# Raiden-Makoto/MLX-VAE

Hardware: AMD Instinct MI355X
Metric: SELFIES sequences/sec (whole node), AR-CVAE training step (higher is better)
Workload: dtype f32

## Files before the change

### include/arcvae_hip.h

```cpp
#ifndef ARCVAE_HIP_H
#define ARCVAE_HIP_H

#include <stdint.h>

#ifdef __cplusplus
extern "C" {
#endif

#define ARCVAE_OK 0
#define ARCVAE_ERR_ARG (-1)
#define ARCVAE_ERR_LAUNCH (-2)
#define ARCVAE_ERR_DEVICE (-3)

#define ARCVAE_GEMM_ACCUMULATE 1
#define ARCVAE_GEMM_TANH 2
#define ARCVAE_GEMM_SPLITK 4
#define ARCVAE_GEMM_NO_SKINNY 8
#define ARCVAE_GEMM_TILE64 16
#define ARCVAE_GEMM_TILE128 32
#define ARCVAE_GEMM_DTANH 64
#define ARCVAE_GEMM_TILE_WIDE 128
#define ARCVAE_GEMM_BF16 256
#define ARCVAE_GEMM_SPLIT3 512
#define ARCVAE_GEMM_QUIET 1024
#define ARCVAE_LSTM_RETILE 1
#define ARCVAE_LSTM_BF16 2
#define ARCVAE_LSTM_SPLIT3 4
#define ARCVAE_PERSIST_BF16 2
#define ARCVAE_RS_HALF 16
#define ARCVAE_RS_HALF1 32
#define ARCVAE_DEC_SPLIT3 512
#define ARCVAE_DEC_NO_GPRE 1024
#define ARCVAE_DEC_PART_HEAD 2048
#define ARCVAE_DEC_PART_TAIL 4096
#define ARCVAE_DEC_BF16 256

#ifdef ARCVAE_HIP_BUILD
typedef hipStream_t arcvae_stream_t;
#else
typedef void* arcvae_stream_t;
#endif

int arcvae_abi_version(int* arch_gfx950);

int arcvae_gemm_f32(int transA, int transB, int M, int N, int K, const float* A, int lda,
                    const float* B, int ldb, float* C, int ldc, const float* bias, int flags,
                    arcvae_stream_t stream);

int arcvae_enc_lstm_ws_floats(int B, int T, int H, int L, int flags, long* floats );
int arcvae_transpose_tokens(const int32_t* src_bt, int32_t* dst_tb, int B, int T, arcvae_stream_t stream);
int arcvae_enc_lstm_forward(const int32_t* x_tb, const float* table0, const float* const* Wx,
                            const float* const* Wh, const float* const* bias, float* hseq, float* hseq_t,
                            float* cseq, float* gseq, float* wt, float* wT_bwd , int B, int T, int V,
                            int H, int L, int flags , const long* ws_floats ,
                            void* h_oct ,
                            unsigned long long* trace , arcvae_stream_t stream);
int arcvae_enc_lstm_tiled(int B, int H, int L);
int arcvae_enc_lstm_tiled_for(int B, int H, int L, int flags);
int arcvae_enc_lstm_operand_slots(int B, int T, int H, int L, int flags);
int arcvae_enc_lstm_backward(const float* const* Wx, const float* const* Wh, const float* cseq,
                             const float* gseq, const float* dh_top, int ld_dh_top, float* dG, float* dG_t,
                             float* dcs, float* dxs, float* wT, int B, int T, int H, int L, int s_begin,
                             int s_end, int flags ,
                             const long* ws_floats ,
                             void* dG_oct ,
                             unsigned* start_signal ,
                             unsigned long long* trace , arcvae_stream_t stream);
int arcvae_enc_lstm_persistent_ok(int B, int T, int H, int L);
int arcvae_enc_lstm_forward_persistent(const int32_t* x_tb, const float* table0, const float* const* Wx,
                                       const float* const* Wh, const float* const* bias, float* hseq, float* cseq,
                                       float* gseq, float* wT_bwd, long wT_bwd_floats , float* comb ,
                                       unsigned* sync_ws, unsigned* start_signal, int B, int T, int V, int H, int L,
                                       int flags, unsigned long long* trace, arcvae_stream_t stream);
int arcvae_enc_prologue(const int32_t* x_bt, int32_t* x_tb, float* zero_f32, long n_zero, float* zero2_f32 , long n_zero2,
                        unsigned* sync_ws, int n_sync, int sync_keep ,
                        const float* cond, const float* Wc, const float* bc, float* comb, float* stats, int n_stats,
                        float* onehot_ws, int V, int B, int T, int H, int C, arcvae_stream_t stream);
int arcvae_enc_lstm_bwd_persistent_ok(int B, int T, int H, int L);
int arcvae_enc_lstm_backward_persistent(const float* cseq, const float* gseq, const float* dh_top, int ld_dh_top,
                                        float* dG, float* dcs, float* dxs, const float* wT, unsigned* sync_ws,
                                        unsigned* start_signal, int B, int T, int H, int L, int s_begin, int s_end,
                                        int chunk_index, unsigned long long* trace, arcvae_stream_t stream);
int arcvae_enc_lstm_bwd_rs_ok(int B, int T, int H, int L);
long arcvae_enc_lstm_bwd_rs_part_floats(int B, int T, int H, int L);
int arcvae_enc_lstm_bwd_rs_halves(int B, int T, int H, int L);
int arcvae_enc_lstm_persist_groups(int B, int H, int L);
int arcvae_enc_lstm_backward_persistent_rs(const float* const* Wx, const float* const* Wh, const float* cseq,
                                           const float* gseq, const float* dh_top, int ld_dh_top, float* dG, float* dcs,
                                           float* dxs, float* part_ws, long part_ws_floats, unsigned* sync_ws,
                                           unsigned* start_signal, int B, int T, int H, int L, int s_begin, int s_end, int chunk_index,
                                           int flags ,
                                           unsigned long long* trace,
                                           arcvae_stream_t stream);
int arcvae_enc_lstm_backward_fused(const float* const* Wx, const float* const* Wh, const float* cseq, const float* gseq,
                                   const float* hseq, const int32_t* x_tb, const float* dh_top, int ld_dh_top,
                                   float* dG, float* dcs, float* dxs, float* part_ws, long part_ws_floats, unsigned* sync_ws,
                                   unsigned* start_signal, float* const* dWx, float* const* dWh, float* const* dbias,
                                   float* dtable_ws, int B, int T, int V, int H, int L, int s_begin, int s_end,
                                   int chunk_index, unsigned long long* trace, arcvae_stream_t stream);
int arcvae_enc_lstm_wgrad(const int32_t* x_tb, const float* emb, const float* Wx0, const float* hseq,
                          const float* dG, float* dtable_ws, float* onehot_ws, float* dEmb, float* const* dWx,
                          float* const* dWh, float* const* dbias, int B, int T, int V, int E, int H, int L,
                          int t_lo, int t_hi, int first, int last, int parts ,
                          const void* h_oct, const void* dG_oct ,
                          const long* ws_floats , arcvae_stream_t stream);

int arcvae_enc_heads_forward(const float* hT, const float* cond, const float* Wc, const float* bc,
                             const float* Wmu, const float* bmu, const float* Wlh, const float* blh,
                             const float* Wlv, const float* blv, const float* eps, float* comb, float* lh,
                             float* mu_raw, float* lv_raw, float* mu, float* logvar, float* z, float* stats,
                             int B, int H, int Z, int C, float free_bits, int comb_ready, arcvae_stream_t stream);
int arcvae_enc_seam_ok(int B, int H, int Z);
int arcvae_enc_seam(const float* comb, const float* Wmu, const float* bmu, const float* Wlh, const float* blh, const float* Wlv,
                    const float* blv, const float* eps, const float* hyper, float* lh, float* mu_raw, float* lv_raw, float* mu,
                    float* logvar, float* z, float* stats, float* scalars, float* dmu_raw, float* dlv_raw, float* dlh, float* dcomb,
                    unsigned* sync_ws, int B, int H, int Z, int T, float free_bits, int phases, int flags, arcvae_stream_t stream);
int arcvae_stats_set_recon(const float* rowloss, int B, float* stats, int Z, arcvae_stream_t stream);
int arcvae_latent_loss(const float* stats, const float* hyper, const float* mu, const float* logvar,
                       float* scalars, float* dmu_raw, float* dlv_raw, int B, int Z, int T, float free_bits,
                       arcvae_stream_t stream);
int arcvae_loss_finalize(const float* stats, float* scalars, int Z, int T, const unsigned* guard_a,
                         const unsigned* guard_b, arcvae_stream_t stream);
int arcvae_recon_finalize(const float* rowloss, int B, float* stats, float* scalars, int Z, int T,
                          const unsigned* guard_a, const unsigned* guard_b, arcvae_stream_t stream);
int arcvae_enc_heads_backward(const float* cond, const float* Wmu, const float* Wlh, const float* Wlv,
                              const float* comb, const float* lh, const float* dmu_raw, const float* dlv_raw,
                              float* dlh, float* dcomb, float* dWc, float* dbc, float* dWmu, float* dbmu,
                              float* dWlh, float* dblh, float* dWlv, float* dblv, int B, int H, int Z, int C,
                              int phase , arcvae_stream_t stream);

int arcvae_reparameterize(const float* mu, const float* logvar, const float* eps, float* z, long n,
                          arcvae_stream_t stream);
int arcvae_latent_stats(const float* mu, const float* logvar, float* stats, float* krow, int B, int Z,
                        float free_bits, arcvae_stream_t stream);
int arcvae_ce_rows(const float* logits, const int32_t* targets, float* ce, long R, int V, arcvae_stream_t stream);
int arcvae_sum(const float* x, long n, float* out, float scale, arcvae_stream_t stream);

int arcvae_dec_forward_dense(const float* emb, const float* const* Wx, const float* const* bias,
                             const float* Wout, const float* bout, const float* cond, float* tableD,
                             float* hact, float* gpre, float* logits, float* lse, int32_t* nxt, int B, int V,
                             int E, int C, int H, int L, int mode, float temperature, arcvae_stream_t stream);
int arcvae_dec_chain_ce(const int32_t* x, const uint8_t* coins, const int32_t* nxt, const float* lse,
                        const float* logits, int32_t* fed, float* rowloss, int B, int T, int V,
                        arcvae_stream_t stream);
int arcvae_dec_ce_backward(const int32_t* x, const int32_t* fed, const float* logits, const float* lse,
                           float* dlogits, int B, int T, int V, float inv_count, arcvae_stream_t stream);
int arcvae_dec_gather_logits(const float* dense, const int32_t* fed, float* out, int B, int T, int V,
                             arcvae_stream_t stream);
int arcvae_dec_sample_chain(const int32_t* nxt, int32_t* tokens, int32_t* first_end, int B, int V,
                            int max_len, int end_token, arcvae_stream_t stream);
int arcvae_dec_sample_chain_categorical(const float* dense_logits, int32_t* tokens, int32_t* first_end, int B, int V, int max_len,
                                        int end_token, float temperature, unsigned long long seed, arcvae_stream_t stream);
int arcvae_dec_row_lse(const float* dense_logits, float* lse, long R, int V, float temperature, arcvae_stream_t stream);
int arcvae_dec_beam_ws_bytes(int B, int K, int max_len, long* bytes);
int arcvae_dec_beam_search(const float* dense_logits, const float* lse, int32_t* tokens, float* scores, int32_t* lengths, void* ws,
                           long ws_bytes, int B, int V, int K, int max_len, int min_len, int end_token, int pad_token,
                           float temperature, arcvae_stream_t stream);
int arcvae_dec_sequence_logprob(const float* dense_logits, const float* lse, const int32_t* tokens, float* out, int B, int T, int V,
                                int end_token, float temperature, arcvae_stream_t stream);
int arcvae_dec_viterbi_ws_bytes(int B, int V, int max_len, long* bytes);
int arcvae_dec_viterbi(const float* dense_logits, const float* lse, int32_t* tokens, float* score, int32_t* length, void* ws,
                       long ws_bytes, int B, int V, int max_len, int min_len, int end_token, int pad_token, float temperature,
                       arcvae_stream_t stream);
int arcvae_dec_chain_marginals(const float* dense_logits, const float* lse, float* alive, int B, int V, int max_len, int end_token,
                               float temperature, arcvae_stream_t stream);
#define ARCVAE_KBEST_ROWS_IN_FLIGHT 1024
int arcvae_dec_kbest_ws_bytes(int B, int V, int K, int max_len, long* bytes);
int arcvae_dec_kbest(const float* dense_logits, const float* lse, int32_t* tokens , float* scores ,
                     int32_t* lengths , void* ws, long ws_bytes, int B, int V, int K, int max_len, int min_len,
                     int end_token, int pad_token, float temperature, arcvae_stream_t stream);
int arcvae_dec_topkp_rows(const float* dense_logits, long table_rows, const int32_t* rows, long R, int V, float temperature,
                          int top_k, float top_p, int32_t* count, int32_t* tokens, float* cum, arcvae_stream_t stream);
int arcvae_dec_topkp_ws_bytes(int B, int V, int top_k, long* bytes);
int arcvae_dec_sample_chain_topkp(const float* dense_logits, int32_t* tokens, int32_t* first_end, void* ws, long ws_bytes, int B,
                                  int V, int max_len, int end_token, float temperature, int top_k, float top_p,
                                  const unsigned long long* seed, arcvae_stream_t stream);
int arcvae_dec_backward_dense(const float* emb, const float* const* Wx, const float* const* bias,
                              const float* Wout, const float* cond, const float* tableD, const float* hact,
                              const float* gpre, const float* dlogits, float* dh, float* dG, float* dtableD,
                              float* wcpart, float* dEmb, float* const* dWx, float* const* dbias, float* dWout,
                              float* dbout, int B, int V, int E, int C, int H, int L, int flags ,
                              arcvae_stream_t stream);

int arcvae_dense_stack_ok(long R, int H, int L);
int arcvae_dense_stack_ws_floats(long R, int H, int L, long* floats );
int arcvae_dense_stack_forward(const float* const* Wx, const float* const* bias, float* hact, float* gates, float* ws,
                               long ws_floats , long R,
                               int H, int L, int flags ,
                               arcvae_stream_t stream);
int arcvae_dense_stack_backward(const float* gates, const float* dh_top, float* dG, float* dh0, float* const* dWx,
                                float* const* dbias, float* ws, long ws_floats, long R, int H, int L, int flags , arcvae_stream_t stream);

int arcvae_adam_update(float* params, const float* grads, float* m, float* v, long n, double lr,
                       double beta1, double beta2, double eps, const unsigned* guard_a, const unsigned* guard_b,
                       arcvae_stream_t stream);

int arcvae_adam_update_finalize(float* params, const float* grads, float* m, float* v, long n, double lr, double beta1,
                                double beta2, double eps, const unsigned* guard_a, const unsigned* guard_b,
                                const float* rowloss, int B, float* stats, float* scalars, int Z, int T, arcvae_stream_t stream);

int arcvae_prop_ws_floats(int B, int Z, int C, int Hp, long* floats);
int arcvae_prop_forward(const float* z, const float* cond, const float* W1, const float* b1, const float* W2,
                        const float* b2, const float* hyper, float* pred, float* scalars, float* ws, long ws_floats,
                        int B, int Z, int C, int Hp, arcvae_stream_t stream);
int arcvae_prop_backward(const float* z, const float* cond, const float* eps, const float* mu_raw, const float* lv_raw,
                         const float* W1, const float* b1, const float* W2, const float* b2, const float* hyper,
                         float* d_mu_raw, float* d_lv_raw, float* pred, float* ws, long ws_floats, int B, int Z, int C,
                         int Hp, arcvae_stream_t stream);
int arcvae_prop_wgrad(const float* z, const float* ws, long ws_floats, const float* hyper, float* dW1, float* db1,
                      float* dW2, float* db2, float* scalars, int B, int Z, int C, int Hp, arcvae_stream_t stream);

int arcvae_grad_sumsq_partials(long n, long* count);
int arcvae_grad_sumsq(const float* grads, long n, float* partials, long partials_cap, arcvae_stream_t stream);
int arcvae_adam_update_clipped(float* params, const float* grads, float* m, float* v, long n, double lr, double beta1,
                               double beta2, double eps, const unsigned* guard_a, const unsigned* guard_b,
                               const float* partials, long n_partials, double max_norm, float* scalars, arcvae_stream_t stream);
int arcvae_adam_update_finalize_clipped(float* params, const float* grads, float* m, float* v, long n, double lr,
                                        double beta1, double beta2, double eps, const unsigned* guard_a,
                                        const unsigned* guard_b, const float* rowloss, int B, float* stats, float* scalars,
                                        int Z, int T, const float* partials, long n_partials, double max_norm,
                                        arcvae_stream_t stream);

int arcvae_adam_step(float* params, const float* grads, float* m, float* v, long n,
                     const float* lr_dev,
                     double beta1, double beta2, double eps,
                     const unsigned* guard_a, const unsigned* guard_b,
                     const float* rowloss, int B, float* stats, float* scalars, int Z, int T,
                     const float* partials, long n_partials, double max_norm,
                     arcvae_stream_t stream);

int arcvae_colsum_accum(const float* X, int rows, int cols, int ld, float* out, float scale,
                        arcvae_stream_t stream);
int arcvae_segsum_rows_accum(const float* X, const int32_t* seg, int rows, int nseg, int cols, float* out,
                             arcvae_stream_t stream);
int arcvae_transpose_batched(const float* const* src, float* const* dst, const int* rows, const int* cols,
                             int n, arcvae_stream_t stream);
int arcvae_debug_occupy(int blocks, int threads, int lds_bytes, int spin_us, arcvae_stream_t stream);
int arcvae_scale_inplace(float* x, long n, float s, arcvae_stream_t stream);
int arcvae_zero(float* x, int rows, int cols, int ld, arcvae_stream_t stream);
int arcvae_table_finalize(const float* dT, const float* Wx0, int ldw, const float* emb, float* dEmb, float* dWx0,
                          float* db0, int V, int E, int G, arcvae_stream_t stream);
int arcvae_table_fold(const float* dT, const float* dT2, const float* Wx0, int ldw, const float* emb, float* dEmb,
                      float* dWx0, float* db0, int V, int E, int G, int g_lo, int g_hi, arcvae_stream_t stream);
int arcvae_gate_wait(const unsigned* flag, unsigned* steps, unsigned stride, unsigned offset, int advance,
                     unsigned max_polls, unsigned* err, arcvae_stream_t stream);
int arcvae_gate_set(unsigned* flag, unsigned value, int add, arcvae_stream_t stream);
// ... 9 lines not shown
```

### mlx-vae_amd/arcvae_hip/_lib.py

```python
from __future__ import annotations

import ctypes as C
import os
from typing import Iterable, Optional, Sequence

import torch

_HERE = os.path.dirname(os.path.abspath(__file__))
LIB_PATH = os.environ.get("ARCVAE_HIP_LIB", os.path.join(_HERE, "libarcvae_hip.so"))

GEMM_ACCUMULATE = 1
GEMM_TANH = 2
GEMM_SPLITK = 4
GEMM_NO_SKINNY = 8
GEMM_BF16 = 256
GEMM_SPLIT3 = 512
GEMM_QUIET = 1024
LSTM_RETILE = 1
LSTM_BF16 = 2
LSTM_SPLIT3 = 4
RS_HALF, RS_HALF1 = 16, 32
PERSIST_BF16 = 2
DEC_BF16 = 256
DEC_SPLIT3 = 512
DEC_PART_HEAD = 2048
DEC_PART_TAIL = 4096
DEC_NO_GPRE = 1024
WGRAD_BF16 = 128
WGRAD_QUIET = 512
WGRAD_FOLD = 8192

_vp = C.c_void_p
_i = C.c_int
_f = C.c_float
_d = C.c_double
_l = C.c_long
_pp = C.POINTER(C.c_void_p)
_ip = C.POINTER(C.c_int)
_lp = C.POINTER(C.c_long)

SIGNATURES = {
    "arcvae_abi_version": [_ip],
    "arcvae_gemm_f32": [_i, _i, _i, _i, _i, _vp, _i, _vp, _i, _vp, _i, _vp, _i, _vp],
    "arcvae_transpose_tokens": [_vp, _vp, _i, _i, _vp],
    "arcvae_enc_lstm_ws_floats": [_i, _i, _i, _i, _i, _lp],
    "arcvae_enc_lstm_forward": [_vp, _vp, _pp, _pp, _pp, _vp, _vp, _vp, _vp, _vp, _vp, _i, _i, _i, _i, _i, _i, _lp, _vp, _vp, _vp],
    "arcvae_enc_lstm_tiled": [_i, _i, _i],
    "arcvae_enc_lstm_tiled_for": [_i, _i, _i, _i],
    "arcvae_enc_lstm_operand_slots": [_i, _i, _i, _i, _i],
    "arcvae_dense_stack_ok": [_l, _i, _i],
    "arcvae_dense_stack_ws_floats": [_l, _i, _i, _lp],
    "arcvae_dense_stack_forward": [_pp, _pp, _vp, _vp, _vp, _l, _l, _i, _i, _i, _vp],
    "arcvae_dense_stack_backward": [_vp, _vp, _vp, _vp, _pp, _pp, _vp, _l, _l, _i, _i, _i, _vp],
    "arcvae_enc_lstm_persistent_ok": [_i, _i, _i, _i],
    "arcvae_enc_lstm_forward_persistent": [_vp, _vp, _pp, _pp, _pp, _vp, _vp, _vp, _vp, _l, _vp, _vp, _vp, _i, _i, _i, _i, _i, _i, _vp, _vp],
    "arcvae_enc_prologue": [_vp, _vp, _vp, _l, _vp, _l, _vp, _i, _i, _vp, _vp, _vp, _vp, _vp, _i, _vp, _i, _i, _i, _i, _i, _vp],
    "arcvae_enc_lstm_bwd_persistent_ok": [_i, _i, _i, _i],
    "arcvae_enc_lstm_backward_persistent": [_vp, _vp, _vp, _i, _vp, _vp, _vp, _vp, _vp, _vp, _i, _i, _i, _i, _i, _i, _i, _vp, _vp],
    "arcvae_enc_lstm_bwd_rs_ok": [_i, _i, _i, _i],
    "arcvae_enc_lstm_bwd_rs_halves": [_i, _i, _i, _i],
    "arcvae_enc_lstm_persist_groups": [_i, _i, _i],
    "arcvae_enc_lstm_bwd_rs_part_floats": [_i, _i, _i, _i],
    "arcvae_enc_lstm_backward_persistent_rs": [_pp, _pp, _vp, _vp, _vp, _i, _vp, _vp, _vp, _vp, _l, _vp, _vp, _i, _i, _i, _i, _i, _i, _i, _i, _vp, _vp],
    "arcvae_enc_lstm_backward_fused": [_pp, _pp, _vp, _vp, _vp, _vp, _vp, _i, _vp, _vp, _vp, _vp, _l, _vp, _vp, _pp, _pp, _pp, _vp,
                                       _i, _i, _i, _i, _i, _i, _i, _i, _vp, _vp],
    "arcvae_enc_lstm_backward": [_pp, _pp, _vp, _vp, _vp, _i, _vp, _vp, _vp, _vp, _vp, _i, _i, _i, _i, _i, _i, _i, _lp, _vp, _vp, _vp, _vp],
    "arcvae_enc_lstm_wgrad": [_vp, _vp, _vp, _vp, _vp, _vp, _vp, _vp, _pp, _pp, _pp, _i, _i, _i, _i, _i, _i, _i, _i, _i, _i, _i, _vp, _vp, _lp, _vp],
    "arcvae_enc_heads_forward": [_vp] * 19 + [_i, _i, _i, _i, _f, _i, _vp],
    "arcvae_enc_seam_ok": [_i, _i, _i],
    "arcvae_enc_seam": [_vp] * 22 + [_i, _i, _i, _i, _f, _i, _i, _vp],
    "arcvae_stats_set_recon": [_vp, _i, _vp, _i, _vp],
    "arcvae_latent_loss": [_vp, _vp, _vp, _vp, _vp, _vp, _vp, _i, _i, _i, _f, _vp],
    "arcvae_loss_finalize": [_vp, _vp, _i, _i, _vp, _vp, _vp],
    "arcvae_recon_finalize": [_vp, _i, _vp, _vp, _i, _i, _vp, _vp, _vp],
    "arcvae_enc_heads_backward": [_vp] * 18 + [_i, _i, _i, _i, _i, _vp],
    "arcvae_dec_forward_dense": [_vp, _pp, _pp, _vp, _vp, _vp, _vp, _vp, _vp, _vp, _vp, _vp,
                                 _i, _i, _i, _i, _i, _i, _i, _f, _vp],
    "arcvae_dec_chain_ce": [_vp, _vp, _vp, _vp, _vp, _vp, _vp, _i, _i, _i, _vp],
    "arcvae_dec_ce_backward": [_vp, _vp, _vp, _vp, _vp, _i, _i, _i, _f, _vp],
    "arcvae_dec_gather_logits": [_vp, _vp, _vp, _i, _i, _i, _vp],
    "arcvae_dec_sample_chain": [_vp, _vp, _vp, _i, _i, _i, _i, _vp],
    "arcvae_dec_sample_chain_categorical": [_vp, _vp, _vp, _i, _i, _i, _i, _f, C.c_ulonglong, _vp],
    "arcvae_dec_row_lse": [_vp, _vp, _l, _i, _f, _vp],
    "arcvae_dec_beam_ws_bytes": [_i, _i, _i, _lp],
    "arcvae_dec_beam_search": [_vp, _vp, _vp, _vp, _vp, _vp, _l, _i, _i, _i, _i, _i, _i, _i, _f, _vp],
    "arcvae_dec_sequence_logprob": [_vp, _vp, _vp, _vp, _i, _i, _i, _i, _f, _vp],
    "arcvae_dec_viterbi_ws_bytes": [_i, _i, _i, _lp],
    "arcvae_dec_viterbi": [_vp, _vp, _vp, _vp, _vp, _vp, _l, _i, _i, _i, _i, _i, _i, _f, _vp],
    "arcvae_dec_chain_marginals": [_vp, _vp, _vp, _i, _i, _i, _i, _f, _vp],
    "arcvae_dec_kbest_ws_bytes": [_i, _i, _i, _i, _lp],
    "arcvae_dec_kbest": [_vp, _vp, _vp, _vp, _vp, _vp, _l, _i, _i, _i, _i, _i, _i, _i, _f, _vp],
    "arcvae_dec_topkp_rows": [_vp, _l, _vp, _l, _i, _f, _i, _f, _vp, _vp, _vp, _vp],
    "arcvae_dec_topkp_ws_bytes": [_i, _i, _i, _lp],
    "arcvae_dec_sample_chain_topkp": [_vp, _vp, _vp, _vp, _l, _i, _i, _i, _i, _f, _i, _f, _vp, _vp],
    "arcvae_dec_backward_dense": [_vp, _pp, _pp, _vp, _vp, _vp, _vp, _vp, _vp, _vp, _vp, _vp, _vp, _vp,
                                  _pp, _pp, _vp, _vp, _i, _i, _i, _i, _i, _i, _i, _vp],
    "arcvae_reparameterize": [_vp, _vp, _vp, _vp, _l, _vp],
    "arcvae_latent_stats": [_vp, _vp, _vp, _vp, _i, _i, _f, _vp],
    "arcvae_ce_rows": [_vp, _vp, _vp, _l, _i, _vp],
    "arcvae_sum": [_vp, _l, _vp, _f, _vp],
    "arcvae_adam_update": [_vp, _vp, _vp, _vp, _l, _d, _d, _d, _d, _vp, _vp, _vp],
    "arcvae_adam_update_finalize": [_vp, _vp, _vp, _vp, _l, _d, _d, _d, _d, _vp, _vp, _vp, _i, _vp, _vp, _i, _i, _vp],
    "arcvae_colsum_accum": [_vp, _i, _i, _i, _vp, _f, _vp],
    "arcvae_segsum_rows_accum": [_vp, _vp, _i, _i, _i, _vp, _vp],
    "arcvae_transpose_batched": [_pp, _pp, _ip, _ip, _i, _vp],
    "arcvae_scale_inplace": [_vp, _l, _f, _vp],
    "arcvae_debug_occupy": [_i, _i, _i, _i, _vp],
    "arcvae_zero": [_vp, _i, _i, _i, _vp],
    "arcvae_table_finalize": [_vp, _vp, _i, _vp, _vp, _vp, _vp, _i, _i, _i, _vp],
    "arcvae_table_fold": [_vp, _vp, _vp, _i, _vp, _vp, _vp, _vp, _i, _i, _i, _i, _i, _vp],
    "arcvae_gate_wait": [_vp, _vp, C.c_uint, C.c_uint, _i, C.c_uint, _vp, _vp],
    "arcvae_gate_set": [_vp, C.c_uint, _i, _vp],
    "arcvae_tile_weights": [_pp, _pp, _ip, _ip, _i, _i, _vp],
    "arcvae_copy_buffers": [_pp, _pp, _lp, _i, _vp],
    "arcvae_prop_ws_floats": [_i, _i, _i, _i, _lp],
    "arcvae_prop_forward": [_vp] * 10 + [_l, _i, _i, _i, _i, _vp],
    "arcvae_prop_backward": [_vp] * 14 + [_l, _i, _i, _i, _i, _vp],
    "arcvae_prop_wgrad": [_vp, _vp, _l] + [_vp] * 6 + [_i, _i, _i, _i, _vp],
    "arcvae_grad_sumsq_partials": [_l, _lp],
    "arcvae_grad_sumsq": [_vp, _l, _vp, _l, _vp],
    "arcvae_adam_update_clipped": [_vp, _vp, _vp, _vp, _l, _d, _d, _d, _d, _vp, _vp, _vp, _l, _d, _vp, _vp],
    "arcvae_adam_update_finalize_clipped": [_vp, _vp, _vp, _vp, _l, _d, _d, _d, _d, _vp, _vp, _vp, _i, _vp, _vp, _i, _i,
                                            _vp, _l, _d, _vp],
    "arcvae_adam_step": [_vp, _vp, _vp, _vp, _l, _vp, _d, _d, _d, _vp, _vp, _vp, _i, _vp, _vp, _i, _i, _vp, _l, _d, _vp],
}

LONG_RESULTS = {"arcvae_enc_lstm_bwd_rs_part_floats"}

_lib: Optional[C.CDLL] = None


class ArcvaeHipError(RuntimeError):
    pass


def load() -> C.CDLL:
    global _lib
    if _lib is not None:
        return _lib
    if not os.path.exists(LIB_PATH):
        raise ArcvaeHipError(
            f"{LIB_PATH} not found: build it with `make -C mlx-vae_amd/csrc` "
            "(or `python -c 'import __graft_entry__ as g; g.build()'`). There is no CPU fallback.")
    lib = C.CDLL(LIB_PATH)
    for name, argtypes in SIGNATURES.items():
        fn = getattr(lib, name)
        fn.argtypes = argtypes
        fn.restype = C.c_long if name in LONG_RESULTS else C.c_int
    _lib = lib
    return lib


def check(rc: int, what: str) -> None:
    if rc != 0:
        raise ArcvaeHipError(f"{what} failed with code {rc} "
                             "(-1 bad argument/shape, -2 launch error, -3 device)")


def call(name: str, *args) -> None:
    check(getattr(load(), name)(*args), name)


def ptr(t: Optional[torch.Tensor]) -> C.c_void_p:
    if t is None:
        return C.c_void_p(0)
    if not t.is_cuda:
        raise ArcvaeHipError("arcvae_hip kernels need device tensors (no CPU path)")
    if not t.is_contiguous():
        raise ArcvaeHipError("arcvae_hip kernels need contiguous tensors")
    return C.c_void_p(t.data_ptr())


def ptr_array(ts: Sequence[Optional[torch.Tensor]]):
    arr = (C.c_void_p * len(ts))()
    for i, t in enumerate(ts):
        arr[i] = None if t is None else ptr(t).value
    return C.cast(arr, _pp), arr


def stream_ptr(stream: Optional[torch.cuda.Stream] = None) -> C.c_void_p:
    s = stream if stream is not None else torch.cuda.current_stream()
    return C.c_void_p(s.cuda_stream)


def gemm(transA: bool, transB: bool, M: int, N: int, K: int, A: torch.Tensor, lda: int, Bm: torch.Tensor,
         ldb: int, Cm: torch.Tensor, ldc: int, bias: Optional[torch.Tensor] = None, flags: int = 0,
         a_off: int = 0, b_off: int = 0, c_off: int = 0) -> None:
    def p(t, off):
        return C.c_void_p(t.data_ptr() + 4 * off)
    call("arcvae_gemm_f32", int(transA), int(transB), M, N, K, p(A, a_off), lda, p(Bm, b_off), ldb,
         p(Cm, c_off), ldc, ptr(bias), flags, stream_ptr())
```

### mlx-vae_amd/arcvae_hip/engine.py

```python
from __future__ import annotations

import ctypes as C
import dataclasses
import os
from typing import Dict, Optional, Sequence, Tuple

import numpy as np
import torch

from . import _lib
from ._lib import call, ptr, ptr_array, stream_ptr
from .store import ParamStore

SCALAR_KEYS = ("total_loss", "recon_loss", "kl_loss", "weighted_kl", "collapse_penalty", "prop_loss",
               "weighted_prop_loss", "mutual_info", "mi_penalty")


@dataclasses.dataclass(frozen=True)
class ModelDims:
    V: int
    E: int
    H: int
    Z: int
    C: int
# ... 5 lines not shown
        if not (1 <= self.L <= 8):
            raise ValueError("num_layers must be in [1, 8]")
        if not (1 <= self.C <= 8):
            raise ValueError("num_conditions must be in [1, 8]")
        if not (2 <= self.V <= 255):
            raise ValueError("vocab_size must be in [2, 255] (the vocabulary-dense decoder's per-row V x V histogram lives in LDS)")


class DeviceRate:
    __slots__ = ("word",)

    def __init__(self, word: torch.Tensor):
        self.word = word


LR_DEVICE = "lr_device"


def lr_key(lr):
    return LR_DEVICE if isinstance(lr, DeviceRate) else float(lr)


class Workspace:

    def __init__(self, d: ModelDims, B: int, T: int, device, train: bool = True):
        f32 = dict(dtype=torch.float32, device=device)
        i32 = dict(dtype=torch.int32, device=device)
        V, E, H, Z, Cc, L = d.V, d.E, d.H, d.Z, d.C, d.L
        G, BV = 4 * H, B * V
        self.B, self.T = B, T
        self.bf16 = False
        self.bf16_parts = 0
        self.planes = False
        self.x = torch.zeros(B, T, **i32)
        self.x_tb = torch.zeros(T, B, **i32)
        self.coins = torch.ones(T, dtype=torch.uint8, device=device)
        self.cond = torch.zeros(B, Cc, **f32)
        self._hyper_vals = None
        self.eps = torch.zeros(B, Z, **f32)
        self.hyper = torch.zeros(8, **f32)
        self.rate = DeviceRate(torch.zeros(1, **f32))
        self._rate_val = None
        self.table0 = torch.empty(V, G, **f32)
        self.hseq = torch.empty(L, T, B, H, **f32)
        RS = int(os.environ.get("ARCVAE_RING", "16"))
        RS = T if (RS <= 0 or RS > T) else RS
        self.hseq_t = torch.empty(L, RS, B * H * 3 // 2, **f32)
        self.wt = torch.empty(2 * L - 1, G * H * 3 // 2, **f32)
        self.cseq = torch.empty(L, T, B, H, **f32)
        self.gseq = torch.empty(L, T, B, G, **f32)
        self.comb = torch.empty(B, 2 * H, **f32)
        self.lh = torch.empty(B, 2 * H, **f32)
        self.mu_raw = torch.empty(B, Z, **f32)
        self.lv_raw = torch.empty(B, Z, **f32)
        self.mu = torch.empty(B, Z, **f32)
        self.logvar = torch.empty(B, Z, **f32)
        self.z = torch.empty(B, Z, **f32)
        self.stats = torch.zeros(2 * Z + 4, **f32)
        self.psync = torch.zeros(8192, **i32)
        self.psync_words = 5696
        self.seam_bwd_done = False
        self.bptt_rearmed = False
        self.trace_fwd: Optional[torch.Tensor] = None
        self.trace_bwd: Optional[torch.Tensor] = None
        self.scalars = torch.zeros(16, **f32)
        self.tableD = torch.empty(V, G, **f32)
        self.hact = torch.empty(L, BV, H, **f32)
        self.gpre = torch.empty(max(L - 1, 1), BV, G, **f32)
        self.logits = torch.empty(BV, V, **f32)
        self.lse = torch.empty(BV, **f32)
        self.nxt = torch.zeros(BV, **i32)
        self.fed = torch.zeros(B, T, **i32)
        self.rowloss = torch.zeros(B, **f32)
        if train:
            self.dmu_raw = torch.empty(B, Z, **f32)
            self.dlv_raw = torch.empty(B, Z, **f32)
            self.dlh = torch.empty(B, 2 * H, **f32)
            self.dcomb = torch.empty(B, 2 * H, **f32)
            self.dG = self.gseq if os.environ.get("ARCVAE_INPLACE_DG", "1") != "0" else torch.empty(L, T, B, G, **f32)
            self.dG_t = torch.empty(L, RS, B * G * 3 // 2, **f32)
            self.dcs = torch.empty(L, RS, B, H, **f32)
            self.dxs = torch.empty(L, RS, B, H, **f32)
            self.wT = torch.empty(2 * L - 1, H * G * 3 // 2, **f32)
            self.dtables = torch.zeros(2, V, G, **f32)
            self.dtable0 = self.dtables[0]
            self.dtable1 = self.dtables[1]
            self.tables_zeroed = False
            self.onehot = torch.empty(T * B, (V + 3) // 4 * 4, **f32)
            npart = _lib.load().arcvae_enc_lstm_bwd_rs_part_floats(B, T, H, L)
            if npart > 0:
                self.ppart = torch.empty(npart, **f32)
            self.dlogits = torch.empty(BV, V, **f32)
            self.ddh = torch.empty(2, BV, H, **f32)
            self.ddG = torch.empty(BV, G, **f32)
            self.dtableD = torch.empty(V, G, **f32)
            self.wcpart = torch.empty(V, G, max(Cc, 1), **f32)


def _lstm_flags(ws) -> int:
    if ws.bf16_parts & 1:
        return _lib.LSTM_BF16
    return _lib.LSTM_SPLIT3 if os.environ.get("ARCVAE_LSTM_SPLIT3", "1") != "0" else 0


def _caps(ws, h=None, g=None):
    def n(t):
        return 0 if t is None else t.numel() * t.element_size() // 4
    h = ws.hseq_t if h is None else h
    g = getattr(ws, "dG_t", None) if g is None else g
    return (C.c_long * 4)(n(h), n(g), n(ws.wt), n(getattr(ws, "wT", None)))


def _oct(ws, name: str) -> C.c_void_p:
    t = getattr(ws, name, None)
    return ptr(t) if t is not None else C.c_void_p(0)


def _layer_ptrs(store: ParamStore, L: int, leaf: str, grad: bool = False, skip0: bool = False):
    get = store.g if grad else store.p
    ts = [None if (skip0 and l == 0) else get(f"lstm_layer_{l}.{leaf}") for l in range(L)]
    return ptr_array(ts)


def bptt_reduce_scatter_ok(ws, d: ModelDims) -> bool:
    if os.environ.get("ARCVAE_PERSIST_BWD", "3") != "3":
        return False
    return _lib.load().arcvae_enc_lstm_bwd_rs_ok(ws.B, ws.T, d.H, d.L) == 1


def fused_wgrad_ok(ws, d: ModelDims) -> bool:
    return os.environ.get("ARCVAE_FUSED_WGRAD", "0") == "1" and d.V <= 128 and bptt_reduce_scatter_ok(ws, d)


def persistent_forward_ok(ws: Workspace, d: ModelDims) -> bool:
    return _lib.load().arcvae_enc_lstm_persistent_ok(ws.B, ws.T, d.H, d.L) == 1


def seam_fused_ok(ws: Workspace, d: ModelDims) -> bool:
    return persistent_forward_ok(ws, d) and _lib.load().arcvae_enc_seam_ok(ws.B, d.H, d.Z) == 1


def encoder_seam(enc: ParamStore, ws: Workspace, d: ModelDims, free_bits: float, phases: int) -> None:
    train = (phases & 2) != 0
    call("arcvae_enc_seam", ptr(ws.comb), ptr(enc.p("fc_mu.weight")), ptr(enc.p("fc_mu.bias")),
         ptr(enc.p("fc_logvar_hidden.weight")), ptr(enc.p("fc_logvar_hidden.bias")), ptr(enc.p("fc_logvar.weight")),
         ptr(enc.p("fc_logvar.bias")), ptr(ws.eps), ptr(ws.hyper), ptr(ws.lh), ptr(ws.mu_raw), ptr(ws.lv_raw), ptr(ws.mu),
         ptr(ws.logvar), ptr(ws.z), ptr(ws.stats), ptr(ws.scalars), ptr(ws.dmu_raw) if train else C.c_void_p(0),
         ptr(ws.dlv_raw) if train else C.c_void_p(0), ptr(ws.dlh) if train else C.c_void_p(0),
         ptr(ws.dcomb) if train else C.c_void_p(0), ptr(ws.psync), ws.B, d.H, d.Z, ws.T, float(free_bits), phases, 1, stream_ptr())
    if train:
        ws.seam_bwd_done = True


def encoder_forward(enc: ParamStore, ws: Workspace, d: ModelDims, free_bits: float,
                    start_signal: Optional[C.c_void_p] = None, zero_grad: bool = False, seam: int = 1) -> None:
    B, T = ws.B, ws.T
    G = 4 * d.H
    s = stream_ptr()
    wx, _k1 = _layer_ptrs(enc, d.L, "Wx", skip0=True)
    wh, _k2 = _layer_ptrs(enc, d.L, "Wh")
    bs, _k3 = _layer_ptrs(enc, d.L, "bias", skip0=True)
    if persistent_forward_ok(ws, d):
        grad = enc.grad if zero_grad else None
        tabs = ws.dtables if (zero_grad and hasattr(ws, "dtables")) else None
        ws.tables_zeroed = tabs is not None
        ws.bptt_rearmed = True
        call("arcvae_enc_prologue", ptr(ws.x), ptr(ws.x_tb), ptr(grad), C.c_long(grad.numel() if grad is not None else 0),
             ptr(tabs), C.c_long(tabs.numel() if tabs is not None else 0), ptr(ws.psync), ws.psync_words, 500, ptr(ws.cond), ptr(enc.p("condition_fc.weight")), ptr(enc.p("condition_fc.bias")),
             ptr(ws.comb), ptr(ws.stats), 2 * d.Z + 4, ptr(ws.onehot) if (zero_grad and hasattr(ws, "onehot")) else C.c_void_p(0),
             d.V, B, T, d.H, d.C, s)
        comb_ready = 1
        call("arcvae_gemm_f32", 0, 1, d.V, G, d.E, ptr(enc.p("embedding.weight")), d.E,
             ptr(enc.p("lstm_layer_0.Wx")), d.E, ptr(ws.table0), G, ptr(enc.p("lstm_layer_0.bias")), 0, s)
        need_wT = hasattr(ws, "wT") and not bptt_reduce_scatter_ok(ws, d)
        call("arcvae_enc_lstm_forward_persistent", ptr(ws.x_tb), ptr(ws.table0), wx, wh, bs, ptr(ws.hseq),
             ptr(ws.cseq), ptr(ws.gseq), ptr(ws.wT) if need_wT else C.c_void_p(0), C.c_long(ws.wT.numel() if need_wT else 0),
             ptr(ws.comb), ptr(ws.psync),
             start_signal if start_signal is not None else C.c_void_p(0), B, T, d.V, d.H, d.L,
             1 | (_lib.PERSIST_BF16 if ws.bf16_parts & 1 else 0) | (_lstm_flags(ws) & _lib.LSTM_SPLIT3), ptr(ws.trace_fwd), s)
    else:
        comb_ready = 0
        if zero_grad:
            enc.grad.zero_()
        call("arcvae_transpose_tokens", ptr(ws.x), ptr(ws.x_tb), B, T, s)
        call("arcvae_gemm_f32", 0, 1, d.V, G, d.E, ptr(enc.p("embedding.weight")), d.E,
             ptr(enc.p("lstm_layer_0.Wx")), d.E, ptr(ws.table0), G, ptr(enc.p("lstm_layer_0.bias")), 0, s)
        wT = ptr(ws.wT) if hasattr(ws, "wT") else C.c_void_p(0)
        if start_signal is not None:
            call("arcvae_gate_set", start_signal, 1, 1, s)
        call("arcvae_enc_lstm_forward", ptr(ws.x_tb), ptr(ws.table0), wx, wh, bs, ptr(ws.hseq), ptr(ws.hseq_t),
             ptr(ws.cseq), ptr(ws.gseq), ptr(ws.wt), wT, B, T, d.V, d.H, d.L, _lstm_flags(ws), _caps(ws),
             _oct(ws, "h_oct"), ptr(ws.trace_fwd), s)
    if comb_ready and seam_fused_ok(ws, d):
        encoder_seam(enc, ws, d, free_bits, 3 if (seam == 3 and hasattr(ws, "dcomb")) else 1)
        return
    hT = ws.hseq[d.L - 1, T - 1]
    call("arcvae_enc_heads_forward", ptr(hT), ptr(ws.cond), ptr(enc.p("condition_fc.weight")),
         ptr(enc.p("condition_fc.bias")), ptr(enc.p("fc_mu.weight")), ptr(enc.p("fc_mu.bias")),
         ptr(enc.p("fc_logvar_hidden.weight")), ptr(enc.p("fc_logvar_hidden.bias")),
         ptr(enc.p("fc_logvar.weight")), ptr(enc.p("fc_logvar.bias")), ptr(ws.eps), ptr(ws.comb), ptr(ws.lh),
         ptr(ws.mu_raw), ptr(ws.lv_raw), ptr(ws.mu), ptr(ws.logvar), ptr(ws.z), ptr(ws.stats), B, d.H, d.Z,
         d.C, float(free_bits), comb_ready, s)


def _dec_gemm_bits(ws) -> int:
    if ws.bf16_parts & 2:
        return _lib.DEC_BF16
    return _lib.DEC_SPLIT3 if getattr(ws, "dec_split3", False) else 0


def decoder_forward_dense(dec: ParamStore, ws: Workspace, d: ModelDims, mode: int = 0,
                          temperature: float = 1.0, keep_gpre: bool = True, alone: bool = False) -> None:
    if not keep_gpre:
        mode |= _lib.DEC_NO_GPRE
    wx, _k1 = _layer_ptrs(dec, d.L, "Wx")
    bs, _k2 = _layer_ptrs(dec, d.L, "bias")

    def part(bits):
        call("arcvae_dec_forward_dense", ptr(dec.p("embedding.weight")), wx, bs, ptr(dec.p("fc_out.weight")),
             ptr(dec.p("fc_out.bias")), ptr(ws.cond), ptr(ws.tableD), ptr(ws.hact), ptr(ws.gpre), ptr(ws.logits),
             ptr(ws.lse), ptr(ws.nxt), ws.B, d.V, d.E, d.C, d.H, d.L, mode | bits | _dec_gemm_bits(ws),
             float(temperature), stream_ptr())

    if alone and not keep_gpre and not (ws.bf16_parts & 2) and os.environ.get("ARCVAE_SAMPLER_TILED", "0") == "1" \
            and _lib.load().arcvae_dense_stack_ok(ws.B * d.V, d.H, d.L) == 1:
        if getattr(ws, "dense_ws_fwd", None) is None:
            n = C.c_long(0)
            _lib.load().arcvae_dense_stack_ws_floats(ws.B * d.V, d.H, d.L, C.byref(n))
            ws.dense_ws_fwd = torch.empty(n.value, dtype=torch.float32, device=ws.hact.device)
        mode &= ~_lib.DEC_NO_GPRE
        part(_lib.DEC_PART_HEAD)
        call("arcvae_dense_stack_forward", wx, bs, ptr(ws.hact), C.c_void_p(0), ptr(ws.dense_ws_fwd), C.c_long(ws.dense_ws_fwd.numel()),
             ws.B * d.V, d.H, d.L, 1, stream_ptr())
        part(_lib.DEC_PART_TAIL)
        return
    if keep_gpre and getattr(ws, "dense_ws", None) is not None:
        part(_lib.DEC_PART_HEAD)
        call("arcvae_dense_stack_forward", wx, bs, ptr(ws.hact), ptr(ws.gpre), ptr(ws.dense_ws), C.c_long(ws.dense_ws.numel()),
             ws.B * d.V, d.H, d.L, _lib.LSTM_BF16 if (ws.bf16_parts & 2) else 0, stream_ptr())
        part(_lib.DEC_PART_TAIL)
        ws.dense_fwd = True
        return
    ws.dense_fwd = False
    part(0)


def decoder_chain(ws: Workspace, d: ModelDims) -> None:
    call("arcvae_dec_chain_ce", ptr(ws.x), ptr(ws.coins), ptr(ws.nxt), ptr(ws.lse), ptr(ws.logits), ptr(ws.fed),
         ptr(ws.rowloss), ws.B, ws.T, d.V, stream_ptr())


def decoder_backward(dec: ParamStore, ws: Workspace, d: ModelDims, inv_count: float) -> None:
    s = stream_ptr()
    call("arcvae_dec_ce_backward", ptr(ws.x), ptr(ws.fed), ptr(ws.logits), ptr(ws.lse), ptr(ws.dlogits), ws.B,
         ws.T, d.V, float(inv_count), s)
    wx, _k1 = _layer_ptrs(dec, d.L, "Wx")
    bs, _k2 = _layer_ptrs(dec, d.L, "bias")
    dwx, _k3 = _layer_ptrs(dec, d.L, "Wx", grad=True)
    dbs, _k4 = _layer_ptrs(dec, d.L, "bias", grad=True)

    def part(bits, dh):
        call("arcvae_dec_backward_dense", ptr(dec.p("embedding.weight")), wx, bs, ptr(dec.p("fc_out.weight")),
             ptr(ws.cond), ptr(ws.tableD), ptr(ws.hact), ptr(ws.gpre), ptr(ws.dlogits), dh, ptr(ws.ddG),
             ptr(ws.dtableD), ptr(ws.wcpart), ptr(dec.g("embedding.weight")), dwx, dbs, ptr(dec.g("fc_out.weight")),
             ptr(dec.g("fc_out.bias")), ws.B, d.V, d.E, d.C, d.H, d.L, bits | _dec_gemm_bits(ws), s)

    if getattr(ws, "dense_fwd", False):
        part(_lib.DEC_PART_TAIL, ptr(ws.ddh))
        call("arcvae_dense_stack_backward", ptr(ws.gpre), ptr(ws.ddh[0]), ptr(ws.ddG), ptr(ws.ddh[1]), dwx, dbs,
             ptr(ws.dense_ws), C.c_long(ws.dense_ws.numel()), ws.B * d.V, d.H, d.L, _lib.LSTM_BF16 if (ws.bf16_parts & 2) else 0, s)
        part(_lib.DEC_PART_HEAD, ptr(ws.ddh[1]))
        return
    part(0, ptr(ws.ddh))


def latent_loss(ws: Workspace, d: ModelDims, free_bits: float, with_grads: bool) -> None:
    call("arcvae_latent_loss", ptr(ws.stats), ptr(ws.hyper), ptr(ws.mu), ptr(ws.logvar), ptr(ws.scalars),
         ptr(ws.dmu_raw) if with_grads else C.c_void_p(0), ptr(ws.dlv_raw) if with_grads else C.c_void_p(0),
         ws.B, d.Z, ws.T, float(free_bits), stream_ptr())


def prop_backward(prop: ParamStore, ws: Workspace, d: ModelDims, hp: int) -> None:
    call("arcvae_prop_backward", ptr(ws.z), ptr(ws.cond), ptr(ws.eps), ptr(ws.mu_raw), ptr(ws.lv_raw),
         ptr(prop.p("fc1.weight")), ptr(prop.p("fc1.bias")), ptr(prop.p("fc2.weight")), ptr(prop.p("fc2.bias")),
         ptr(ws.hyper), ptr(ws.dmu_raw), ptr(ws.dlv_raw), ptr(ws.pred), ptr(ws.prop_ws), C.c_long(ws.prop_ws.numel()),
         ws.B, d.Z, d.C, hp, stream_ptr())


def prop_wgrad(prop: ParamStore, ws: Workspace, d: ModelDims, hp: int) -> None:
    call("arcvae_prop_wgrad", ptr(ws.z), ptr(ws.prop_ws), C.c_long(ws.prop_ws.numel()), ptr(ws.hyper),
         ptr(prop.g("fc1.weight")), ptr(prop.g("fc1.bias")), ptr(prop.g("fc2.weight")), ptr(prop.g("fc2.bias")),
         ptr(ws.scalars), ws.B, d.Z, d.C, hp, stream_ptr())


def prop_forward(prop: ParamStore, ws: Workspace, d: ModelDims, hp: int) -> None:
    call("arcvae_prop_forward", ptr(ws.z), ptr(ws.cond), ptr(prop.p("fc1.weight")), ptr(prop.p("fc1.bias")),
         ptr(prop.p("fc2.weight")), ptr(prop.p("fc2.bias")), ptr(ws.hyper), ptr(ws.pred), ptr(ws.scalars),
         ptr(ws.prop_ws), C.c_long(ws.prop_ws.numel()), ws.B, d.Z, d.C, hp, stream_ptr())


def _inline(key, fn, stream) -> None:
    with torch.cuda.stream(stream):
        fn()


class Gates:
    STRIDE = 9
    LONG, SHORT = 16_000_000, 3_000
    P, Q, NS, NA, ERR, PROBE, R, NM, D, H, HG = range(11)

    def __init__(self, device):
        self.mem = torch.zeros(11 * 32, dtype=torch.int32, device=device)
        self._probed: Dict[Tuple[int, int], bool] = {}

    def word(self, i: int) -> C.c_void_p:
        return C.c_void_p(self.mem.data_ptr() + 128 * i)

    def signal(self, w: int, add: int = 1) -> None:
        call("arcvae_gate_set", self.word(w), add, 1, stream_ptr())

    def wait(self, w: int, steps: int, stride: int, offset: int, advance: bool = False) -> None:
        call("arcvae_gate_wait", self.word(w), self.word(steps), stride, offset, int(advance), self.LONG,
             self.word(self.ERR), stream_ptr())

    def join(self) -> None:
        self.wait(self.R, self.NM, 2, 2, advance=True)

    def errors(self) -> int:
        return int(self.mem[self.ERR * 32].item())

    def probe(self, waiter: torch.cuda.Stream, signaller: torch.cuda.Stream) -> bool:
        key = (waiter.cuda_stream, signaller.cuda_stream)
        if key not in self._probed:
            torch.cuda.synchronize()
            self.mem[self.PROBE * 32] = 0
            before = self.errors()
            with torch.cuda.stream(waiter):
                call("arcvae_gate_wait", self.word(self.PROBE), C.c_void_p(0), 0, 1, 0, self.SHORT,
                     self.word(self.ERR), stream_ptr())
            with torch.cuda.stream(signaller):
                call("arcvae_gate_set", self.word(self.PROBE), 1, 0, stream_ptr())
            torch.cuda.synchronize()
            ok = self.errors() == before
            self.mem[self.ERR * 32] = before
            torch.cuda.synchronize()
            self._probed[key] = ok
        return self._probed[key]


class SegmentRunner:

    def __init__(self, capture: bool):
        self.capture = capture
        self._g: Dict[str, object] = {}
        self._cap_stream: Optional[torch.cuda.Stream] = None
        self.steps = 0

    def __call__(self, key: str, fn, stream: torch.cuda.Stream, eager_first: bool = True) -> None:
        with torch.cuda.stream(stream):
            if not self.capture:
                fn()
                return
            g = self._g.get(key)
            if g is None and not eager_first:
                try:
                    if self._cap_stream is None:
                        self._cap_stream = torch.cuda.Stream(device=stream.device)
                    g = torch.cuda.CUDAGraph()
                    with torch.cuda.graph(g, stream=self._cap_stream, capture_error_mode="thread_local"):
                        fn()
                    self._g[key] = g
                    g.replay()
                except Exception as exc:
                    print(f"[arcvae_hip] graph capture of segment {key!r} failed ({exc}); running it eagerly")
                    torch.cuda.synchronize()
                    self._g[key] = False
                    fn()
                return
            if g is None:
                fn()
                stream.synchronize()
                try:
                    if self._cap_stream is None:
                        self._cap_stream = torch.cuda.Stream(device=stream.device)
                    g = torch.cuda.CUDAGraph()
                    with torch.cuda.graph(g, stream=self._cap_stream, capture_error_mode="thread_local"):
                        fn()
                    self._g[key] = g
                except Exception as exc:
                    print(f"[arcvae_hip] graph capture of segment {key!r} failed ({exc}); running it eagerly")
                    torch.cuda.synchronize()
                    self._g[key] = False
            elif g is False:
                fn()
            else:
                g.replay()


WGRAD_QUIET_DEFAULT = "1"
TAIL_FORM_DEFAULT = "1"


def wgrad_quiet() -> bool:
    return os.environ.get("ARCVAE_WGRAD_QUIET", WGRAD_QUIET_DEFAULT) != "0"


class EncoderBackwardPlan:

    FRACTIONS_LAUNCHES = "0.3,0.6,0.85,1.0"
    FRACTIONS_PERSISTENT = "0.63,1.0"
    FRACTIONS_QUIET = "0.7,1.0"
    FRACTIONS_FUSED = "1.0"

    def __init__(self, enc: ParamStore, ws: Workspace, d: ModelDims):
        self.enc, self.ws, self.d = enc, ws, d
        L, T = d.L, ws.T
        self.persistent = bptt_reduce_scatter_ok(ws, d)
        self.fused = fused_wgrad_ok(ws, d)
        self.quiet = (self.persistent and not self.fused and ws.B <= 64 and wgrad_quiet()
                      and not getattr(ws, "bf16", False))
        default = self.FRACTIONS_FUSED if self.fused else (self.FRACTIONS_QUIET if self.quiet else
                                                           (self.FRACTIONS_PERSISTENT if self.persistent else self.FRACTIONS_LAUNCHES))
        self.FRACTIONS = tuple(float(f) for f in os.environ.get("ARCVAE_BPTT_CHUNKS", default).split(","))
        self.S = T + 2 * (L - 1)
        self._wx = _layer_ptrs(enc, L, "Wx", skip0=True)
        self._wh = _layer_ptrs(enc, L, "Wh")
        self._dwx = _layer_ptrs(enc, L, "Wx", grad=True)
        self._dwh = _layer_ptrs(enc, L, "Wh", grad=True)
        self._dbs = _layer_ptrs(enc, L, "bias", grad=True)
        self.chunks = self.chunk_schedule(T, L, self.FRACTIONS)

    @staticmethod
    def chunk_schedule(T: int, L: int, fractions) -> list:
        S = T + 2 * (L - 1)
        bounds = sorted({0, S} | {min(S, max(1, round(f * S))) for f in fractions})
        chunks = []
        t_hi = T
        for s0, s1 in zip(bounds[:-1], bounds[1:]):
            t_lo = 0 if s1 >= S else min(T, max(0, T - s1 + 2 * (L - 1)))
            chunks.append((s0, s1, t_lo, t_hi, t_hi == T, s1 >= S))
            t_hi = t_lo
        return chunks

    def heads(self, phase: int) -> None:
        enc, ws, d = self.enc, self.ws, self.d
        if phase in (0, 1) and getattr(ws, "seam_bwd_done", False):
            ws.seam_bwd_done = False
            if phase == 1:
                return
            phase = 2
        call("arcvae_enc_heads_backward", ptr(ws.cond), ptr(enc.p("fc_mu.weight")),
             ptr(enc.p("fc_logvar_hidden.weight")), ptr(enc.p("fc_logvar.weight")), ptr(ws.comb), ptr(ws.lh),
             ptr(ws.dmu_raw), ptr(ws.dlv_raw), ptr(ws.dlh), ptr(ws.dcomb), ptr(enc.g("condition_fc.weight")),
             ptr(enc.g("condition_fc.bias")), ptr(enc.g("fc_mu.weight")), ptr(enc.g("fc_mu.bias")),
             ptr(enc.g("fc_logvar_hidden.weight")), ptr(enc.g("fc_logvar_hidden.bias")),
             ptr(enc.g("fc_logvar.weight")), ptr(enc.g("fc_logvar.bias")), ws.B, d.H, d.Z, d.C, phase, stream_ptr())

    def sweep(self, s0: int, s1: int, start_signal: Optional[C.c_void_p] = None, chunk_index: int = 0) -> None:
        ws, d = self.ws, self.d
        sig = start_signal if start_signal is not None else C.c_void_p(0)
        rearmed = 1 if (chunk_index == 0 and getattr(ws, "bptt_rearmed", False)) else 0
        if chunk_index == 0:
            ws.bptt_rearmed = False
        if self.fused:
            enc = self.enc
            call("arcvae_enc_lstm_backward_fused", self._wx[0], self._wh[0], ptr(ws.cseq), ptr(ws.gseq), ptr(ws.hseq),
                 ptr(ws.x_tb), ptr(ws.dcomb), 2 * d.H, ptr(ws.dG), ptr(ws.dcs), ptr(ws.dxs), ptr(ws.ppart), C.c_long(ws.ppart.numel()), ptr(ws.psync),
                 sig, self._dwx[0], self._dwh[0], self._dbs[0], ptr(ws.dtable0), ws.B, ws.T, d.V, d.H, d.L, s0, s1,
                 chunk_index, ptr(ws.trace_bwd), stream_ptr())
            return
        if self.persistent:
            halves = _lib.load().arcvae_enc_lstm_bwd_rs_halves(ws.B, ws.T, d.H, d.L) == 1
            for hf in ((_lib.RS_HALF, _lib.RS_HALF | _lib.RS_HALF1) if halves else (0,)):
                call("arcvae_enc_lstm_backward_persistent_rs", self._wx[0], self._wh[0], ptr(ws.cseq), ptr(ws.gseq),
                     ptr(ws.dcomb), 2 * d.H, ptr(ws.dG), ptr(ws.dcs), ptr(ws.dxs), ptr(ws.ppart), C.c_long(ws.ppart.numel()), ptr(ws.psync),
                     sig if not (hf & _lib.RS_HALF1) else C.c_void_p(0),
                     ws.B, ws.T, d.H, d.L, s0, s1, chunk_index, (_lib.PERSIST_BF16 if ws.bf16_parts & 1 else 0) | rearmed | hf,
                     ptr(ws.trace_bwd) if not (hf & _lib.RS_HALF1) else C.c_void_p(0), stream_ptr())
            return
        if _lib.load().arcvae_enc_lstm_bwd_persistent_ok(ws.B, ws.T, d.H, d.L) == 1:
            call("arcvae_enc_lstm_backward_persistent", ptr(ws.cseq), ptr(ws.gseq), ptr(ws.dcomb), 2 * d.H, ptr(ws.dG),
                 ptr(ws.dcs), ptr(ws.dxs), ptr(ws.wT), ptr(ws.psync), sig, ws.B, ws.T, d.H, d.L, s0, s1, chunk_index,
                 ptr(ws.trace_bwd), stream_ptr())
            return
        call("arcvae_enc_lstm_backward", self._wx[0], self._wh[0], ptr(ws.cseq), ptr(ws.gseq), ptr(ws.dcomb),
             2 * d.H, ptr(ws.dG), ptr(ws.dG_t), ptr(ws.dcs), ptr(ws.dxs), ptr(ws.wT), ws.B, ws.T, d.H, d.L, s0, s1,
             _lstm_flags(ws),
             _caps(ws), _oct(ws, "dG_oct"), start_signal if start_signal is not None else C.c_void_p(0), ptr(ws.trace_bwd), stream_ptr())

    def wgrad(self, t_lo: int, t_hi: int, first: bool, last: bool, parts: int = 3, table=None) -> None:
        enc, ws, d = self.enc, self.ws, self.d
        if os.environ.get("ARCVAE_DEBUG_SKIP_WGRAD", "0") == "1":
            return
        if self.fused:
            if last and (parts & 2):
                call("arcvae_table_finalize", ptr(ws.dtable0), ptr(enc.p("lstm_layer_0.Wx")), d.E,
                     ptr(enc.p("embedding.weight")), ptr(enc.g("embedding.weight")), ptr(enc.g("lstm_layer_0.Wx")),
                     ptr(enc.g("lstm_layer_0.bias")), d.V, d.E, 4 * d.H, stream_ptr())
            return
        if (ws.bf16_parts & 4) and not self.persistent:
            parts |= _lib.WGRAD_BF16
        elif getattr(ws, "pl_g", None) is not None:
            parts |= 2048 | 4096 | 16
            call("arcvae_enc_lstm_wgrad", ptr(ws.x_tb), ptr(enc.p("embedding.weight")), ptr(enc.p("lstm_layer_0.Wx")),
                 ptr(ws.hseq), ptr(ws.dG), ptr(table if table is not None else ws.dtable0), ptr(ws.onehot),
                 ptr(enc.g("embedding.weight")), self._dwx[0], self._dwh[0], self._dbs[0], ws.B, ws.T, d.V, d.E, d.H, d.L,
                 t_lo, t_hi, int(first), int(last), parts, ptr(ws.pl_h), ptr(ws.pl_g), _caps(ws, ws.pl_h, ws.pl_g), stream_ptr())
            return
        elif getattr(ws, "planes", False) and not self.persistent:
            parts |= 2048 | 16
            call("arcvae_enc_lstm_wgrad", ptr(ws.x_tb), ptr(enc.p("embedding.weight")), ptr(enc.p("lstm_layer_0.Wx")),
                 ptr(ws.hseq), ptr(ws.dG), ptr(table if table is not None else ws.dtable0), ptr(ws.onehot),
                 ptr(enc.g("embedding.weight")), self._dwx[0], self._dwh[0], self._dbs[0], ws.B, ws.T, d.V, d.E, d.H, d.L,
                 t_lo, t_hi, int(first), int(last), parts, ptr(ws.hseq_t), ptr(ws.dG_t), _caps(ws), stream_ptr())
            return
        elif (not self.persistent and os.environ.get("ARCVAE_WGRAD_SPLIT3", "1") != "0"
              and (_lib.load().arcvae_enc_lstm_tiled_for(ws.B, d.H, d.L, _lstm_flags(ws)) & 2)):
            parts |= 1024 | 16
        elif not (self.persistent and ws.B <= 64):
            parts |= 16
        elif last and os.environ.get("ARCVAE_WIDE_TAIL", "0") == "1":
            parts |= 64
        elif self.quiet:
            parts |= _lib.WGRAD_QUIET
        call("arcvae_enc_lstm_wgrad", ptr(ws.x_tb), ptr(enc.p("embedding.weight")), ptr(enc.p("lstm_layer_0.Wx")),
             ptr(ws.hseq), ptr(ws.dG), ptr(table if table is not None else ws.dtable0), ptr(ws.onehot),
             ptr(enc.g("embedding.weight")), self._dwx[0],
             self._dwh[0],
             self._dbs[0], ws.B, ws.T, d.V, d.E, d.H, d.L, t_lo, t_hi, int(first), int(last), parts,
             _oct(ws, "h_oct"), _oct(ws, "dG_oct"), None, stream_ptr())


def encoder_backward(enc: ParamStore, ws: Workspace, d: ModelDims, aux: Optional[torch.cuda.Stream] = None,
                     run=_inline, prologue=None, after_first=None, aux2: Optional[torch.cuda.Stream] = None,
                     gates: Optional[Gates] = None, epilogue=None) -> None:
    plan = EncoderBackwardPlan(enc, ws, d)
    main = torch.cuda.current_stream()
    if aux is None:
        def everything():
            if prologue:
                prologue()
            plan.heads(0)
            plan.sweep(0, plan.S)
            plan.wgrad(0, ws.T, True, True)
        run("enc_all", everything, main)
        if after_first:
            after_first()
        return
    if gates is not None:
        _encoder_backward_gated(plan, ws, aux, aux2, run, prologue, after_first, gates, epilogue)
        return
    for c, (s0, s1, t_lo, t_hi, first, last) in enumerate(plan.chunks):
        def main_seg(c=c, s0=s0, s1=s1):
            if c == 0:
                if prologue:
                    prologue()
                plan.heads(1)
            plan.sweep(s0, s1, None, c)

        split_tail = last and aux2 is not None

        def aux_seg(c=c, t_lo=t_lo, t_hi=t_hi, first=first, last=last, split_tail=split_tail):
            if c == 0:
                plan.heads(2)
            plan.wgrad(t_lo, t_hi, first, last, 1 if split_tail else 3)

        run(f"main{c}", main_seg, main)
        if c == 0 and after_first:
            after_first()
        ev = torch.cuda.Event()
        ev.record(main)
        aux.wait_event(ev)
        if split_tail:
            aux2.wait_stream(aux)
            aux2.wait_event(ev)
            run(f"aux2_{c}", lambda a=t_lo, b=t_hi, f=first, l=last: plan.wgrad(a, b, f, l, 2), aux2)
        run(f"aux{c}", aux_seg, aux)
    main.wait_stream(aux)
    if aux2 is not None:
        main.wait_stream(aux2)


def _tables_on_main(plan, ws) -> bool:
    return (ws is not None and hasattr(ws, "dtable1") and os.environ.get("ARCVAE_TABLE_ON_MAIN", "1") != "0"
            and bool(getattr(plan, "persistent", False)) and persistent_forward_ok(ws, plan.d))


def _encoder_backward_gated(plan: EncoderBackwardPlan, ws: Workspace, aux, aux2, run, prologue, after_first,
                            g: Gates, epilogue=None) -> None:
    main = torch.cuda.current_stream()
    nc = len(plan.chunks)
    if nc + 1 > g.STRIDE:
        raise ValueError("too many BPTT chunks for the gate stride")
    if getattr(plan, "fused", False) and nc == 1 and aux2 is not None:
        _encoder_backward_gated_fused(plan, ws, aux, aux2, run, prologue, after_first, g)
        return
    tail_on_side = aux2 is not None and nc >= 2
    table_on_side = tail_on_side and os.environ.get("ARCVAE_TABLE_ON_SIDE", "1") != "0"
    mid_batch = ws is not None and ws.B >= 256 and not (_lib.load().arcvae_enc_lstm_tiled_for(ws.B, plan.d.H, plan.d.L, _lstm_flags(ws)) & 2)
    two_launches = (plan.persistent and not getattr(plan, "quiet", False)) or mid_batch
    wx_on_side = table_on_side and os.environ.get("ARCVAE_WX_ON_SIDE", "1" if two_launches else "0") != "0"
    own_tables = table_on_side and _tables_on_main(plan, ws)
    tail_form1 = (own_tables and bool(getattr(plan, "quiet", False)) and not wx_on_side
                  and os.environ.get("ARCVAE_TAIL_FORM", TAIL_FORM_DEFAULT) == "1")

    def pre_zeroed() -> int:
        return 256 if (nc == 2 and ws is not None and getattr(ws, "tables_zeroed", False)) else 0

    def main_seg():
        if prologue:
            prologue()
        plan.heads(1)
        for c, (s0, s1, _t_lo, _t_hi, _first, _last) in enumerate(plan.chunks):
            plan.sweep(s0, s1, g.word(g.P) if c > 0 else g.word(g.H), c)
        g.signal(g.P, g.STRIDE - nc)
        if tail_form1:
            _s0, _s1, t_lo_l, t_hi_l, first_l, last_l = plan.chunks[-1]
            plan.wgrad(t_lo_l, t_hi_l, first_l, last_l, 1)
        elif own_tables:
            _s0, _s1, t_lo_l, t_hi_l, _f, _l = plan.chunks[-1]
            plan.wgrad(t_lo_l, t_hi_l, True, True, 2 | 32 | pre_zeroed(), table=getattr(ws, "dtable1", None))
        if epilogue is not None:
            epilogue()

    if epilogue is not None:
# ... 582 lines not shown
```

### mlx-vae_amd/csrc/latent.hip

```cpp
#include "ops.h"
#include "skinny.h"
#include "xcd.h"

namespace {

__global__ __launch_bounds__(256) void build_comb_kernel(const float* __restrict__ hT,
                                                         const float* __restrict__ cond,
                                                         const float* __restrict__ Wc,
                                                         const float* __restrict__ bc, float* comb, float* stats,
                                                         int nstats, int B, int H, int C) {
    const int idx = blockIdx.x * blockDim.x + threadIdx.x;
    if (idx < nstats) stats[idx] = 0.f;
    if (idx >= B * 2 * H) return;
    const int b = idx / (2 * H), j = idx % (2 * H);
    float v;
    if (j < H) {
        v = hT[(long)b * H + j];
    } else {
        const int u = j - H;
        float s = 0.f;
        for (int c = 0; c < C; ++c) s += cond[b * C + c] * Wc[u * C + c];
        v = s + bc[u];
    }
    comb[idx] = v;
// ... 243 lines not shown
                       logvar, z, stats, B, Z, fb_min);
    return arcvae_launch_status();
}

extern "C" int arcvae_stats_set_recon(const float* rowloss, int B, float* stats, int Z, hipStream_t stream) {
    if (!rowloss || !stats || B <= 0 || Z <= 0) return ARCVAE_ERR_ARG;
    hipLaunchKernelGGL(sum_to_kernel, dim3(1), dim3(256), 0, stream, rowloss, B, stats + 2 * Z + 3);
    return arcvae_launch_status();
}

extern "C" int arcvae_latent_loss(const float* stats, const float* hyper, const float* mu, const float* logvar,
                                  float* scalars, float* dmu_raw, float* dlv_raw, int B, int Z, int T,
                                  float free_bits, hipStream_t stream) {
    if (!stats || !hyper || !mu || !logvar || !scalars || B <= 0 || Z <= 0 || T <= 0) return ARCVAE_ERR_ARG;
    if (dmu_raw && dlv_raw) {
        const float fb_min = free_bits > 0.0f ? free_bits / (float)Z : 0.0f;
        hipLaunchKernelGGL(latent_grad_kernel, dim3(ceil_div(B * Z, 256)), dim3(256), 0, stream, mu, logvar, stats,
                           hyper, scalars, dmu_raw, dlv_raw, B, Z, T, fb_min);
    } else {
        hipLaunchKernelGGL(latent_scalars_kernel, dim3(1), dim3(256), 0, stream, stats, hyper, scalars, Z, T);
    }
    return arcvae_launch_status();
}

namespace {
__device__ __forceinline__ bool step_guard_tripped(const unsigned* ga, const unsigned* gb) {
    return (ga && __hip_atomic_load(ga, __ATOMIC_RELAXED, __HIP_MEMORY_SCOPE_AGENT) != 0u) ||
           (gb && __hip_atomic_load(gb, __ATOMIC_RELAXED, __HIP_MEMORY_SCOPE_AGENT) != 0u);
}
__device__ __forceinline__ void poison_scalars(float* scalars) {
    for (int i = 0; i < 9; ++i) scalars[i] = __builtin_nanf("");
    scalars[15] = 1.0f;
}
__global__ void loss_finalize_kernel(const float* __restrict__ stats, float* scalars, int Z, int T,
                                     const unsigned* ga, const unsigned* gb) {
    if (threadIdx.x == 0 && blockIdx.x == 0) {
        const float recon = stats[2 * Z + 3] / (stats[2 * Z + 2] * (float)T);
        scalars[1] = recon;
        scalars[0] = recon + scalars[3] + scalars[4] + scalars[6] + scalars[8];
        scalars[15] = 0.0f;
        if (step_guard_tripped(ga, gb)) poison_scalars(scalars);
    }
}
}

namespace {
__global__ __launch_bounds__(256) void recon_finalize_kernel(const float* __restrict__ rowloss, int n, float* stats,
                                                             float* scalars, int Z, int T, const unsigned* ga,
                                                             const unsigned* gb) {
    float s = 0.f;
    for (int i = threadIdx.x; i < n; i += 256) s += rowloss[i];
    __shared__ float red[4];
    s = wave_sum(s);
    if ((threadIdx.x & 63) == 0) red[threadIdx.x >> 6] = s;
    __syncthreads();
    if (threadIdx.x == 0) {
        const float ce = (red[0] + red[1]) + (red[2] + red[3]);
        stats[2 * Z + 3] = ce;
        const float recon = ce / (stats[2 * Z + 2] * (float)T);
        scalars[1] = recon;
        scalars[0] = recon + scalars[3] + scalars[4] + scalars[6] + scalars[8];
        scalars[15] = 0.0f;
        if (step_guard_tripped(ga, gb)) poison_scalars(scalars);
    }
}
}

extern "C" int arcvae_recon_finalize(const float* rowloss, int B, float* stats, float* scalars, int Z, int T,
                                     const unsigned* guard_a, const unsigned* guard_b, hipStream_t stream) {
    if (!rowloss || !stats || !scalars || B <= 0 || Z <= 0 || T <= 0) return ARCVAE_ERR_ARG;
    hipLaunchKernelGGL(recon_finalize_kernel, dim3(1), dim3(256), 0, stream, rowloss, B, stats, scalars, Z, T, guard_a,
                       guard_b);
    return arcvae_launch_status();
}

extern "C" int arcvae_loss_finalize(const float* stats, float* scalars, int Z, int T, const unsigned* guard_a,
                                    const unsigned* guard_b, hipStream_t stream) {
    if (!stats || !scalars || Z <= 0 || T <= 0) return ARCVAE_ERR_ARG;
    hipLaunchKernelGGL(loss_finalize_kernel, dim3(1), dim3(64), 0, stream, stats, scalars, Z, T, guard_a, guard_b);
    return arcvae_launch_status();
}


namespace {
struct HeadsWg {
    const float* A[4];
    const float* B[4];
    float* C[4];
    float* bias[4];
    int M[4], N[4], lda[4], ldb[4], ldc[4];
    int tile0[5];
    int K;
};
__global__ __launch_bounds__(256) void heads_wgrad_kernel(HeadsWg g) {
    __shared__ __attribute__((aligned(16))) float As[16][64];
    __shared__ __attribute__((aligned(16))) float Bs[16][64];
    int pi = 0;
    while (pi < 3 && (int)blockIdx.x >= g.tile0[pi + 1]) ++pi;
    const int t = blockIdx.x - g.tile0[pi];
    const int M = g.M[pi], N = g.N[pi], ntn = N > 0 ? (N + 63) >> 6 : 1;
    const int m0 = (t / ntn) * 64, n0 = (t % ntn) * 64;
    const float* __restrict__ A = g.A[pi];
    const float* __restrict__ Bm = g.B[pi];
    const int lda = g.lda[pi], ldb = g.ldb[pi];
    const int tid = threadIdx.x, tx = tid & 15, ty = tid >> 4;
    float acc[4][4], bsum[4] = {0.f, 0.f, 0.f, 0.f};
#pragma unroll
    for (int i = 0; i < 4; ++i)
#pragma unroll
        for (int j = 0; j < 4; ++j) acc[i][j] = 0.f;
    for (int k0 = 0; k0 < g.K; k0 += 16) {
#pragma unroll
        for (int e = 0; e < 4; ++e) {
            const int idx = tid + 256 * e, kk = idx >> 6, c = idx & 63;
            const bool kin = k0 + kk < g.K;
            As[kk][c] = (kin && m0 + c < M) ? A[(long)(k0 + kk) * lda + m0 + c] : 0.f;
            Bs[kk][c] = (kin && n0 + c < N) ? Bm[(long)(k0 + kk) * ldb + n0 + c] : 0.f;
        }
        __syncthreads();
#pragma unroll
        for (int kk = 0; kk < 16; ++kk) {
            const f32x4 a = *reinterpret_cast<const f32x4*>(&As[kk][4 * ty]);
            const f32x4 b = *reinterpret_cast<const f32x4*>(&Bs[kk][4 * tx]);
#pragma unroll
            for (int i = 0; i < 4; ++i) {
                bsum[i] += a[i];
#pragma unroll
                for (int j = 0; j < 4; ++j) acc[i][j] = fmaf(a[i], b[j], acc[i][j]);
            }
        }
        __syncthreads();
    }
#pragma unroll
    for (int i = 0; i < 4; ++i) {
        const int m = m0 + 4 * ty + i;
        if (m >= M) continue;
        float* c = g.C[pi] + (long)m * g.ldc[pi] + n0 + 4 * tx;
#pragma unroll
        for (int j = 0; j < 4; ++j)
            if (n0 + 4 * tx + j < N) c[j] += acc[i][j];
        if (n0 == 0 && tx == 0 && g.bias[pi]) g.bias[pi][m] += bsum[i];
    }
}
}

extern "C" int arcvae_enc_heads_backward(const float* cond, const float* Wmu, const float* Wlh, const float* Wlv,
                                         const float* comb, const float* lh, const float* dmu_raw,
                                         const float* dlv_raw, float* dlh, float* dcomb, float* dWc, float* dbc,
                                         float* dWmu, float* dbmu, float* dWlh, float* dblh, float* dWlv,
                                         float* dblv, int B, int H, int Z, int C, int phase, hipStream_t stream) {
    if (!cond || !Wmu || !Wlh || !Wlv || !comb || !lh || !dmu_raw || !dlv_raw || !dlh || !dcomb || !dWc || !dbc ||
        !dWmu || !dbmu || !dWlh || !dblh || !dWlv || !dblv)
        return ARCVAE_ERR_ARG;
    if (phase < 0 || phase > 2) return ARCVAE_ERR_ARG;
    const int H2 = 2 * H;
    const int ACC = ARCVAE_GEMM_ACCUMULATE;
    int rc;
    if (phase == 0 || phase == 1) {
        const bool pair = B <= 256 && (Z % 64) == 0 && (reinterpret_cast<uintptr_t>(dmu_raw) & 15) == 0 &&
                          (reinterpret_cast<uintptr_t>(dlv_raw) & 15) == 0;
        if (pair) {
            const int M[2] = {B, B}, N[2] = {H2, H2}, K[2] = {Z, Z}, lda[2] = {Z, Z}, ldb[2] = {H2, H2}, ldc[2] = {H2, H2};
            const float* A[2] = {dmu_raw, dlv_raw};
            const float* Bm[2] = {Wmu, Wlv};
            float* Cm[2] = {dcomb, dlh};
            const float* bias[2] = {nullptr, lh};
            const int fl[2] = {0, ARCVAE_GEMM_DTANH};
            if ((rc = arcvae_gemm_skinny_pair(0, M, N, K, A, lda, Bm, ldb, Cm, ldc, bias, fl, stream))) return rc;
        } else {
        if ((rc = arcvae_gemm_f32(0, 0, B, H2, Z, dmu_raw, Z, Wmu, H2, dcomb, H2, nullptr, 0, stream))) return rc;
        if ((rc = arcvae_gemm_f32(0, 0, B, H2, Z, dlv_raw, Z, Wlv, H2, dlh, H2, lh, ARCVAE_GEMM_DTANH, stream)))
            return rc;
        }
        if ((rc = arcvae_gemm_f32(0, 0, B, H2, H2, dlh, H2, Wlh, H2, dcomb, H2, nullptr, ACC, stream))) return rc;
    }
    if ((phase == 0 || phase == 2) && arcvae_env_int("ARCVAE_HEADS_WGRAD_FUSED", 1) != 0) {
        HeadsWg g;
        const float* As_[4] = {dmu_raw, dlv_raw, dlh, dcomb + H};
        const float* Bs_[4] = {comb, lh, comb, cond};
        float* Cs_[4] = {dWmu, dWlv, dWlh, dWc};
        float* bs_[4] = {dbmu, dblv, dblh, dbc};
        const int Ms[4] = {Z, Z, H2, H}, Ns[4] = {H2, H2, H2, C}, la[4] = {Z, Z, H2, H2}, lb[4] = {H2, H2, H2, C > 0 ? C : 1},
                  lc[4] = {H2, H2, H2, C > 0 ? C : 1};
        int tiles = 0;
        for (int i = 0; i < 4; ++i) {
            g.A[i] = As_[i]; g.B[i] = Bs_[i]; g.C[i] = Cs_[i]; g.bias[i] = bs_[i];
            g.M[i] = Ms[i]; g.N[i] = Ns[i]; g.lda[i] = la[i]; g.ldb[i] = lb[i]; g.ldc[i] = lc[i];
            g.tile0[i] = tiles;
            tiles += ceil_div(Ms[i], 64) * (Ns[i] > 0 ? ceil_div(Ns[i], 64) : 1);
        }
        g.tile0[4] = tiles;
        g.K = B;
        hipLaunchKernelGGL(heads_wgrad_kernel, dim3(tiles), dim3(256), 0, stream, g);
        return arcvae_launch_status();
    }
    if (phase == 0 || phase == 2) {
        if ((rc = arcvae_gemm_f32(1, 0, Z, H2, B, dmu_raw, Z, comb, H2, dWmu, H2, nullptr, ACC, stream))) return rc;
        if ((rc = arcvae_colsum_accum(dmu_raw, B, Z, Z, dbmu, 1.0f, stream))) return rc;
        if ((rc = arcvae_gemm_f32(1, 0, Z, H2, B, dlv_raw, Z, lh, H2, dWlv, H2, nullptr, ACC, stream))) return rc;
        if ((rc = arcvae_colsum_accum(dlv_raw, B, Z, Z, dblv, 1.0f, stream))) return rc;
        if ((rc = arcvae_gemm_f32(1, 0, H2, H2, B, dlh, H2, comb, H2, dWlh, H2, nullptr, ACC, stream))) return rc;
        if ((rc = arcvae_colsum_accum(dlh, B, H2, H2, dblh, 1.0f, stream))) return rc;
        if (C > 0) {
            if ((rc = arcvae_gemm_f32(1, 0, H, C, B, dcomb + H, H2, cond, C, dWc, C, nullptr, ACC, stream))) return rc;
        }
        if ((rc = arcvae_colsum_accum(dcomb + H, B, H, H2, dbc, 1.0f, stream))) return rc;
    }
    return arcvae_launch_status();
}

namespace {
struct SeamArgs {
    const float *comb, *Wmu, *bmu, *Wlh, *blh, *Wlv, *blv, *eps, *hyper;
    float *lh, *mu_raw, *lv_raw, *mu, *logvar, *z, *stats, *scalars, *dmu_raw, *dlv_raw, *dlh, *dcomb;
    unsigned* sync;
    int B, H2, Z, T, RX, phases, launch;
    int dbg;
    float fb_min;
};
constexpr int SEAM_R = 8;

__device__ __forceinline__ bool seam_xcd_barrier(unsigned* my_flag, const unsigned* xflags, unsigned epoch, unsigned* err,
                                                 unsigned* s_ok) {
    const int tid = threadIdx.x, lane = tid & 63, wave = tid >> 6;
    ps_stores_in_l2();
    __syncthreads();
    if (tid == 0) __hip_atomic_store(my_flag, epoch, __ATOMIC_RELAXED, __HIP_MEMORY_SCOPE_WORKGROUP);
    if (wave == 1) {
        unsigned spins = 0;
        while (true) {
            const unsigned v = (lane < 32) ? __hip_atomic_load(xflags + lane, __ATOMIC_RELAXED, __HIP_MEMORY_SCOPE_AGENT) : epoch;
            if (__all((int)(v - epoch) >= 0)) break;
            if (++spins > 4000000u || __hip_atomic_load(err, __ATOMIC_RELAXED, __HIP_MEMORY_SCOPE_AGENT)) {
                if (lane == 0) { atomicAdd(err, 1u); *s_ok = 0; }
                break;
            }
            __builtin_amdgcn_s_sleep(1);
        }
    }
    __syncthreads();
    return *s_ok != 0;
}

__global__ __launch_bounds__(256) void enc_seam_kernel(SeamArgs a) {
    extern __shared__ __attribute__((aligned(16))) float sm[];
    __shared__ unsigned s_role, s_xcc, s_ok;
    __shared__ float s_red[8];
    const int tid = threadIdx.x, lane = tid & 63, wave = tid >> 6;
    const int B = a.B, H2 = a.H2, Z = a.Z, Zc = Z >> 5, Hc = H2 >> 5, LDW = H2 + 4, LDZ = Z + 4;
    unsigned* err = a.sync + PS_ERR;
    if (tid == 0) {
        s_xcc = ps_xcc_id();
        s_role = atomicAdd(a.sync + PSEAM_CNT + 8 * a.launch + (s_xcc & 7), 1u);
        s_ok = 1;
    }
    __syncthreads();
    const unsigned xcc = __builtin_amdgcn_readfirstlane(s_xcc), role = __builtin_amdgcn_readfirstlane(s_role);
    if (xcc >= 8 || role >= 32) {
        if (tid == 0) atomicAdd(err, 1u);
        return;
    }
    const int row0 = xcc * a.RX, RXl = max(0, min(a.RX, B - row0));
    unsigned* my_flag = a.sync + PSEAM + xcc * 32 + role;
    const unsigned* xflags = a.sync + PSEAM + xcc * 32;
    const bool fwd = (a.phases & 1) != 0, bwd = (a.phases & 2) != 0;
    float* wA = sm;
    float* wB = wA + (Zc + Hc) * LDW;
    float* wD = wB + Zc * LDW;
    float* wE1 = wD + Z * Hc;
    float* wE2 = wE1 + Z * Hc;
    float* act = wE2 + H2 * Hc;
    float* g1 = act + SEAM_R * LDW;
    float* g2 = g1 + SEAM_R * LDZ;
    float* mr = g2 + SEAM_R * LDZ;
    float* lhown = mr + SEAM_R * 8;
    const int q4 = H2 >> 2;
    if (fwd) {
        for (int i = tid; i < (Zc + Hc) * q4; i += 256) {
            const int r = i / q4, k4 = i - r * q4;
            const float* src = r < Zc ? a.Wmu + (long)(role * Zc + r) * H2 : a.Wlh + (long)(role * Hc + r - Zc) * H2;
            *reinterpret_cast<f32x4*>(wA + r * LDW + 4 * k4) = *reinterpret_cast<const f32x4*>(src + 4 * k4);
        }
        for (int i = tid; i < Zc * q4; i += 256) {
            const int r = i / q4, k4 = i - r * q4;
            *reinterpret_cast<f32x4*>(wB + r * LDW + 4 * k4) = *reinterpret_cast<const f32x4*>(a.Wlv + (long)(role * Zc + r) * H2 + 4 * k4);
        }
        for (int i = tid; i < RXl * q4; i += 256) {
            const int r = i / q4, k4 = i - r * q4;
            *reinterpret_cast<f32x4*>(act + r * LDW + 4 * k4) = *reinterpret_cast<const f32x4*>(a.comb + (long)(row0 + r) * H2 + 4 * k4);
        }
    }
    if (bwd) {
        const int c4 = Hc >> 2;
        for (int i = tid; i < Z * c4; i += 256) {
            const int j = i / c4, c = i - j * c4;
            *reinterpret_cast<f32x4*>(wD + j * Hc + 4 * c) = *reinterpret_cast<const f32x4*>(a.Wlv + (long)j * H2 + role * Hc + 4 * c);
            *reinterpret_cast<f32x4*>(wE1 + j * Hc + 4 * c) = *reinterpret_cast<const f32x4*>(a.Wmu + (long)j * H2 + role * Hc + 4 * c);
        }
        for (int i = tid; i < H2 * c4; i += 256) {
            const int k = i / c4, c = i - k * c4;
            *reinterpret_cast<f32x4*>(wE2 + k * Hc + 4 * c) = *reinterpret_cast<const f32x4*>(a.Wlh + (long)k * H2 + role * Hc + 4 * c);
        }
    }
    __syncthreads();
    if (a.dbg == 1) return;
    const int oB = tid >> 3, sB = tid & 7, iB = oB & 7, jq = oB >> 3;
    const bool ownB = sB == 0 && jq < Zc && iB < RXl;
    const int jcol = role * Zc + min(jq, Zc - 1);
    const int oD = tid >> 1, sD = tid & 1, iD = oD & 7, qD = oD >> 3;
    const bool actD = qD < Hc && iD < RXl;
    float m_v = 0.f, lv_v = 0.f;
    if (fwd) {
        if (tid < 8 * (Zc + Hc)) {
            const int i = tid & 7, c = tid >> 3;
            if (i < RXl) {
                const f32x4* w4 = reinterpret_cast<const f32x4*>(wA + c * LDW);
                const f32x4* x4 = reinterpret_cast<const f32x4*>(act + i * LDW);
                float a0 = 0.f, a1 = 0.f, a2 = 0.f, a3 = 0.f;
#pragma unroll 2
                for (int k = 0; k < q4; k += 4) {
                    const f32x4 w0 = w4[k], x0 = x4[k], w1 = w4[k + 1], x1 = x4[k + 1], w2 = w4[k + 2], x2 = x4[k + 2], w3 = w4[k + 3], x3 = x4[k + 3];
                    a0 = fmaf(x0[0], w0[0], a0); a0 = fmaf(x0[1], w0[1], a0); a0 = fmaf(x0[2], w0[2], a0); a0 = fmaf(x0[3], w0[3], a0);
                    a1 = fmaf(x1[0], w1[0], a1); a1 = fmaf(x1[1], w1[1], a1); a1 = fmaf(x1[2], w1[2], a1); a1 = fmaf(x1[3], w1[3], a1);
                    a2 = fmaf(x2[0], w2[0], a2); a2 = fmaf(x2[1], w2[1], a2); a2 = fmaf(x2[2], w2[2], a2); a2 = fmaf(x2[3], w2[3], a2);
                    a3 = fmaf(x3[0], w3[0], a3); a3 = fmaf(x3[1], w3[1], a3); a3 = fmaf(x3[2], w3[2], a3); a3 = fmaf(x3[3], w3[3], a3);
                }
                const float acc = (a0 + a1) + (a2 + a3);
// ... 362 lines not shown
```

### mlx-vae_amd/csrc/lstm.hip

```cpp
#include "ops.h"
#include "skinny.h"
#include "xcd.h"

namespace {

__device__ __forceinline__ int xcd_group_block(int x, int gx, int on) {
    return (on && (gx & 7) == 0) ? (x & 7) * (gx >> 3) + (x >> 3) : x;
}

struct FwdJob {
    const float* xin;
    const float* Wx;
    const float* hprev;
    const float* Wh;
    const float* pre;
    const int32_t* tok;
    const float* cprev;
    float* h;
    float* ht;
    float* c;
    float* gates;
    void* oct;
};
struct FwdArgs {
// ... 2024 lines not shown
    const unsigned* xflags = a.flags + xcc * 32;

    for (int s = a.s_begin; s < a.s_end; ++s) {
        const int skew = 2 * (LL - 1 - el);
        const int t = is_cell ? T - 1 - (s - skew) : T - 1 - (s + 1 - skew);
        const bool jact = slot < S && t >= 0 && t < T;
        float gi[MAXP], gf[MAXP], gg[MAXP], go[MAXP], c_v[MAXP], cprev_v[MAXP], ext_v[MAXP];
#pragma unroll
        for (int i = 0; i < MAXP; ++i) {
            gi[i] = gf[i] = gg[i] = go[i] = c_v[i] = cprev_v[i] = ext_v[i] = 0.f;
            const int p = p0 + 64 * i;
            const int erow = p / UW, ul = p - erow * UW;
            if (is_cell && jact && p < RX * UW && row0 + erow < B) {
                const int eb = row0 + erow, unit = role * UW + ul;
                const long hb = (long)eb * H + unit;
                const float* gp = a.gseq + el * lG + (long)t * sG + (long)eb * G + unit;
                gi[i] = gp[0]; gf[i] = gp[H]; gg[i] = gp[2 * H]; go[i] = gp[3 * H];
                c_v[i] = a.cseq[el * lH + (long)t * sH + hb];
                if (t > 0) cprev_v[i] = a.cseq[el * lH + (long)(t - 1) * sH + hb];
                if (el == LL - 1 && t == T - 1) ext_v[i] = a.dh_top[(long)eb * a.ld_dh_top + unit];
                if (s == a.s_begin) {
                    dcst[i] = (t < T - 1) ? a.dcs[((long)el * RS + ((t + 1) % RS)) * sH + hb] : 0.f;
                    if (el < LL - 1) ext_v[i] = a.dxs[((long)el * RS + (t % RS)) * sH + hb];
                }
            }
        }
        if (s > 0) {
            if (wave == 0) {
                unsigned spins = 0;
                while (true) {
                    const unsigned v = (lane < 32) ? __hip_atomic_load(xflags + lane, __ATOMIC_RELAXED, __HIP_MEMORY_SCOPE_AGENT)
                                                   : (unsigned)s;
                    if (__all((int)(v - (unsigned)s) >= 0)) break;
                    if (++spins > 4000000u || __hip_atomic_load(a.err, __ATOMIC_RELAXED, __HIP_MEMORY_SCOPE_AGENT)) {
                        if (lane == 0) { atomicAdd(a.err, 1u); s_ok = 0; }
                        break;
                    }
                    __builtin_amdgcn_s_sleep(1);
                }
            }
            __syncthreads();
            if (!s_ok) return;
        }
        if (tr) a.trace[2 * s] = wall_clock64();
        const float* srcp[S];
#pragma unroll
        for (int j = 0; j < S; ++j) {
            const bool cellj = j < LL;
            const int lj = cellj ? (LL - 1 - j) : (j - LL);
            const int skj = 2 * (LL - 1 - lj);
            const int tj = cellj ? T - 1 - (s - skj) : T - 1 - (s + 1 - skj);
            const float* pj = nullptr;
            if (tj >= 0 && tj < T) {
                if (cellj) { if (tj < T - 1) pj = a.dG + lj * lG + (long)(tj + 1) * sG; }
                else pj = a.dG + (lj + 1) * lG + (long)tj * sG;
            }
            srcp[j] = pj;
        }
        f32x4 fa[2][RT][CHP];
#define PB_LOAD(BUF, J, HALF)                                                                                  \
        if (srcp[J]) {                                                                                         \
            const __amdgpu_buffer_rsrc_t rs = ps_rsrc(srcp[J], sG * 4);                                        \
            _Pragma("unroll") for (int rt = 0; rt < RT; ++rt) {                                                \
                const unsigned off = (unsigned)(((long)arow[rt] * G + (wave * CHB + (HALF) * CHP) * 16 + q4) * 4); \
                _Pragma("unroll") for (int c = 0; c < CHP; ++c)                                                \
                    fa[BUF][rt][c] = ps_load_sc1_x4(rs, off + c * 64);                                         \
            }                                                                                                  \
        }
        PB_LOAD(0, 0, 0)
        f32x4 acc[RT];
#pragma unroll
        for (int k = 0; k < S * NH; ++k) {
            const int j = k / NH, h = k % NH;
            if (k + 1 < S * NH) { PB_LOAD((k + 1) & 1, (k + 1 < S * NH ? (k + 1) / NH : j), (k + 1) % NH) }
            if (h == 0) {
#pragma unroll
                for (int rt = 0; rt < RT; ++rt) acc[rt] = f32x4{0.f, 0.f, 0.f, 0.f};
            }
            if (srcp[j]) {
#pragma unroll
                for (int c = 0; c < CHP; ++c) {
                    const int kc = wave * CHB + h * CHP + c;
                    const f32x4 w = *reinterpret_cast<const f32x4*>(wl + ((j * NCHB + kc) * UW + ub) * 16 + q4);
#pragma unroll
                    for (int rt = 0; rt < RT; ++rt) {
                        acc[rt] = __builtin_amdgcn_mfma_f32_16x16x4f32(fa[k & 1][rt][c].x, w.x, acc[rt], 0, 0, 0);
                        acc[rt] = __builtin_amdgcn_mfma_f32_16x16x4f32(fa[k & 1][rt][c].y, w.y, acc[rt], 0, 0, 0);
                        acc[rt] = __builtin_amdgcn_mfma_f32_16x16x4f32(fa[k & 1][rt][c].z, w.z, acc[rt], 0, 0, 0);
                        acc[rt] = __builtin_amdgcn_mfma_f32_16x16x4f32(fa[k & 1][rt][c].w, w.w, acc[rt], 0, 0, 0);
                    }
                }
            }
            if (h == NH - 1) {
                float* rp = red + (wave * S + j) * 256 * RT;
#pragma unroll
                for (int rt = 0; rt < RT; ++rt)
#pragma unroll
                    for (int reg = 0; reg < 4; ++reg) rp[(16 * rt + (lane >> 4) * 4 + reg) * 16 + r] = acc[rt][reg];
            }
        }
#undef PB_LOAD
        __syncthreads();
        if (jact) {
#pragma unroll
            for (int i = 0; i < MAXP; ++i) {
                const int p = p0 + 64 * i;
                const int erow = p / UW, ul = p - erow * UW;
                if (p >= RX * UW || row0 + erow >= B) continue;
                const int eb = row0 + erow, unit = role * UW + ul;
                const long hb = (long)eb * H + unit;
                const int o = slot * 256 * RT + erow * 16 + ul;
                float dh = (red[o] + red[S * 256 * RT + o]) + (red[2 * S * 256 * RT + o] + red[3 * S * 256 * RT + o]);
                if (!is_cell) {
                    dxl[(((s + 1) & 1) * LL + el) * NP + p] = dh;
                    a.dxs[((long)el * RS + (t % RS)) * sH + hb] = dh;
                } else {
                    float ext = ext_v[i];
                    if (el < LL - 1 && s != a.s_begin) ext = dxl[((s & 1) * LL + el) * NP + p];
                    dh += ext;
                    const float tc = tanhf(c_v[i]);
                    const float d_o = dh * tc * go[i] * (1.f - go[i]);
                    const float dc = dh * go[i] * (1.f - tc * tc) + dcst[i];
                    const float d_i = dc * gg[i] * gi[i] * (1.f - gi[i]);
                    const float d_f = t > 0 ? dc * cprev_v[i] * gf[i] * (1.f - gf[i]) : 0.f;
                    const float d_g = dc * gi[i] * (1.f - gg[i] * gg[i]);
                    dcst[i] = dc * gf[i];
                    a.dcs[((long)el * RS + (t % RS)) * sH + hb] = dcst[i];
                    float* dp = a.dG + el * lG + (long)t * sG + (long)eb * G + unit;
                    dp[0] = d_i; dp[H] = d_f; dp[2 * H] = d_g; dp[3 * H] = d_o;
                }
            }
        }
        ps_stores_in_l2();
        __syncthreads();
        if (tid == 0) __hip_atomic_store(my_flag, (unsigned)(s + 1), __ATOMIC_RELAXED, __HIP_MEMORY_SCOPE_WORKGROUP);
        if (tr) a.trace[2 * s + 1] = wall_clock64();
    }
}


struct PersistRsArgs {
    PersistBwdArgs b;
    const float* W[3];
    float* part;
    const float* hseq;
    const int32_t* x_tb;
    float* dW[3];
    float* dbias1;
    float* dtable;
    int V;
    int fw_dbg;
    int parmask;
    unsigned* done;
};

template <int LL, bool WR, int MF, bool FW = false, int RG = 1, int NG = 1, bool SB = false>
__global__ __launch_bounds__(256, NG) void lstm_bwd_persist_rs_kernel(PersistRsArgs ar) {
    static_assert(MF == 0 || WR, "the 4x4x1 form keeps its weights in registers");
    static_assert(!FW || MF == 1, "fused weight gradients: 4x4x1 form only");
    static_assert(RG == 1 || (MF != 0 && !FW) || (MF == 0 && (RG == 2 || RG == 4) && WR && !FW), "row groups: 4x4 forms or 16-row tiles; weight gradients by GEMM");
    static_assert(NG == 1 || (MF == 0 && RG == 2), "two groups: the 16-row tile form");
    constexpr bool R16 = MF == 0 && RG >= 2;
    constexpr int NRT = R16 ? RG / 2 : 1;
    constexpr int DGL = LL * 16 * 32;
    const PersistBwdArgs& a = ar.b;
    constexpr int UW = 8, S = 2 * LL - 1, WS = 36;
    extern __shared__ __attribute__((aligned(16))) float lds[];
    float* wloc = lds;
    float* dgl = wloc + (WR ? 0 : S * 256 * WS);
    float* dxl = dgl + RG * DGL;
    float* dtl = dxl + RG * 128;
    __shared__ unsigned s_role, s_xcc, s_ok, s_grp;
    arcvae_set_prio(a.prio);
    const int tid = threadIdx.x, lane = tid & 63, wave = tid >> 6;
    const int B = a.B, T = a.T, H = a.H, G = 4 * a.H, RS = a.RS;
    if (tid == 0) {
        s_xcc = ps_xcc_id();
        unsigned g_, r_;
        ps_take_role<NG>(a.cnt, a.cucnt, s_xcc, g_, r_);
        s_grp = g_; s_role = r_;
        s_ok = 1;
        if (blockIdx.x == 0 && a.start_signal)
            __hip_atomic_fetch_add(a.start_signal, 1u, __ATOMIC_RELAXED, __HIP_MEMORY_SCOPE_AGENT);
    }
    __syncthreads();
    const unsigned xcc = __builtin_amdgcn_readfirstlane(s_xcc), role = __builtin_amdgcn_readfirstlane(s_role);
    const unsigned grp = NG == 1 ? 0u : __builtin_amdgcn_readfirstlane(s_grp);
    if (xcc >= 8 || role >= 32) {
        if (tid == 0) atomicAdd(a.err, 1u);
        return;
    }
    const int RX = NG == 1 ? a.RX : max(0, min(16, a.RX - 16 * (int)grp));
    const bool tr = a.trace && xcc == 0 && role == 0 && grp == 0 && tid == 0;
    const int r = lane & 15, q4 = (lane >> 4) * 4;
    f32x4 wr[(WR && !MF) ? S : 1][(WR && !MF) ? 4 : 1][(WR && !MF) ? 2 : 1];
    float wq[MF == 1 ? S : 1][MF == 1 ? 2 : 1][MF == 1 ? 32 : 1];
    s16x4_l wqb[MF == 2 ? S : 1][MF == 2 ? 2 : 1][MF == 2 ? 8 : 1];
    const int rg = lane >> 5, ug = (lane >> 2) & 7, ij = lane & 3;
    if constexpr (MF == 2) {
#pragma unroll
        for (int si = 0; si < S; ++si)
#pragma unroll
            for (int ch = 0; ch < 2; ++ch)
#pragma unroll
                for (int k4 = 0; k4 < 8; ++k4) {
                    f32x4 w;
#pragma unroll
                    for (int e = 0; e < 4; ++e) {
                        const int k = 4 * k4 + e;
                        w[e] = ar.W[si][(long)((k >> 3) * H + role * UW + (k & 7)) * H + 64 * wave + 32 * ch + 4 * ug + ij];
                    }
                    wqb[si][ch][k4] = pk4_bf16(w);
                }
    } else if constexpr (MF == 1) {
#pragma unroll
        for (int si = 0; si < S; ++si)
#pragma unroll
            for (int ch = 0; ch < 2; ++ch)
#pragma unroll
                for (int k = 0; k < 32; ++k)
                    wq[si][ch][k] = ar.W[si][(long)((k >> 3) * H + role * UW + (k & 7)) * H + 64 * wave + 32 * ch + 4 * ug + ij];
    } else if constexpr (WR) {
#pragma unroll
        for (int si = 0; si < S; ++si)
#pragma unroll
            for (int n = 0; n < 4; ++n)
#pragma unroll
                for (int c = 0; c < 2; ++c)
#pragma unroll
                    for (int e = 0; e < 4; ++e) {
                        const int k = 16 * c + q4 + e;
                        wr[si][n][c][e] = ar.W[si][(long)((k >> 3) * H + role * UW + (k & 7)) * H + 64 * wave + 16 * n + r];
                    }
    } else {
#pragma unroll
        for (int si = 0; si < S; ++si) {
            float wv[32];
#pragma unroll
            for (int k = 0; k < 32; ++k) wv[k] = ar.W[si][(long)((k >> 3) * H + role * UW + (k & 7)) * H + tid];
#pragma unroll
            for (int k = 0; k < 32; k += 4)
                *reinterpret_cast<f32x4*>(wloc + (si * 256 + tid) * WS + k) = f32x4{wv[k], wv[k + 1], wv[k + 2], wv[k + 3]};
        }
    }
    for (int i = tid; i < RG * DGL; i += 256) dgl[i] = 0.f;
    if constexpr (FW)
        for (int i = tid; i < ar.V * 33; i += 256) dtl[i] = 0.f;
    __syncthreads();
    const int row0 = a.row_base + (int)xcc * a.row_xs + 16 * (int)grp;
    const long sH = (long)B * H, sG = (long)B * G, lH = (long)T * sH, lG = (long)T * sG;
    auto dgl_row = [&](int g, int l, int rw) -> float* {
        return R16 ? dgl + (l * 16 * NRT + 8 * g + rw) * 32 : dgl + g * DGL + (l * 16 + rw) * 32;
    };
    constexpr int NQ = FW ? S : 1;
    f32x16 wacc[NQ][2];
    float wa[NQ][4], wb[NQ][4][2];
    float bsum[4] = {0.f, 0.f, 0.f, 0.f};
    bool wq_on[NQ];
    if constexpr (FW) {
#pragma unroll
        for (int q = 0; q < NQ; ++q) {
            wq_on[q] = false;
#pragma unroll
            for (int tl_ = 0; tl_ < 2; ++tl_)
#pragma unroll
                for (int g = 0; g < 16; ++g) wacc[q][tl_][g] = 0.f;
        }
    }
    auto wg_prepare = [&](int sp, int q_lo, int q_hi) {
        if constexpr (FW) {
#pragma unroll
            for (int q = 0; q < NQ; ++q) {
                if (q < q_lo || q >= q_hi) continue;
                const int lq = (q == 2) ? 0 : LL - 1;
                const int tq = T - 1 - (sp - 2 * (LL - 1 - lq));
                const int lh = (q == 1) ? 0 : lq;
                const int th = (q == 1) ? tq : tq - 1;
                wq_on[q] = tq >= 0 && tq < T && th >= 0;
                if (!wq_on[q]) continue;
                const float* hp = ar.hseq + lh * lH + (long)th * sH + 64 * wave + (lane & 31);
#pragma unroll
                for (int kk = 0; kk < 4; ++kk) {
                    const int row = 2 * kk + (lane >> 5);
                    wa[q][kk] = dgl[(lq * 16 + row) * 32 + (lane & 31)];
                    const bool rok = row < RX && row0 + row < B && !(ar.fw_dbg & 1);
                    const float* hr = hp + (long)min(row0 + row, B - 1) * H;
                    wb[q][kk][0] = rok ? hr[0] : 0.f;
                    wb[q][kk][1] = rok ? hr[32] : 0.f;
                }
            }
        }
    };
    auto wg_mfma = [&](int q) {
        if constexpr (FW) {
            if (q < NQ && wq_on[q < NQ ? q : 0] && !(ar.fw_dbg & 2)) {
                const int qq = q < NQ ? q : 0;
#pragma unroll
                for (int kk = 0; kk < 4; ++kk) {
                    wacc[qq][0] = __builtin_amdgcn_mfma_f32_32x32x2f32(wa[qq][kk], wb[qq][kk][0], wacc[qq][0], 0, 0, 0);
                    wacc[qq][1] = __builtin_amdgcn_mfma_f32_32x32x2f32(wa[qq][kk], wb[qq][kk][1], wacc[qq][1], 0, 0, 0);
                }
            }
        }
    };
    const int slot = tid >> 6, p = tid & 63;
    const bool is_cell = slot < LL;
    const int el = is_cell ? (LL - 1 - slot) : (slot - LL);
    const int erow = p >> 3, ul = p & 7;
    const int unit = role * UW + ul;
    bool eact[RG];
    int eb[RG];
    long hb[RG];
    float dcst[RG];
#pragma unroll
    for (int g = 0; g < RG; ++g) {
        eact[g] = slot < S && 8 * g + erow < RX && row0 + 8 * g + erow < B;
        eb[g] = min(row0 + 8 * g + erow, B - 1);
        hb[g] = (long)eb[g] * H + unit;
        dcst[g] = 0.f;
    }
    unsigned* my_flag = a.flags + (grp * 8 + xcc) * 32 + role;
    const unsigned* xflags = a.flags + (grp * 8 + xcc) * 32;
    const long part_src = (long)8 * 32 * 32 * 64;
    float* const part_grp = ar.part + (long)grp * RG * 2 * S * part_src;
    if constexpr (NG == 2) ps_stagger(grp, a.stagger);
    constexpr bool single = SB;
    unsigned* my_done = single ? ar.done + (grp * 8 + xcc) * 32 + role : nullptr;
    const unsigned* xdone = single ? ar.done + (grp * 8 + xcc) * 32 : nullptr;
    auto wait_gathered = [&](unsigned dv, int s) {
        unsigned spins = 0;
        while (!__all((int)(dv - (unsigned)s) >= 0)) {
            if (++spins > 4000000u || __hip_atomic_load(a.err, __ATOMIC_RELAXED, __HIP_MEMORY_SCOPE_AGENT)) {
                if (lane == 0) atomicAdd(a.err, 1u);
                break;
            }
            __builtin_amdgcn_s_sleep(1);
            dv = (lane < 32) ? __hip_atomic_load(xdone + lane, __ATOMIC_RELAXED, __HIP_MEMORY_SCOPE_AGENT) : (unsigned)s;
        }
    };

    for (int s = a.s_begin; s < a.s_end; ++s) {
        PS_STAMP(0);
        unsigned dv = (unsigned)s;
        if constexpr (SB) { if (lane < 32) dv = __hip_atomic_load(xdone + lane, __ATOMIC_RELAXED, __HIP_MEMORY_SCOPE_AGENT); }
        bool may_store = !SB;
        const int skew = 2 * (LL - 1 - el);
        const int t = is_cell ? T - 1 - (s - skew) : T - 1 - (s + 1 - skew);
        const bool jact = slot < S && t >= 0 && t < T;
        float gi[RG], gf[RG], gg[RG], go[RG], c_v[RG], cprev_v[RG], ext_v[RG];
        auto prefetch = [&]() {
#pragma unroll
            for (int g = 0; g < RG; ++g) {
                gi[g] = gf[g] = gg[g] = go[g] = c_v[g] = cprev_v[g] = ext_v[g] = 0.f;
                if (eact[g] && is_cell && jact) {
                    const float* gp = a.gseq + el * lG + (long)t * sG + (long)eb[g] * G + unit;
                    gi[g] = gp[0]; gf[g] = gp[H]; gg[g] = gp[2 * H]; go[g] = gp[3 * H];
                    c_v[g] = a.cseq[el * lH + (long)t * sH + hb[g]];
                    if (t > 0) cprev_v[g] = a.cseq[el * lH + (long)(t - 1) * sH + hb[g]];
                    if (el == LL - 1 && t == T - 1) ext_v[g] = a.dh_top[(long)eb[g] * a.ld_dh_top + unit];
                    if (s == a.s_begin) {
                        dcst[g] = (t < T - 1) ? a.dcs[((long)el * RS + ((t + 1) % RS)) * sH + hb[g]] : 0.f;
                        if (el < LL - 1) ext_v[g] = a.dxs[((long)el * RS + (t % RS)) * sH + hb[g]];
                    }
                }
            }
        };
#ifndef ARCVAE_RS_LATE_PREFETCH
#define ARCVAE_RS_LATE_PREFETCH 1
#endif
        if constexpr (ARCVAE_RS_LATE_PREFETCH == 0 || FW) prefetch();
        int tok = 0;
        if constexpr (FW) {
            if (eact[0] && is_cell && jact && el == 0) tok = min(max(ar.x_tb[(long)t * B + eb[0]], 0), ar.V - 1);
        }
        if (s == a.s_begin) {
            for (int i = tid; i < RG * LL * 8 * 32; i += 256) {
                const int g = i / (LL * 256), ig = i - g * (LL * 256);
                const int l = ig / 256, rem = ig - l * 256, rw = rem >> 5, k = rem & 31;
                const int tl_ = T - 1 - (s - 2 * (LL - 1 - l));
                float v = 0.f;
                if (tl_ + 1 >= 0 && tl_ + 1 < T && 8 * g + rw < RX && row0 + 8 * g + rw < B)
                    v = a.dG[l * lG + (long)(tl_ + 1) * sG + (long)(row0 + 8 * g + rw) * G + (k >> 3) * H + role * UW + (k & 7)];
                dgl_row(g, l, rw)[k] = v;
            }
            __syncthreads();
        }
        if (s > a.s_begin) wg_prepare(s - 1, 0, 2);
        PS_STAMP_START();
        float* pbase = part_grp + (long)(SB ? 0 : (s & 1)) * S * part_src + (long)xcc * 32 * 32 * 64;
#pragma unroll
        for (int g = 0; g < (R16 ? 1 : RG); ++g)
#pragma unroll
        for (int j = 0; j < S; ++j) {
            const bool cellj = j < LL;
            const int lj = cellj ? (LL - 1 - j) : (j - LL);
            const int skj = 2 * (LL - 1 - lj);
            const int tj = cellj ? T - 1 - (s - skj) : T - 1 - (s + 1 - skj);
            const bool actj = tj >= 0 && tj < T && (!cellj || tj < T - 1);
            const int ls = cellj ? lj : lj + 1;
            if constexpr (MF != 0) {
                float* pdst = pbase + (long)g * 2 * S * part_src + j * part_src + ((long)((64 * wave + 4 * ug) >> 3) * 32 + role) * 64 + (4 * rg + ij) * 8 + ((4 * ug) & 7);
// ... 398 lines not shown
        }
        if (tile_mt) {
            if (tile_mt == 44) launch_fwd_tile<4, 4>(a, B, H, nj, stream);
            else if (tile_mt == 4) launch_fwd_tile<4, 2>(a, B, H, nj, stream);
            else if (tile_mt == 2) launch_fwd_tile<2, 2>(a, B, H, nj, stream);
            else launch_fwd_tile<1, 2>(a, B, H, nj, stream);
            continue;
        }
        if (step2) {
            dim3 grid2(H / 8, ceil_div(B, 32), nj);
            DISPATCH_CH(H, launch_fwd2, a, grid2, stream)
            continue;
        }
        dim3 grid(H / 4, ceil_div(B, 16), nj);
        DISPATCH_CH(H, launch_fwd, a, grid, stream)
    }
    return arcvae_launch_status();
}


extern "C" int arcvae_enc_lstm_persistent_ok(int B, int T, int H, int L) { return persist_shape_ok(B, T, H, L) ? 1 : 0; }

extern "C" int arcvae_enc_lstm_forward_persistent(const int32_t* x_tb, const float* table0, const float* const* Wx,
                                                  const float* const* Wh, const float* const* bias, float* hseq,
                                                  float* cseq, float* gseq, float* wT_bwd, long wT_bwd_floats, float* comb,
                                                  unsigned* sync_ws, unsigned* start_signal, int B, int T, int V, int H,
                                                  int L, int flags, unsigned long long* trace, hipStream_t stream) {
    if (!x_tb || !table0 || !Wx || !Wh || !bias || !hseq || !cseq || !gseq || !sync_ws) return ARCVAE_ERR_ARG;
    if (V <= 0 || !persist_shape_ok(B, T, H, L)) return ARCVAE_ERR_ARG;
    if (wT_bwd) {
        long need[4];
        lstm_ws_need(B, T, H, L, flags, need);
        if (wT_bwd_floats < need[3]) return ARCVAE_ERR_ARG;
    }
    for (int l = 0; l < L; ++l)
        if (!Wh[l] || (l > 0 && (!Wx[l] || !bias[l]))) return ARCVAE_ERR_ARG;
    int rc;
    if (wT_bwd) {
        rc = tile_all_weights(Wx, Wh, nullptr, wT_bwd, H, L, 0,
                              bwd_split3(B, H, L, flags) ? 2 : (bwd_bf16(B, H, L, flags) ? 1 : 0), stream);
        if (rc != ARCVAE_OK) return rc;
    }
    if (!(flags & 1)) {
        rc = arcvae_zero(reinterpret_cast<float*>(sync_ws), 1, PS_WORDS, PS_WORDS, stream);
        if (rc != ARCVAE_OK) return rc;
        if (!(flags & ARCVAE_PERSIST_BF16) && persist_layer_split(B, H, L)) {
            rc = arcvae_zero(reinterpret_cast<float*>(sync_ws + PS_LS_FLAGS), 1, 256, 256, stream);
            if (rc != ARCVAE_OK) return rc;
        }
    }
    PersistArgs a;
    a.x_tb = x_tb; a.table0 = table0; a.hseq = hseq; a.cseq = cseq; a.gseq = gseq; a.comb = comb;
    for (int i = 0; i < 7; ++i) a.W[i] = Wh[0];
    for (int l = 0; l < L; ++l) { a.W[l] = Wh[l]; if (l > 0) a.W[L + l - 1] = Wx[l]; }
    for (int l = 0; l < ARCVAE_MAX_LAYERS; ++l) a.bias[l] = (l > 0 && l < L) ? bias[l] : nullptr;
    a.sync = sync_ws; a.start_signal = start_signal; a.trace = trace;
    a.flags = sync_ws + PS_FLAGS; a.cnt = sync_ws + PS_CNT; a.cucnt = nullptr; a.stagger = 0;
    a.B = B; a.T = T; a.H = H; a.V = V; a.RX = ceil_div(B, 8); a.prio = arcvae_step_prio();
    if (persist_two_groups(B, H, L, 1)) {
        if (!(flags & 1)) {
            rc = arcvae_zero(reinterpret_cast<float*>(sync_ws + PS2_FWD_FLAGS), 1, PS2_WORDS - PS2_FWD_FLAGS, PS2_WORDS - PS2_FWD_FLAGS, stream);
            if (rc != ARCVAE_OK) return rc;
        }
        a.flags = sync_ws + PS2_FWD_FLAGS; a.cnt = sync_ws + PS2_FWD_CNT;
        a.stagger = arcvae_env_int("ARCVAE_PERSIST2_STAGGER_FWD", 200);
        a.cucnt = arcvae_env_int("ARCVAE_PERSIST2_ASSIGN", 1) != 0 ? sync_ws + PS2_CU : nullptr;
        if (L == 1) launch_persist<2, 1, 1, 0, 2>(a, persist2_lds_bytes(), stream);
        else launch_persist<2, 2, 1, 0, 2>(a, persist2_lds_bytes(), stream);
        return arcvae_launch_status();
    }
    const size_t lds = persist_lds_bytes(B, H, L);
    const int NT = H / 128;
    const int RTn = persist_row_tiles(B);
#define PS_LAUNCH(N_, L_) do { if (RTn == 2) launch_persist<N_, L_, 2>(a, lds, stream); else launch_persist<N_, L_, 1>(a, lds, stream); } while (0)
#define PS_BY_L(N_) switch (L) { case 1: PS_LAUNCH(N_, 1); break; case 2: PS_LAUNCH(N_, 2); break; case 3: PS_LAUNCH(N_, 3); break; default: PS_LAUNCH(N_, 4); break; }
    if (NT == 2 && L <= 2 && a.RX <= 8 && arcvae_env_int("ARCVAE_FWD_MFMA", 1) != 0) {
        if (flags & ARCVAE_PERSIST_BF16) {
            if (L == 1) launch_persist<2, 1, 1, 2>(a, lds, stream); else launch_persist<2, 2, 1, 2>(a, lds, stream);
        } else if (persist_layer_split(B, H, L)) {
            launch_persist<2, 2, 1, 1, 1, 1>(a, lds > PS_LS_LDS ? lds : PS_LS_LDS, stream);
        } else {
            if (L == 1) launch_persist<2, 1, 1, 1>(a, lds, stream); else launch_persist<2, 2, 1, 1>(a, lds, stream);
        }
    } else if (NT == 1) { PS_BY_L(1) } else if (NT == 2) { PS_BY_L(2) } else { PS_BY_L(3) }
#undef PS_BY_L
#undef PS_LAUNCH
    return arcvae_launch_status();
}


extern "C" int arcvae_enc_lstm_bwd_persistent_ok(int B, int T, int H, int L) { return persist_bwd_shape_ok(B, T, H, L) ? 1 : 0; }

extern "C" int arcvae_enc_lstm_backward_persistent(const float* cseq, const float* gseq, const float* dh_top,
                                                   int ld_dh_top, float* dG, float* dcs, float* dxs, const float* wT,
                                                   unsigned* sync_ws, unsigned* start_signal, int B, int T, int H,
                                                   int L, int s_begin, int s_end, int chunk_index,
                                                   unsigned long long* trace, hipStream_t stream) {
    if (!cseq || !gseq || !dh_top || !dG || !dcs || !dxs || !wT || !sync_ws) return ARCVAE_ERR_ARG;
    if (!persist_bwd_shape_ok(B, T, H, L) || ld_dh_top < H) return ARCVAE_ERR_ARG;
    const int S = T + 2 * (L - 1);
    if (s_begin < 0 || s_end > S || s_begin >= s_end) return ARCVAE_ERR_ARG;
    if (chunk_index < 0 || chunk_index >= 8 || (chunk_index == 0) != (s_begin == 0)) return ARCVAE_ERR_ARG;
    if (chunk_index == 0) {
        const int rc = arcvae_zero(reinterpret_cast<float*>(sync_ws + PS_BWD), 1, PS_WORDS + 64, PS_WORDS + 64, stream);
        if (rc != ARCVAE_OK) return rc;
    }
    PersistBwdArgs a;
    a.wT = wT; a.cseq = cseq; a.gseq = gseq; a.dh_top = dh_top; a.dG = dG; a.dcs = dcs; a.dxs = dxs;
    a.sync = sync_ws + PS_BWD; a.err = sync_ws + PS_ERR; a.start_signal = start_signal; a.trace = trace;
    a.B = B; a.T = T; a.H = H; a.RX = ceil_div(B, 8); a.RS = arcvae_ring_slots(T); a.ld_dh_top = ld_dh_top;
    a.row_base = 0; a.row_xs = a.RX;
    a.s_begin = s_begin; a.s_end = s_end; a.prio = arcvae_step_prio();
    a.cnt_off = chunk_index == 0 ? 0 : (PS_WORDS - PS_CNT) + 8 * (chunk_index - 1);
    a.flags = a.sync + PS_FLAGS; a.cnt = a.sync + PS_CNT + a.cnt_off; a.cucnt = nullptr; a.stagger = 0;
    const size_t lds = persist_bwd_lds_bytes(B, H, L);
    const int NT = H / 128;
    const int RTn = persist_row_tiles(B);
#define PB_BY_L(N_)                                                                                          \
    if (RTn == 2) { if (L == 1) launch_persist_bwd<N_, 1, 2>(a, lds, stream); else launch_persist_bwd<N_, 2, 2>(a, lds, stream); } \
    else { if (L == 1) launch_persist_bwd<N_, 1, 1>(a, lds, stream); else launch_persist_bwd<N_, 2, 1>(a, lds, stream); }
    if (NT == 1) { PB_BY_L(1) } else if (NT == 2) { PB_BY_L(2) } else { PB_BY_L(3) }
#undef PB_BY_L
    return arcvae_launch_status();
}


extern "C" int arcvae_enc_lstm_bwd_rs_halves(int B, int T, int H, int L) {
    return (arcvae_env_int("ARCVAE_PERSIST", 1) != 0 && arcvae_env_int("ARCVAE_RS_HALVES", 0) != 0 && H == 256 && L >= 1 && L <= 2 &&
            B > 128 && B <= 256 && T >= 1 && !persist_two_groups(B, H, L, 2)) ? 1 : 0;
}
extern "C" int arcvae_enc_lstm_bwd_rs_ok(int B, int T, int H, int L) {
    return (arcvae_env_int("ARCVAE_PERSIST", 1) != 0 && H == 256 && L >= 1 && L <= 2 && B >= 1 &&
            (B <= arcvae_env_int("ARCVAE_RS_MAX_B", 128) || persist_two_groups(B, H, L, 2) ||
             arcvae_enc_lstm_bwd_rs_halves(B, T, H, L) == 1) && B <= 256 && T >= 1) ? 1 : 0;
}

static inline long bwd_rs_part_floats(int B, int H, int L) {
    const int rows_x = ceil_div(B, 8);
    const int rgn = persist_two_groups(B, H, L, 2) ? 4 : (rows_x <= 8 ? 1 : (rows_x <= 16 ? 2 : 4));
    return (long)rgn * 2 * (2 * L - 1) * 8 * 32 * 32 * 64;
}
extern "C" long arcvae_enc_lstm_bwd_rs_part_floats(int B, int T, int H, int L) {
    return arcvae_enc_lstm_bwd_rs_ok(B, T, H, L) == 1 ? bwd_rs_part_floats(B, H, L) : 0;
}

extern "C" int arcvae_enc_lstm_persist_groups(int B, int H, int L) {
    return (arcvae_env_int("ARCVAE_PERSIST", 1) != 0 && B > 0 && persist_two_groups(B, H, L, 3)) ? 2 : 1;
}

namespace {
struct FusedWgrad {
    const float* hseq; const int32_t* x_tb; float* const* dWx; float* const* dWh; float* const* dbias; float* dtable; int V;
};
int launch_bwd_rs(const float* const* Wx, const float* const* Wh, const float* cseq, const float* gseq,
                  const float* dh_top, int ld_dh_top, float* dG, float* dcs, float* dxs, float* part_ws, long part_ws_floats,
                  unsigned* sync_ws, unsigned* start_signal, int B, int T, int H, int L, int s_begin, int s_end,
                  int chunk_index, unsigned long long* trace, const FusedWgrad* fused, int flags, hipStream_t stream) {
    if (!Wx || !Wh || !cseq || !gseq || !dh_top || !dG || !dcs || !dxs || !part_ws || !sync_ws) return ARCVAE_ERR_ARG;
    if (H != 256 || L < 1 || L > 2 || B < 1 || B > 256 || T < 1 || ld_dh_top < H) return ARCVAE_ERR_ARG;
    if (arcvae_env_int("ARCVAE_PERSIST", 1) == 0) return ARCVAE_ERR_ARG;
    if (part_ws_floats < bwd_rs_part_floats(B, H, L)) return ARCVAE_ERR_ARG;
    const bool halves = (flags & ARCVAE_RS_HALF) != 0;
    const int half = (flags & ARCVAE_RS_HALF1) ? 1 : 0;
    if (halves && (fused || B <= 128 || (flags & ARCVAE_PERSIST_BF16))) return ARCVAE_ERR_ARG;
    const int rows_x = halves ? 16 : ceil_div(B, 8);
    const bool two = !halves && !fused && !(flags & ARCVAE_PERSIST_BF16) && persist_two_groups(B, H, L, 2);
    const int rgn = two ? 2 : (rows_x <= 8 ? 1 : (rows_x <= 16 ? 2 : 4));
    if (fused && rgn != 1) return ARCVAE_ERR_ARG;
    const int S = T + 2 * (L - 1);
    if (s_begin < 0 || s_end > S || s_begin >= s_end) return ARCVAE_ERR_ARG;
    if (chunk_index < 0 || chunk_index >= 8 || (chunk_index == 0) != (s_begin == 0)) return ARCVAE_ERR_ARG;
    const int bwd_base = (halves && half) ? PS2_BWD_FLAGS : PS_BWD;
    if (chunk_index == 0 && !(flags & 1)) {
        int rc = two ? arcvae_zero(reinterpret_cast<float*>(sync_ws + PS2_BWD_FLAGS), 1, PS2_CU - PS2_BWD_FLAGS, PS2_CU - PS2_BWD_FLAGS, stream)
                     : arcvae_zero(reinterpret_cast<float*>(sync_ws + bwd_base), 1, PS_WORDS + 64, PS_WORDS + 64, stream);
        if (rc == ARCVAE_OK) rc = arcvae_zero(reinterpret_cast<float*>(sync_ws + PS3_DONE), 1, 512, 512, stream);
        if (rc != ARCVAE_OK) return rc;
    }
    PersistRsArgs ar;
    PersistBwdArgs& a = ar.b;
    a.wT = nullptr; a.cseq = cseq; a.gseq = gseq; a.dh_top = dh_top; a.dG = dG; a.dcs = dcs; a.dxs = dxs;
    a.sync = sync_ws + bwd_base; a.err = sync_ws + PS_ERR; a.start_signal = start_signal; a.trace = trace;
    a.B = B; a.T = T; a.H = H; a.RX = rows_x; a.RS = arcvae_ring_slots(T); a.ld_dh_top = ld_dh_top;
    a.row_base = halves ? 16 * half : 0; a.row_xs = halves ? 32 : rows_x;
    a.s_begin = s_begin; a.s_end = s_end; a.prio = arcvae_step_prio();
    a.cnt_off = chunk_index == 0 ? 0 : (PS_WORDS - PS_CNT) + 8 * (chunk_index - 1);
    a.flags = a.sync + PS_FLAGS; a.cnt = a.sync + PS_CNT + a.cnt_off; a.cucnt = nullptr; a.stagger = 0;
    if (two) {
        a.stagger = arcvae_env_int("ARCVAE_PERSIST2_STAGGER_BWD", 200);
        a.flags = sync_ws + PS2_BWD_FLAGS; a.cnt = sync_ws + PS2_BWD_CNT + 16 * chunk_index;
        a.cucnt = arcvae_env_int("ARCVAE_PERSIST2_ASSIGN", 1) != 0 ? sync_ws + PS2_CU : nullptr;
    }
    if (L == 2) { ar.W[0] = Wh[1]; ar.W[1] = Wh[0]; ar.W[2] = Wx[1]; }
    else { ar.W[0] = Wh[0]; ar.W[1] = Wh[0]; ar.W[2] = Wh[0]; }
    for (int i = 0; i < 2 * L - 1; ++i) if (!ar.W[i]) return ARCVAE_ERR_ARG;
    ar.part = part_ws;
    ar.fw_dbg = arcvae_env_int("ARCVAE_FW_DEBUG", 0);
    const int single_env = arcvae_env_int("ARCVAE_RS_SINGLE", -1);
    const bool single = !fused && single_env != 0 && rows_x > 16;
    ar.parmask = single ? 0 : 1;
    ar.done = sync_ws + PS3_DONE;
    ar.hseq = nullptr; ar.x_tb = nullptr; ar.dW[0] = ar.dW[1] = ar.dW[2] = nullptr; ar.dbias1 = nullptr; ar.dtable = nullptr; ar.V = 0;
    if (fused) {
        if (!fused->hseq || !fused->x_tb || !fused->dWx || !fused->dWh || !fused->dbias || !fused->dtable || fused->V < 1 ||
            fused->V > 128)
            return ARCVAE_ERR_ARG;
        ar.hseq = fused->hseq; ar.x_tb = fused->x_tb; ar.dtable = fused->dtable; ar.V = fused->V;
        ar.dW[0] = fused->dWh[L - 1];
        if (L == 2) { ar.dW[1] = fused->dWx[1]; ar.dW[2] = fused->dWh[0]; ar.dbias1 = fused->dbias[1]; }
        else { ar.dW[1] = ar.dW[0]; ar.dW[2] = ar.dW[0]; }
        for (int i = 0; i < 2 * L - 1; ++i) if (!ar.dW[i]) return ARCVAE_ERR_ARG;
        if (L == 2 && !ar.dbias1) return ARCVAE_ERR_ARG;
        if (chunk_index == 0) {
            const int rc = arcvae_zero(fused->dtable, fused->V, 4 * H, 4 * H, stream);
            if (rc != ARCVAE_OK) return rc;
        }
    }
    const bool wreg = arcvae_env_int("ARCVAE_RS_WREG", 1) != 0 || fused || rgn > 1;
    size_t lds = sizeof(float) * ((wreg ? 0 : (size_t)(2 * L - 1) * 256 * 36) + (size_t)rgn * (L * 16 * 32 + 128) + (fused ? 128 * 33 : 0));
    if (lds < persist_lds_floor()) lds = persist_lds_floor();
    if (two) lds = persist2_lds_bytes();
    auto launch = [&](auto kern) {
        (void)hipFuncSetAttribute((const void*)kern, hipFuncAttributeMaxDynamicSharedMemorySize, 150 * 1024);
        hipLaunchKernelGGL(kern, dim3(two ? 512 : 256), dim3(256), lds, stream, ar);
    };
    if (two) {
        if (L == 1) launch(lstm_bwd_persist_rs_kernel<1, true, 0, false, 2, 2>); else launch(lstm_bwd_persist_rs_kernel<2, true, 0, false, 2, 2>);
        return arcvae_launch_status();
    }
    if (rgn >= 2 && !(flags & ARCVAE_PERSIST_BF16) && arcvae_env_int("ARCVAE_RS_R16", 1) != 0) {
        if (rgn == 4) {
            const size_t need = sizeof(float) * (size_t)rgn * (L * 16 * 32 + 128), kb = (size_t)arcvae_env_int("ARCVAE_RS_R32_LDS_KB", 0) * 1024;
            lds = need > kb ? need : kb;
        }
        if (rgn == 2) { if (L == 1) launch(lstm_bwd_persist_rs_kernel<1, true, 0, false, 2>); else launch(lstm_bwd_persist_rs_kernel<2, true, 0, false, 2>); }
        else if (single) { if (L == 1) launch(lstm_bwd_persist_rs_kernel<1, true, 0, false, 4, 1, true>); else launch(lstm_bwd_persist_rs_kernel<2, true, 0, false, 4, 1, true>); }
        else { if (L == 1) launch(lstm_bwd_persist_rs_kernel<1, true, 0, false, 4>); else launch(lstm_bwd_persist_rs_kernel<2, true, 0, false, 4>); }
        return arcvae_launch_status();
    }
    const bool mf = (wreg && arcvae_env_int("ARCVAE_RS_MFMA", 1) != 0) || fused || rgn > 1;
    if ((flags & ARCVAE_PERSIST_BF16) && mf && !fused && rgn <= 2) {
        if (rgn == 2) {
            if (L == 1) launch(lstm_bwd_persist_rs_kernel<1, true, 2, false, 2>); else launch(lstm_bwd_persist_rs_kernel<2, true, 2, false, 2>);
        } else {
            if (L == 1) launch(lstm_bwd_persist_rs_kernel<1, true, 2>); else launch(lstm_bwd_persist_rs_kernel<2, true, 2>);
        }
    } else
    if (rgn == 2) {
        if (L == 1) launch(lstm_bwd_persist_rs_kernel<1, true, 1, false, 2>); else launch(lstm_bwd_persist_rs_kernel<2, true, 1, false, 2>);
    } else if (rgn == 4) {
        if (L == 1) launch(lstm_bwd_persist_rs_kernel<1, true, 1, false, 4>); else launch(lstm_bwd_persist_rs_kernel<2, true, 1, false, 4>);
    } else if (L == 1) {
        if (fused) launch(lstm_bwd_persist_rs_kernel<1, true, 1, true>);
        else if (mf) launch(lstm_bwd_persist_rs_kernel<1, true, 1>);
        else if (wreg) launch(lstm_bwd_persist_rs_kernel<1, true, 0>);
        else launch(lstm_bwd_persist_rs_kernel<1, false, 0>);
    } else {
        if (fused) launch(lstm_bwd_persist_rs_kernel<2, true, 1, true>);
        else if (mf) launch(lstm_bwd_persist_rs_kernel<2, true, 1>);
        else if (wreg) launch(lstm_bwd_persist_rs_kernel<2, true, 0>);
        else launch(lstm_bwd_persist_rs_kernel<2, false, 0>);
    }
    return arcvae_launch_status();
}
}

extern "C" int arcvae_enc_lstm_backward_persistent_rs(const float* const* Wx, const float* const* Wh, const float* cseq,
                                                      const float* gseq, const float* dh_top, int ld_dh_top, float* dG,
                                                      float* dcs, float* dxs, float* part_ws, long part_ws_floats,
                                                      unsigned* sync_ws, unsigned* start_signal, int B, int T, int H, int L,
                                                      int s_begin, int s_end, int chunk_index, int flags,
                                                      unsigned long long* trace, hipStream_t stream) {
    return launch_bwd_rs(Wx, Wh, cseq, gseq, dh_top, ld_dh_top, dG, dcs, dxs, part_ws, part_ws_floats, sync_ws, start_signal, B, T, H, L,
                         s_begin, s_end, chunk_index, trace, nullptr, flags, stream);
}

extern "C" int arcvae_enc_lstm_backward_fused(const float* const* Wx, const float* const* Wh, const float* cseq,
                                              const float* gseq, const float* hseq, const int32_t* x_tb,
                                              const float* dh_top, int ld_dh_top, float* dG, float* dcs, float* dxs,
                                              float* part_ws, long part_ws_floats, unsigned* sync_ws, unsigned* start_signal,
                                              float* const* dWx, float* const* dWh, float* const* dbias,
                                              float* dtable_ws, int B, int T, int V, int H, int L, int s_begin, int s_end,
                                              int chunk_index, unsigned long long* trace, hipStream_t stream) {
    FusedWgrad f;
    f.hseq = hseq; f.x_tb = x_tb; f.dWx = dWx; f.dWh = dWh; f.dbias = dbias; f.dtable = dtable_ws; f.V = V;
    return launch_bwd_rs(Wx, Wh, cseq, gseq, dh_top, ld_dh_top, dG, dcs, dxs, part_ws, part_ws_floats, sync_ws, start_signal, B, T, H, L,
                         s_begin, s_end, chunk_index, trace, &f, 0, stream);
}

extern "C" int arcvae_enc_lstm_backward(const float* const* Wx, const float* const* Wh, const float* cseq,
                                        const float* gseq, const float* dh_top, int ld_dh_top, float* dG,
                                        float* dG_t, float* dcs, float* dxs, float* wT, int B, int T, int H,
                                        int L, int s_begin, int s_end, int flags, const long* ws_floats, void* dG_oct,
                                        unsigned* start_signal, unsigned long long* trace, hipStream_t stream) {
    const int retile = flags & ARCVAE_LSTM_RETILE;
    const bool b16 = bwd_bf16(B, H, L, flags), s3 = bwd_split3(B, H, L, flags);
    const bool oct = b16 && dG_oct && (B % 16) == 0;
    if (!Wx || !Wh || !cseq || !gseq || !dh_top || !dG || !dG_t || !dcs || !dxs || !wT || !ws_floats) return ARCVAE_ERR_ARG;
    if (B <= 0 || T <= 0 || L <= 0 || L > ARCVAE_MAX_LAYERS || !hidden_ok(H) || ld_dh_top < H)
        return ARCVAE_ERR_ARG;
    {
        long need[4];
        lstm_ws_need(B, T, H, L, flags, need);
        if (ws_floats[1] < need[1] || ws_floats[3] < need[3]) return ARCVAE_ERR_ARG;
    }
    const int S = T + 2 * (L - 1);
    if (s_begin < 0 || s_end > S || s_begin >= s_end) return ARCVAE_ERR_ARG;
    const long sH = (long)B * H, sG = (long)B * 4 * H;
    const long lH = (long)T * sH, lG = (long)T * sG;
    const long wsz = s3 ? (long)H * 4 * H * 3 / 2 : (long)H * 4 * H;
    const long sGt = s3 ? sG * 3 / 2 : sG;
    if (s_begin == 0 && retile) {
        const float* src[16];
        float* dst[16];
        int cols[16], mode[16];
        int n = 0;
        for (int l = 0; l < L; ++l) {
            if (!Wh[l] || (l > 0 && !Wx[l])) return ARCVAE_ERR_ARG;
            src[n] = Wh[l]; dst[n] = wT + l * wsz; cols[n] = H; mode[n] = s3 ? 5 : (b16 ? 3 : 1); ++n;
            if (l > 0) { src[n] = Wx[l]; dst[n] = wT + (L + l - 1) * wsz; cols[n] = H; mode[n] = s3 ? 5 : (b16 ? 3 : 1); ++n; }
        }
        const int rc = arcvae_tile_weights(src, dst, cols, mode, n, H, stream);
        if (rc != ARCVAE_OK) return rc;
    }
    const int tile_mt = bwd_tile_choice(B, H, L, flags);
    const bool step2 = !tile_mt && choose_step2(B);
    const int RS = arcvae_ring_slots(T), RSo = operand_ring_slots(B, T, H, L, flags);
    for (int s = s_begin; s < s_end; ++s) {
        BwdArgs a;
        a.B = B; a.H = H; a.prio = arcvae_step_prio(); a.remap = arcvae_xcd_remap() | (arcvae_env_int("ARCVAE_TILE_XCD", 0) != 0 ? 2 : 0); a.trace = trace ? trace + 2 * (long)s : nullptr;
        a.dbg = arcvae_env_int("ARCVAE_TILE_DEBUG", 0);
        a.signal = (s == s_begin) ? start_signal : nullptr;
        int nj = 0;
        for (int l = L - 1; l >= 0; --l) {
            const int skew = 2 * (L - 1 - l);
            const int t = T - 1 - (s - skew);
            if (t >= 0 && t < T) {
                BwdJob& j = a.job[nj++];
                const bool top = (l == L - 1), last = (t == T - 1);
                j.kind = 0;
                j.src = last ? nullptr : dG_t + ((long)l * RSo + ((t + 1) % RSo)) * sGt;
                j.WT = wT + l * wsz;
                if (top) { j.ext = last ? dh_top : nullptr; j.ext_ld = ld_dh_top; }
                else { j.ext = dxs + ((long)l * RS + (t % RS)) * sH; j.ext_ld = H; }
                j.gates = gseq + l * lG + t * sG;
                j.c = cseq + l * lH + t * sH;
                j.cprev = t > 0 ? cseq + l * lH + (t - 1) * sH : nullptr;
                j.dcin = last ? nullptr : dcs + ((long)l * RS + ((t + 1) % RS)) * sH;
                j.dcout = dcs + ((long)l * RS + (t % RS)) * sH;
                j.out = dG + l * lG + t * sG;
                j.outt = dG_t + ((long)l * RSo + (t % RSo)) * sGt;
                j.oct = oct ? static_cast<char*>(dG_oct) + 2 * (l * lG + t * sG) : nullptr;
            }
            const int tx = T - 1 - (s + 1 - skew);
            if (l < L - 1 && tx >= 0 && tx < T) {
                BwdJob& j = a.job[nj++];
                j.kind = 1;
                j.src = dG_t + ((long)(l + 1) * RSo + (tx % RSo)) * sGt;
                j.WT = wT + (L + l) * wsz;
                j.ext = nullptr; j.ext_ld = H;
                j.gates = nullptr; j.c = nullptr; j.cprev = nullptr; j.dcin = nullptr; j.dcout = nullptr;
                j.out = dxs + ((long)l * RS + (tx % RS)) * sH;
                j.outt = nullptr; j.oct = nullptr;
            }
        }
        if (nj == 0) continue;
        for (int k = nj; k < ARCVAE_MAX_BWD_JOBS; ++k) a.job[k] = a.job[0];
        if (tile_mt) {
            dim3 tgrid(ceil_div(H, 128), ceil_div(B, 16 * tile_mt), nj);
            if (b16 && tile_mt == 4 && arcvae_env_int("ARCVAE_BWD_KSPLIT", 1) != 0 && (H / 64) * ceil_div(B, 64) * nj >= 200) {
                if (arcvae_env_int("ARCVAE_BF16_KS_QUAD", 1) != 0 && (ld_dh_top % 4) == 0 && (reinterpret_cast<uintptr_t>(dh_top) % 16) == 0)
                    hipLaunchKernelGGL(lstm_bwd_tile_ks3_kernel<1>, dim3(H / 64, ceil_div(B, 64), nj), dim3(256), 64 * 1024, stream, a);
                else
                hipLaunchKernelGGL(lstm_bwd_tile_ks_kernel, dim3(H / 64, ceil_div(B, 64), nj), dim3(256), 48 * 1024, stream, a);
                continue;
            }
            if (s3) {
                const int ks3 = arcvae_env_int("ARCVAE_BWD_KSPLIT3", 1);
                if (ks3 != 0 && (ks3 == 2 || (H / 64) * ceil_div(B, 64) * nj >= tile_min_blocks(flags)) && (ld_dh_top % 4) == 0 &&
                    (reinterpret_cast<uintptr_t>(dh_top) % 16) == 0) {
                    hipLaunchKernelGGL(lstm_bwd_tile_ks3_kernel<2>, dim3(H / 64, ceil_div(B, 64), nj), dim3(256), 64 * 1024, stream, a);
                    continue;
                }
                if (tile_mt == 4) launch_bwd_tile<4, 2>(a, tgrid, stream);
                else if (tile_mt == 2) launch_bwd_tile<2, 2>(a, tgrid, stream);
                else launch_bwd_tile<1, 2>(a, tgrid, stream);
                continue;
            }
            if (b16) {
                if (tile_mt == 4) launch_bwd_tile<4, 1>(a, tgrid, stream);
                else if (tile_mt == 2) launch_bwd_tile<2, 1>(a, tgrid, stream);
                else launch_bwd_tile<1, 1>(a, tgrid, stream);
                continue;
            }
            if (tile_mt == 4) launch_bwd_tile<4>(a, tgrid, stream);
            else if (tile_mt == 2) launch_bwd_tile<2>(a, tgrid, stream);
            else launch_bwd_tile<1>(a, tgrid, stream);
            continue;
        }
        if (step2) {
            dim3 grid2(ceil_div(H, 32), ceil_div(B, 32), nj);
            if (s3) { DISPATCH_CH(H, launch_bwd2s, a, grid2, stream) }
            else { DISPATCH_CH(H, launch_bwd2, a, grid2, stream) }
            continue;
        }
        dim3 grid(H / 16, ceil_div(B, 16), nj);
        DISPATCH_CH(H, launch_bwd, a, grid, stream)
    }
    return arcvae_launch_status();
}

namespace {
__global__ __launch_bounds__(256) void planes_from_f32_kernel(const float* __restrict__ X, __bf16* __restrict__ P, long R, int H) {
    X += (long)blockIdx.y * R * H;
    P += (long)blockIdx.y * 3 * R * H;
    const long i = (long)blockIdx.x * 256 + threadIdx.x;
    const int hq = H >> 2;
    if (i >= R * hq) return;
    const long row = i / hq;
    const int unit = 4 * (int)(i - row * hq);
    const f32x4 v = *reinterpret_cast<const f32x4*>(X + row * H + unit);
    typedef __bf16 bf16x4_l __attribute__((ext_vector_type(4)));
    __bf16 pc[3][4];
#pragma unroll
    for (int k = 0; k < 4; ++k) split3_bf16(v[k], pc[0][k], pc[1][k], pc[2][k]);
    __bf16* tp = P + ((long)(unit >> 5) * R + row) * 32 + (unit & 31);
#pragma unroll
// ... 272 lines not shown
```

### mlx-vae_amd/csrc/misc.hip

```cpp
#include "ops.h"
#include <algorithm>

namespace {

__global__ __launch_bounds__(256) void colsum_kernel(const float* __restrict__ X, int rows, int cols,
                                                     int ld, float* out, float scale, int rows_per_blk) {
    __shared__ float red[4][64];
    const int cl = threadIdx.x & 63, rl = threadIdx.x >> 6;
    const int c = blockIdx.x * 64 + cl;
    const int rbeg = blockIdx.y * rows_per_blk, rend = min(rows, rbeg + rows_per_blk);
    float s = 0.f;
    if (c < cols)
        for (int r = rbeg + rl; r < rend; r += 4) s += X[(long)r * ld + c];
    red[rl][cl] = s;
    __syncthreads();
    if (rl == 0 && c < cols) {
        s = (red[0][cl] + red[1][cl]) + (red[2][cl] + red[3][cl]);
        atomicAdd(out + c, s * scale);
    }
}

struct TrJobs {
    const float* src[16];
    float* dst[16];
    int rows[16];
    int cols[16];
};
__global__ __launch_bounds__(256) void transpose_kernel(TrJobs j) {
    __shared__ float tile[32][33];
    const int z = blockIdx.z;
    const int R = j.rows[z], Cc = j.cols[z];
    const float* __restrict__ s = j.src[z];
    float* d = j.dst[z];
    const int tx = threadIdx.x & 31, ty = threadIdx.x >> 5;
    const int c0 = blockIdx.x * 32, r0 = blockIdx.y * 32;
    if (c0 >= Cc || r0 >= R) return;
#pragma unroll
    for (int i = 0; i < 32; i += 8) {
        const int r = r0 + ty + i, c = c0 + tx;
        if (r < R && c < Cc) tile[ty + i][tx] = s[(long)r * Cc + c];
    }
    __syncthreads();
#pragma unroll
    for (int i = 0; i < 32; i += 8) {
        const int c = c0 + ty + i, r = r0 + tx;
        if (r < R && c < Cc) d[(long)c * R + r] = tile[tx][ty + i];
    }
}

struct TileJobs {
    const float* src[16];
    float* dst[16];
    int cols[16];
    int mode[16];
};
__global__ __launch_bounds__(256) void tile_weights_kernel(TileJobs j, int H) {
    __shared__ float tile[16][65];
    const int z = blockIdx.y;
    const int K = j.cols[z];
    const float* __restrict__ src = j.src[z];
    float* dst = j.dst[z];
    const int tid = threadIdx.x;
    if (j.mode[z] == 0) {
        const long n4 = (long)4 * H * K / 4;
        const int k4n = K >> 2;
        for (long i = (long)blockIdx.x * 256 + tid; i < n4; i += (long)gridDim.x * 256) {
            const int r = (int)(i / k4n), k = (int)(i - (long)r * k4n) * 4;
            const int gate = r / H, unit = r - gate * H;
            const int rp = (unit >> 2) * 16 + gate * 4 + (unit & 3);
            *reinterpret_cast<float4*>(dst + ((long)(k >> 4) * 4 * H + rp) * 16 + (k & 15)) =
                *reinterpret_cast<const float4*>(src + (long)r * K + k);
        }
        return;
    }
    if (j.mode[z] == 4 || j.mode[z] == 5) {
        typedef float f2v __attribute__((ext_vector_type(2)));
        typedef __bf16 b2v __attribute__((ext_vector_type(2)));
        typedef unsigned u4v __attribute__((ext_vector_type(4)));
        auto bf = [](float x) { return __builtin_convertvector(f2v{x, 0.f}, b2v)[0]; };
        auto pk2 = [](__bf16 a, __bf16 b) { return __builtin_bit_cast(unsigned, b2v{a, b}); };
        __bf16* d16 = reinterpret_cast<__bf16*>(dst);
        const long n8 = (long)4 * H * K / 8, plane = (long)4 * H * K;
        const int k8n = K >> 3;
        for (long i = (long)blockIdx.x * 256 + tid; i < n8; i += (long)gridDim.x * 256) {
            float v[8];
            long off;
            if (j.mode[z] == 4) {
                const int r = (int)(i / k8n), k = (int)(i - (long)r * k8n) * 8;
                const int gate = r / H, unit = r - gate * H;
                const int rp = (unit >> 2) * 16 + gate * 4 + (unit & 3);
                const float4 a = *reinterpret_cast<const float4*>(src + (long)r * K + k);
                const float4 b = *reinterpret_cast<const float4*>(src + (long)r * K + k + 4);
                v[0] = a.x; v[1] = a.y; v[2] = a.z; v[3] = a.w; v[4] = b.x; v[5] = b.y; v[6] = b.z; v[7] = b.w;
                off = ((long)(k >> 5) * 4 * H + rp) * 32 + (k & 31);
            } else {
                const int g0 = (int)(i / K) * 8, k = (int)(i % K);
#pragma unroll
                for (int e = 0; e < 8; ++e) v[e] = src[(long)(g0 + e) * K + k];
                off = ((long)(g0 >> 5) * K + k) * 32 + (g0 & 31);
            }
            __bf16 p[3][8];
#pragma unroll
            for (int e = 0; e < 8; ++e) {
                p[0][e] = bf(v[e]);
                const float r1 = v[e] - (float)p[0][e];
                p[1][e] = bf(r1);
                p[2][e] = bf(r1 - (float)p[1][e]);
            }
#pragma unroll
            for (int q = 0; q < 3; ++q)
                *reinterpret_cast<u4v*>(d16 + q * plane + off) =
                    u4v{pk2(p[q][0], p[q][1]), pk2(p[q][2], p[q][3]), pk2(p[q][4], p[q][5]), pk2(p[q][6], p[q][7])};
        }
        return;
    }
    if (j.mode[z] == 2 || j.mode[z] == 3) {
        typedef float f2v __attribute__((ext_vector_type(2)));
        typedef __bf16 b2v __attribute__((ext_vector_type(2)));
        typedef unsigned u4v __attribute__((ext_vector_type(4)));
        auto pk = [](float a, float b) { return __builtin_bit_cast(unsigned, __builtin_convertvector(f2v{a, b}, b2v)); };
        __bf16* d16 = reinterpret_cast<__bf16*>(dst);
        const long n8 = (long)4 * H * K / 8;
        if (j.mode[z] == 2) {
            const int k8n = K >> 3;
            for (long i = (long)blockIdx.x * 256 + tid; i < n8; i += (long)gridDim.x * 256) {
                const int r = (int)(i / k8n), k = (int)(i - (long)r * k8n) * 8;
                const int gate = r / H, unit = r - gate * H;
                const int rp = (unit >> 2) * 16 + gate * 4 + (unit & 3);
                const float4 a = *reinterpret_cast<const float4*>(src + (long)r * K + k);
                const float4 b = *reinterpret_cast<const float4*>(src + (long)r * K + k + 4);
                *reinterpret_cast<u4v*>(d16 + ((long)(k >> 5) * 4 * H + rp) * 32 + (k & 31)) =
                    u4v{pk(a.x, a.y), pk(a.z, a.w), pk(b.x, b.y), pk(b.z, b.w)};
            }
        } else {
            for (long i = (long)blockIdx.x * 256 + tid; i < n8; i += (long)gridDim.x * 256) {
                const int g0 = (int)(i / K) * 8, k = (int)(i % K);
                float v[8];
#pragma unroll
                for (int e = 0; e < 8; ++e) v[e] = src[(long)(g0 + e) * K + k];
                *reinterpret_cast<u4v*>(d16 + ((long)(g0 >> 5) * K + k) * 32 + (g0 & 31)) =
                    u4v{pk(v[0], v[1]), pk(v[2], v[3]), pk(v[4], v[5]), pk(v[6], v[7])};
            }
        }
        return;
    }
    const int ktiles = K >> 6, ntiles = (4 * H / 16) * ktiles;
    for (int t = blockIdx.x; t < ntiles; t += gridDim.x) {
        const int R = t / ktiles, k0 = (t - R * ktiles) * 64;
        __syncthreads();
#pragma unroll
        for (int e = 0; e < 4; ++e) {
            const int rr = (tid >> 6) + 4 * e, kk = tid & 63;
            tile[rr][kk] = src[(long)(R * 16 + rr) * K + k0 + kk];
// ... 261 lines not shown
                for (int i = 0; i < 9; ++i) sc[i] = __builtin_nanf("");
                sc[15] = 1.0f;
            }
        }
    }
    if (tripped) return;
    if (DEV && !(lr >= 0.f && lr <= 3.402823466e+38f)) return;
    const long stride = (long)gridDim.x * blockDim.x;
    for (long i = (long)blockIdx.x * blockDim.x + threadIdx.x; i < n4; i += stride) {
        float4 pp = reinterpret_cast<float4*>(p)[i];
        const float4 gg = reinterpret_cast<const float4*>(g)[i];
        float4 mm = reinterpret_cast<float4*>(m)[i];
        float4 vv = reinterpret_cast<float4*>(v)[i];
#define ADAM1(c)                                   \
        mm.c = b1 * mm.c + omb1 * gg.c;            \
        vv.c = b2 * vv.c + omb2 * (gg.c * gg.c);   \
        pp.c = pp.c - (lr * mm.c) / (sqrtf(vv.c) + eps);
        ADAM1(x) ADAM1(y) ADAM1(z) ADAM1(w)
#undef ADAM1
        reinterpret_cast<float4*>(p)[i] = pp;
        reinterpret_cast<float4*>(m)[i] = mm;
        reinterpret_cast<float4*>(v)[i] = vv;
    }
    for (long i = n4 * 4 + (long)blockIdx.x * blockDim.x + threadIdx.x; i < n; i += stride) {
        const float gi = g[i];
        const float mi = b1 * m[i] + omb1 * gi;
        const float vi = b2 * v[i] + omb2 * (gi * gi);
        m[i] = mi;
        v[i] = vi;
        p[i] = p[i] - (lr * mi) / (sqrtf(vi) + eps);
    }
}

__global__ void zero2d_kernel(float* x, int rows, int cols, int ld) {
    const long n = (long)rows * cols;
    const long stride = (long)gridDim.x * blockDim.x;
    for (long i = (long)blockIdx.x * blockDim.x + threadIdx.x; i < n; i += stride) x[(i / cols) * ld + (i % cols)] = 0.f;
}

__global__ __launch_bounds__(64) void gate_wait_kernel(const unsigned* flag, unsigned* steps, unsigned stride,
                                                       unsigned offset, int advance, unsigned max_polls,
                                                       unsigned* err) {
    if (threadIdx.x != 0) return;
    const unsigned n = steps ? __hip_atomic_load(steps, __ATOMIC_RELAXED, __HIP_MEMORY_SCOPE_AGENT) : 0u;
    const unsigned target = n * stride + offset;
    bool ok = false;
    for (unsigned i = 0; i < max_polls; ++i) {
        const unsigned v = __hip_atomic_load(flag, __ATOMIC_RELAXED, __HIP_MEMORY_SCOPE_AGENT);
        if ((int)(v - target) >= 0) { ok = true; break; }
        __builtin_amdgcn_s_sleep(32);
    }
    if (!ok && err) atomicAdd(err, 1u);
    if (advance && steps) __hip_atomic_store(steps, n + 1u, __ATOMIC_RELAXED, __HIP_MEMORY_SCOPE_AGENT);
    __builtin_amdgcn_fence(__ATOMIC_ACQUIRE, "agent");
}
__global__ __launch_bounds__(64) void gate_set_kernel(unsigned* flag, unsigned value, int add) {
    if (threadIdx.x != 0) return;
    __builtin_amdgcn_fence(__ATOMIC_RELEASE, "agent");
    if (add) __hip_atomic_fetch_add(flag, value, __ATOMIC_RELAXED, __HIP_MEMORY_SCOPE_AGENT);
    else __hip_atomic_store(flag, value, __ATOMIC_RELAXED, __HIP_MEMORY_SCOPE_AGENT);
}

__global__ void scale_kernel(float* x, long n, float s) {
    const long stride = (long)gridDim.x * blockDim.x;
    for (long i = (long)blockIdx.x * blockDim.x + threadIdx.x; i < n; i += stride) x[i] *= s;
}

}

extern "C" int arcvae_colsum_accum(const float* X, int rows, int cols, int ld, float* out, float scale,
                                   hipStream_t stream) {
    if (!X || !out || rows <= 0 || cols <= 0 || ld < cols) return ARCVAE_ERR_ARG;
    int nchunks = min(ceil_div(rows, 64), 128);
    const int rpb = ceil_div(rows, nchunks);
    nchunks = ceil_div(rows, rpb);
    dim3 grid(ceil_div(cols, 64), nchunks);
    hipLaunchKernelGGL(colsum_kernel, grid, dim3(256), arcvae_side_lds_pad(1024), stream, X, rows, cols, ld, out, scale, rpb);
    return arcvae_launch_status();
}

extern "C" int arcvae_transpose_batched(const float* const* src, float* const* dst, const int* rows,
                                        const int* cols, int n, hipStream_t stream) {
    if (n <= 0 || n > 16) return ARCVAE_ERR_ARG;
    TrJobs j;
    int maxr = 0, maxc = 0;
    for (int i = 0; i < n; ++i) {
        if (!src[i] || !dst[i] || rows[i] <= 0 || cols[i] <= 0) return ARCVAE_ERR_ARG;
        j.src[i] = src[i]; j.dst[i] = dst[i]; j.rows[i] = rows[i]; j.cols[i] = cols[i];
        maxr = max(maxr, rows[i]); maxc = max(maxc, cols[i]);
    }
    for (int i = n; i < 16; ++i) { j.src[i] = nullptr; j.dst[i] = nullptr; j.rows[i] = 0; j.cols[i] = 0; }
    dim3 grid(ceil_div(maxc, 32), ceil_div(maxr, 32), n);
    hipLaunchKernelGGL(transpose_kernel, grid, dim3(256), 0, stream, j);
    return arcvae_launch_status();
}

extern "C" int arcvae_tile_weights(const float* const* src, float* const* dst, const int* cols, const int* mode,
                                   int n, int H, hipStream_t stream) {
    if (n <= 0 || n > 16 || H <= 0) return ARCVAE_ERR_ARG;
    TileJobs j;
    for (int i = 0; i < 16; ++i) {
        const int k = i < n ? i : 0;
        if (!src[k] || !dst[k] || cols[k] <= 0 || (cols[k] % 64) != 0) return ARCVAE_ERR_ARG;
        j.src[i] = src[k]; j.dst[i] = dst[k]; j.cols[i] = cols[k]; j.mode[i] = mode[k];
    }
    hipLaunchKernelGGL(tile_weights_kernel, dim3(256, n), dim3(256), 0, stream, j, H);
    return arcvae_launch_status();
}

extern "C" int arcvae_segsum_rows_accum(const float* X, const int32_t* seg, int rows, int nseg, int cols,
                                        float* out, hipStream_t stream) {
    if (!X || !seg || !out || rows <= 0 || nseg <= 0 || cols <= 0) return ARCVAE_ERR_ARG;
    const size_t lds = (size_t)nseg * 64 * sizeof(float);
    if (lds > 64 * 1024) return ARCVAE_ERR_ARG;
    dim3 grid(ceil_div(cols, 64), ceil_div(rows, 256));
    hipLaunchKernelGGL(segsum_kernel, grid, dim3(256), lds + arcvae_side_lds_pad((unsigned)lds), stream, X, seg, rows, nseg, cols, out);
    return arcvae_launch_status();
}

extern "C" int arcvae_table_finalize(const float* dT, const float* Wx0, int ldw, const float* emb, float* dEmb,
                                     float* dWx0, float* db0, int V, int E, int G, hipStream_t stream) {
    if (!dT || !Wx0 || !emb || !dEmb || !dWx0 || !db0) return ARCVAE_ERR_ARG;
    if (V <= 0 || E <= 0 || G <= 0 || (G % 16) != 0 || ldw < E) return ARCVAE_ERR_ARG;
    if ((G % TF_KS) != 0) return ARCVAE_ERR_ARG;
    const int etiles = ceil_div(E, 128);
    const int nA = ceil_div(V, TF_ROWS) * etiles * (G / TF_KS), nB = (G / 16) * ceil_div(E, 64), nC = ceil_div(G, 256);
    const size_t lds = sizeof(float) * (size_t)max(TF_KS * 128 + TF_ROWS * TF_KS + TF_ROWS * 128, 128 * 16 + 128 * 64);
    hipLaunchKernelGGL(table_finalize_kernel, dim3(nA + nB + nC), dim3(256), lds, stream, dT, Wx0, ldw, emb, dEmb, dWx0,
                       db0, V, E, G, nA, nB, etiles);
    return arcvae_launch_status();
}

extern "C" int arcvae_table_fold(const float* dT, const float* dT2, const float* Wx0, int ldw, const float* emb,
                                 float* dEmb, float* dWx0, float* db0, int V, int E, int G, int g_lo, int g_hi,
                                 hipStream_t stream) {
    if (!dT || !Wx0 || !emb || !dEmb || !dWx0 || !db0) return ARCVAE_ERR_ARG;
    if (V <= 0 || E <= 0 || G <= 0 || (G % 16) != 0 || ldw < E) return ARCVAE_ERR_ARG;
    if ((G % TF_KS) != 0) return ARCVAE_ERR_ARG;
    if (g_lo != 0 || g_hi != 0)
        if (g_lo < 0 || g_hi <= g_lo || g_hi > G || (g_lo % 32) != 0 || (g_hi % 32) != 0) return ARCVAE_ERR_ARG;
    if ((reinterpret_cast<uintptr_t>(dT) % 16) != 0 || (reinterpret_cast<uintptr_t>(dT2) % 16) != 0) return ARCVAE_ERR_ARG;
    const int etA = ceil_div(E, 16), etB = ceil_div(E, 32);
    const int nA = ceil_div(V, 16) * etA, nB = ceil_div((G / 32) * etB, 4);
    if (dT2)
        hipLaunchKernelGGL(table_fold_kernel<true>, dim3(nA + nB), dim3(256), 0, stream, dT, dT2, Wx0, ldw, emb, dEmb, dWx0,
                           db0, V, E, G, g_lo, g_hi, nA, etA, etB);
    else
        hipLaunchKernelGGL(table_fold_kernel<false>, dim3(nA + nB), dim3(256), 0, stream, dT, dT2, Wx0, ldw, emb, dEmb, dWx0,
                           db0, V, E, G, g_lo, g_hi, nA, etA, etB);
    return arcvae_launch_status();
}

namespace {
__global__ __launch_bounds__(256) void enc_prologue_kernel(const int32_t* __restrict__ x_bt, int32_t* x_tb, int B, int T,
                                                           float4* zero, long nz4, float4* zero2, long nz4b, unsigned* sync, int nsync, int keep,
                                                           const float* __restrict__ cond, const float* __restrict__ Wc,
                                                           const float* __restrict__ bc, float* comb, float* stats,
                                                           int nstats, int H, int C, float* onehot, int V, int Vp) {
    const long gt = (long)blockIdx.x * 256 + threadIdx.x, gs = (long)gridDim.x * 256;
    if (onehot) {
        const long n = (long)B * T * Vp;
        for (long i = gt; i < n; i += gs) {
            const int r = (int)(i / Vp), v = (int)(i - (long)r * Vp);
            const int t = r / B, bb = r - t * B;
            const int tk = min(max(x_bt[(long)bb * T + t], 0), V - 1);
            onehot[i] = (v == tk) ? 1.0f : 0.0f;
        }
    }
    if (comb) {
        for (long i = gt; i < (long)B * H; i += gs) {
            const int b = (int)(i / H), u = (int)(i - (long)b * H);
            float a = 0.f;
            for (int c = 0; c < C; ++c) a += cond[b * C + c] * Wc[u * C + c];
            comb[(long)b * 2 * H + H + u] = a + bc[u];
        }
        for (long i = gt; i < nstats; i += gs) stats[i] = 0.f;
    }
    for (long i = gt; i < (long)B * T; i += gs) {
        const int t = (int)(i / B), bb = (int)(i % B);
        x_tb[i] = x_bt[(long)bb * T + t];
    }
    for (long i = gt; i < nsync; i += gs)
        if (i != keep) sync[i] = 0u;
    const float4 z = make_float4(0.f, 0.f, 0.f, 0.f);
    for (long i = gt; i < nz4; i += gs) zero[i] = z;
    for (long i = gt; i < nz4b; i += gs) zero2[i] = z;
}
}

extern "C" int arcvae_enc_prologue(const int32_t* x_bt, int32_t* x_tb, float* zero_f32, long n_zero, float* zero2_f32,
                                   long n_zero2, unsigned* sync_ws, int n_sync, int sync_keep, const float* cond, const float* Wc, const float* bc, float* comb,
                                   float* stats, int n_stats, float* onehot_ws, int V, int B, int T, int H, int C,
                                   hipStream_t stream) {
    if (!x_bt || !x_tb || B <= 0 || T <= 0) return ARCVAE_ERR_ARG;
    if (onehot_ws && V <= 0) return ARCVAE_ERR_ARG;
    if (comb && (!cond || !Wc || !bc || !stats || n_stats <= 0 || H <= 0 || C < 0)) return ARCVAE_ERR_ARG;
    if (zero_f32 && ((n_zero % 4) != 0 || (reinterpret_cast<uintptr_t>(zero_f32) & 15) != 0)) return ARCVAE_ERR_ARG;
    if (zero2_f32 && ((n_zero2 % 4) != 0 || (reinterpret_cast<uintptr_t>(zero2_f32) & 15) != 0)) return ARCVAE_ERR_ARG;
    if (n_sync < 0 || (n_sync > 0 && !sync_ws)) return ARCVAE_ERR_ARG;
    hipLaunchKernelGGL(enc_prologue_kernel, dim3(256), dim3(256), 0, stream, x_bt, x_tb, B, T,
                       reinterpret_cast<float4*>(zero_f32), zero_f32 ? n_zero / 4 : 0L, reinterpret_cast<float4*>(zero2_f32),
                       zero2_f32 ? n_zero2 / 4 : 0L, sync_ws, n_sync, sync_keep, cond, Wc, bc, comb,
                       stats, n_stats, H, C, onehot_ws, V, (V + 3) & ~3);
    return arcvae_launch_status();
}

extern "C" int arcvae_transpose_tokens(const int32_t* src, int32_t* dst, int B, int T, hipStream_t stream) {
    if (!src || !dst || B <= 0 || T <= 0) return ARCVAE_ERR_ARG;
    hipLaunchKernelGGL(transpose_tokens_kernel, dim3(ceil_div(B * T, 256)), dim3(256), 0, stream, src, dst, B, T);
    return arcvae_launch_status();
}

namespace {
int launch_adam(float* params, const float* grads, float* m, float* v, long n, double lr, const float* lr_dev,
                       float* rate_out, double beta1, double beta2, double eps, const unsigned* guard_a,
                       const unsigned* guard_b, AdamFinalize fin, hipStream_t stream) {
    const uintptr_t al = reinterpret_cast<uintptr_t>(params) | reinterpret_cast<uintptr_t>(grads) |
                         reinterpret_cast<uintptr_t>(m) | reinterpret_cast<uintptr_t>(v);
    const long n4 = (al & 15) ? 0 : n / 4;
    const float omb1 = (float)(1.0 - beta1), omb2 = (float)(1.0 - beta2);
    const long work = n4 > 0 ? n4 : n;
    const int blocks = (int)min((long)2048, (work + 255) / 256);
    if (lr_dev)
        hipLaunchKernelGGL(adam_kernel<true>, dim3(blocks), dim3(256), 0, stream, params, grads, m, v, n4, n, 0.f, lr_dev,
                           rate_out, (float)beta1, (float)beta2, omb1, omb2, (float)eps, guard_a, guard_b, fin);
    else
        hipLaunchKernelGGL(adam_kernel<false>, dim3(blocks), dim3(256), 0, stream, params, grads, m, v, n4, n, (float)lr,
                           (const float*)nullptr, (float*)nullptr, (float)beta1, (float)beta2, omb1, omb2, (float)eps, guard_a,
                           guard_b, fin);
    return arcvae_launch_status();
}
}

int arcvae_adam_step_plain(float* params, const float* grads, float* m, float* v, long n, const float* lr_dev, double beta1,
                           double beta2, double eps, const unsigned* guard_a, const unsigned* guard_b, const float* rowloss,
                           int B, float* stats, float* scalars, int Z, int T, hipStream_t stream) {
    AdamFinalize fin;
    fin.rowloss = rowloss; fin.stats = stats; fin.scalars = scalars; fin.B = B; fin.Z = Z; fin.T = T;
    return launch_adam(params, grads, m, v, n, 0.0, lr_dev, scalars, beta1, beta2, eps, guard_a, guard_b, fin, stream);
}

extern "C" int arcvae_adam_update(float* params, const float* grads, float* m, float* v, long n,
                                  double lr, double beta1, double beta2, double eps, const unsigned* guard_a,
                                  const unsigned* guard_b, hipStream_t stream) {
    if (!params || !grads || !m || !v || n <= 0) return ARCVAE_ERR_ARG;
    AdamFinalize fin;
    fin.rowloss = nullptr; fin.stats = nullptr; fin.scalars = nullptr; fin.B = fin.Z = fin.T = 0;
    return launch_adam(params, grads, m, v, n, lr, nullptr, nullptr, beta1, beta2, eps, guard_a, guard_b, fin, stream);
}

extern "C" int arcvae_adam_update_finalize(float* params, const float* grads, float* m, float* v, long n, double lr,
                                           double beta1, double beta2, double eps, const unsigned* guard_a,
                                           const unsigned* guard_b, const float* rowloss, int B, float* stats, float* scalars,
                                           int Z, int T, hipStream_t stream) {
    if (!params || !grads || !m || !v || n <= 0 || !rowloss || !stats || !scalars || B <= 0 || Z <= 0 || T <= 0) return ARCVAE_ERR_ARG;
    AdamFinalize fin;
    fin.rowloss = rowloss; fin.stats = stats; fin.scalars = scalars; fin.B = B; fin.Z = Z; fin.T = T;
    return launch_adam(params, grads, m, v, n, lr, nullptr, nullptr, beta1, beta2, eps, guard_a, guard_b, fin, stream);
}

extern "C" int arcvae_zero(float* x, int rows, int cols, int ld, hipStream_t stream) {
    if (!x || rows <= 0 || cols <= 0 || ld < cols) return ARCVAE_ERR_ARG;
    const long n = (long)rows * cols;
    const int blocks = (int)min((long)1024, (n + 255) / 256);
    hipLaunchKernelGGL(zero2d_kernel, dim3(blocks), dim3(256), 0, stream, x, rows, cols, ld);
    return arcvae_launch_status();
}

extern "C" int arcvae_gate_wait(const unsigned* flag, unsigned* steps, unsigned stride, unsigned offset, int advance,
                                unsigned max_polls, unsigned* err, hipStream_t stream) {
    if (!flag || max_polls == 0) return ARCVAE_ERR_ARG;
    hipLaunchKernelGGL(gate_wait_kernel, dim3(1), dim3(64), 0, stream, flag, steps, stride, offset, advance,
                       max_polls, err);
    return arcvae_launch_status();
}
extern "C" int arcvae_gate_set(unsigned* flag, unsigned value, int add, hipStream_t stream) {
    if (!flag) return ARCVAE_ERR_ARG;
    hipLaunchKernelGGL(gate_set_kernel, dim3(1), dim3(64), 0, stream, flag, value, add);
    return arcvae_launch_status();
}

namespace {
__global__ void occupy_kernel(unsigned long long ticks, int lds_floats) {
    extern __shared__ float occ_lds[];
    for (int i = threadIdx.x; i < lds_floats; i += blockDim.x) occ_lds[i] = 0.f;
    const unsigned long long t0 = wall_clock64();
    while (wall_clock64() - t0 < ticks) __builtin_amdgcn_s_sleep(8);
}
}
extern "C" int arcvae_debug_occupy(int blocks, int threads, int lds_bytes, int spin_us, hipStream_t stream) {
    if (blocks <= 0 || blocks > 4096 || threads <= 0 || threads > 1024 || (threads % 64) != 0 || lds_bytes < 0 ||
        lds_bytes > 150 * 1024 || spin_us < 0 || spin_us > 100000)
        return ARCVAE_ERR_ARG;
    (void)hipFuncSetAttribute((const void*)occupy_kernel, hipFuncAttributeMaxDynamicSharedMemorySize, 150 * 1024);
    hipLaunchKernelGGL(occupy_kernel, dim3(blocks), dim3(threads), (size_t)lds_bytes, stream,
                       (unsigned long long)spin_us * 100ull, lds_bytes / 4);
    return arcvae_launch_status();
}

extern "C" int arcvae_scale_inplace(float* x, long n, float s, hipStream_t stream) {
    if (!x || n <= 0) return ARCVAE_ERR_ARG;
    const int blocks = (int)min((long)2048, (n + 255) / 256);
    hipLaunchKernelGGL(scale_kernel, dim3(blocks), dim3(256), 0, stream, x, n, s);
    return arcvae_launch_status();
}

extern "C" int arcvae_abi_version(int* arch_gfx950) {
    if (arch_gfx950) {
        int dev = 0;
        hipDeviceProp_t prop;
        *arch_gfx950 = 0;
        if (hipGetDevice(&dev) == hipSuccess && hipGetDeviceProperties(&prop, dev) == hipSuccess) {
            const char* a = prop.gcnArchName;
            *arch_gfx950 = (a[0] == 'g' && a[1] == 'f' && a[2] == 'x' && a[3] == '9' && a[4] == '5' && a[5] == '0') ? 1 : 0;
        }
    }
    return 1000;
}

namespace {
struct CopyJobs {
    const unsigned char* src[8];
    unsigned char* dst[8];
    long nbytes[8];
    int n;
};
__global__ __launch_bounds__(256) void copy_buffers_kernel(CopyJobs j) {
    const int i = blockIdx.y;
    if (i >= j.n) return;
    const unsigned char* s = j.src[i];
    unsigned char* d = j.dst[i];
    const long nb = j.nbytes[i];
    const long gt = (long)blockIdx.x * 256 + threadIdx.x, gs = (long)gridDim.x * 256;
    long done = 0;
    if (((reinterpret_cast<uintptr_t>(s) | reinterpret_cast<uintptr_t>(d)) & 15) == 0) {
        const long n16 = nb >> 4;
        for (long k = gt; k < n16; k += gs) reinterpret_cast<uint4*>(d)[k] = reinterpret_cast<const uint4*>(s)[k];
        done = n16 << 4;
    }
    for (long k = done + gt; k < nb; k += gs) d[k] = s[k];
}
}

extern "C" int arcvae_copy_buffers(const void* const* src, void* const* dst, const long* nbytes, int n, hipStream_t stream) {
    if (!src || !dst || !nbytes || n <= 0 || n > 8) return ARCVAE_ERR_ARG;
    CopyJobs j;
    j.n = n;
    long mx = 0;
    for (int i = 0; i < 8; ++i) {
        const int k = i < n ? i : 0;
        if (!src[k] || !dst[k] || nbytes[k] < 0) return ARCVAE_ERR_ARG;
        j.src[i] = static_cast<const unsigned char*>(src[k]); j.dst[i] = static_cast<unsigned char*>(dst[k]);
        j.nbytes[i] = nbytes[k];
        if (i < n && nbytes[k] > mx) mx = nbytes[k];
    }
    const int bx = (int)std::min<long>(64, std::max<long>(1, (mx / 16 + 255) / 256));
    hipLaunchKernelGGL(copy_buffers_kernel, dim3(bx, n), dim3(256), 0, stream, j);
// ... 3 lines not shown
```

Baseline: 72490.

## Fold table0 GEMM into encoder prologue and heads dcomb GEMM into BPTT seam

The encoder prologue kernel now also computes the layer-0 embedding×Wx input table with a skinny tiled reduction, which removes a separate GEMM launch. The first backward BPTT chunk kernel gains a 'seam rider' path that computes the dlh×Wlh contribution to dh_top in-kernel before the recurrence starts. The heads backward then skips that GEMM, doing only the remaining half later through new phases 3 and 4. This cuts kernel launches and serialization on the critical path, at the cost of more complexity, extra registers and shared memory in the persistent kernel, and restrictive shape guards.

```diff
diff --git a/include/arcvae_hip.h b/include/arcvae_hip.h
--- a/include/arcvae_hip.h
+++ b/include/arcvae_hip.h
@@ -76,6 +76,11 @@
                         unsigned* sync_ws, int n_sync, int sync_keep ,
                         const float* cond, const float* Wc, const float* bc, float* comb, float* stats, int n_stats,
                         float* onehot_ws, int V, int B, int T, int H, int C, arcvae_stream_t stream);
+int arcvae_enc_prologue_table0(const int32_t* x_bt, int32_t* x_tb, float* zero_f32, long n_zero, float* zero2_f32, long n_zero2,
+                               unsigned* sync_ws, int n_sync, int sync_keep, const float* cond, const float* Wc, const float* bc,
+                               float* comb, float* stats, int n_stats, float* onehot_ws, int V, int B, int T, int H, int C,
+                               const float* emb, const float* Wx0, const float* bias0, float* table0, int E, int G,
+                               arcvae_stream_t stream);
 int arcvae_enc_lstm_bwd_persistent_ok(int B, int T, int H, int L);
 int arcvae_enc_lstm_backward_persistent(const float* cseq, const float* gseq, const float* dh_top, int ld_dh_top,
                                         float* dG, float* dcs, float* dxs, const float* wT, unsigned* sync_ws,
@@ -92,6 +97,12 @@
                                            int flags ,
                                            unsigned long long* trace,
                                            arcvae_stream_t stream);
+int arcvae_enc_lstm_backward_persistent_rs_seam(const float* const* Wx, const float* const* Wh, const float* cseq,
+                                                const float* gseq, float* dh_top, int ld_dh_top, float* dG, float* dcs,
+                                                float* dxs, float* part_ws, long part_ws_floats, unsigned* sync_ws,
+                                                unsigned* start_signal, int B, int T, int H, int L, int s_begin, int s_end,
+                                                int chunk_index, int flags, unsigned long long* trace, const float* add_A, int lda,
+                                                const float* add_W, int ldw, int add_K, arcvae_stream_t stream);
 int arcvae_enc_lstm_backward_fused(const float* const* Wx, const float* const* Wh, const float* cseq, const float* gseq,
                                    const float* hseq, const int32_t* x_tb, const float* dh_top, int ld_dh_top,
                                    float* dG, float* dcs, float* dxs, float* part_ws, long part_ws_floats, unsigned* sync_ws,
diff --git a/mlx-vae_amd/arcvae_hip/_lib.py b/mlx-vae_amd/arcvae_hip/_lib.py
--- a/mlx-vae_amd/arcvae_hip/_lib.py
+++ b/mlx-vae_amd/arcvae_hip/_lib.py
@@ -55,6 +55,8 @@
     "arcvae_enc_lstm_persistent_ok": [_i, _i, _i, _i],
     "arcvae_enc_lstm_forward_persistent": [_vp, _vp, _pp, _pp, _pp, _vp, _vp, _vp, _vp, _l, _vp, _vp, _vp, _i, _i, _i, _i, _i, _i, _vp, _vp],
     "arcvae_enc_prologue": [_vp, _vp, _vp, _l, _vp, _l, _vp, _i, _i, _vp, _vp, _vp, _vp, _vp, _i, _vp, _i, _i, _i, _i, _i, _vp],
+    "arcvae_enc_prologue_table0": [_vp, _vp, _vp, _l, _vp, _l, _vp, _i, _i, _vp, _vp, _vp, _vp, _vp, _i, _vp, _i, _i, _i, _i, _i,
+                                   _vp, _vp, _vp, _vp, _i, _i, _vp],
     "arcvae_enc_lstm_bwd_persistent_ok": [_i, _i, _i, _i],
     "arcvae_enc_lstm_backward_persistent": [_vp, _vp, _vp, _i, _vp, _vp, _vp, _vp, _vp, _vp, _i, _i, _i, _i, _i, _i, _i, _vp, _vp],
     "arcvae_enc_lstm_bwd_rs_ok": [_i, _i, _i, _i],
@@ -62,6 +64,8 @@
     "arcvae_enc_lstm_persist_groups": [_i, _i, _i],
     "arcvae_enc_lstm_bwd_rs_part_floats": [_i, _i, _i, _i],
     "arcvae_enc_lstm_backward_persistent_rs": [_pp, _pp, _vp, _vp, _vp, _i, _vp, _vp, _vp, _vp, _l, _vp, _vp, _i, _i, _i, _i, _i, _i, _i, _i, _vp, _vp],
+    "arcvae_enc_lstm_backward_persistent_rs_seam": [_pp, _pp, _vp, _vp, _vp, _i, _vp, _vp, _vp, _vp, _l, _vp, _vp, _i, _i, _i, _i, _i, _i,
+                                                    _i, _i, _vp, _vp, _i, _vp, _i, _i, _vp],
     "arcvae_enc_lstm_backward_fused": [_pp, _pp, _vp, _vp, _vp, _vp, _vp, _i, _vp, _vp, _vp, _vp, _l, _vp, _vp, _pp, _pp, _pp, _vp,
                                        _i, _i, _i, _i, _i, _i, _i, _i, _vp, _vp],
     "arcvae_enc_lstm_backward": [_pp, _pp, _vp, _vp, _vp, _i, _vp, _vp, _vp, _vp, _vp, _i, _i, _i, _i, _i, _i, _i, _lp, _vp, _vp, _vp, _vp],
diff --git a/mlx-vae_amd/arcvae_hip/engine.py b/mlx-vae_amd/arcvae_hip/engine.py
--- a/mlx-vae_amd/arcvae_hip/engine.py
+++ b/mlx-vae_amd/arcvae_hip/engine.py
@@ -181,6 +181,20 @@
         ws.seam_bwd_done = True
 
 
+SEAM_FOLD_DEFAULT = "3"
+
+
+def seam_fold() -> int:
+    return int(os.environ.get("ARCVAE_SEAM_FOLD", SEAM_FOLD_DEFAULT))
+
+
+def _env_on(name: str) -> bool:
+    try:
+        return int(os.environ.get(name, "1")) != 0
+    except ValueError:
+        return False
+
+
 def encoder_forward(enc: ParamStore, ws: Workspace, d: ModelDims, free_bits: float,
                     start_signal: Optional[C.c_void_p] = None, zero_grad: bool = False, seam: int = 1) -> None:
     B, T = ws.B, ws.T
@@ -194,13 +208,19 @@
         tabs = ws.dtables if (zero_grad and hasattr(ws, "dtables")) else None
         ws.tables_zeroed = tabs is not None
         ws.bptt_rearmed = True
-        call("arcvae_enc_prologue", ptr(ws.x), ptr(ws.x_tb), ptr(grad), C.c_long(grad.numel() if grad is not None else 0),
-             ptr(tabs), C.c_long(tabs.numel() if tabs is not None else 0), ptr(ws.psync), ws.psync_words, 500, ptr(ws.cond), ptr(enc.p("condition_fc.weight")), ptr(enc.p("condition_fc.bias")),
-             ptr(ws.comb), ptr(ws.stats), 2 * d.Z + 4, ptr(ws.onehot) if (zero_grad and hasattr(ws, "onehot")) else C.c_void_p(0),
-             d.V, B, T, d.H, d.C, s)
+        emb, wx0 = enc.p("embedding.weight"), enc.p("lstm_layer_0.Wx")
+        table0_in = bool(seam_fold() & 2) and B <= 64 and not getattr(ws, "bf16", False) and d.V <= 256 and d.E % 64 == 0 and emb.data_ptr() % 16 == 0 and wx0.data_ptr() % 16 == 0
+        pro = (ptr(ws.x), ptr(ws.x_tb), ptr(grad), C.c_long(grad.numel() if grad is not None else 0),
+               ptr(tabs), C.c_long(tabs.numel() if tabs is not None else 0), ptr(ws.psync), ws.psync_words, 500, ptr(ws.cond), ptr(enc.p("condition_fc.weight")), ptr(enc.p("condition_fc.bias")),
+               ptr(ws.comb), ptr(ws.stats), 2 * d.Z + 4, ptr(ws.onehot) if (zero_grad and hasattr(ws, "onehot")) else C.c_void_p(0),
+               d.V, B, T, d.H, d.C)
         comb_ready = 1
-        call("arcvae_gemm_f32", 0, 1, d.V, G, d.E, ptr(enc.p("embedding.weight")), d.E,
-             ptr(enc.p("lstm_layer_0.Wx")), d.E, ptr(ws.table0), G, ptr(enc.p("lstm_layer_0.bias")), 0, s)
+        if table0_in:
+            call("arcvae_enc_prologue_table0", *pro, ptr(emb), ptr(wx0), ptr(enc.p("lstm_layer_0.bias")), ptr(ws.table0), d.E, G, s)
+        else:
+            call("arcvae_enc_prologue", *pro, s)
+            call("arcvae_gemm_f32", 0, 1, d.V, G, d.E, ptr(emb), d.E, ptr(wx0), d.E, ptr(ws.table0), G,
+                 ptr(enc.p("lstm_layer_0.bias")), 0, s)
         need_wT = hasattr(ws, "wT") and not bptt_reduce_scatter_ok(ws, d)
         call("arcvae_enc_lstm_forward_persistent", ptr(ws.x_tb), ptr(ws.table0), wx, wh, bs, ptr(ws.hseq),
              ptr(ws.cseq), ptr(ws.gseq), ptr(ws.wT) if need_wT else C.c_void_p(0), C.c_long(ws.wT.numel() if need_wT else 0),
@@ -458,6 +478,8 @@
         self._dwh = _layer_ptrs(enc, L, "Wh", grad=True)
         self._dbs = _layer_ptrs(enc, L, "bias", grad=True)
         self.chunks = self.chunk_schedule(T, L, self.FRACTIONS)
+        self._seam_rider = False
+        self._heads_cond_half = False
 
     @staticmethod
     def chunk_schedule(T: int, L: int, fractions) -> list:
@@ -478,6 +500,15 @@
             if phase == 1:
                 return
             phase = 2
+        elif (phase == 1 and (seam_fold() & 1) and self.persistent and not self.fused and ws.B <= 64
+              and not getattr(ws, "bf16", False)
+              and _env_on("ARCVAE_RS_WREG") and _env_on("ARCVAE_RS_MFMA")):
+            phase = 3
+            self._seam_rider = self._heads_cond_half = True
+        elif phase in (0, 1):
+            self._seam_rider = self._heads_cond_half = False
+        elif phase == 2 and self._heads_cond_half:
+            phase = 4
         call("arcvae_enc_heads_backward", ptr(ws.cond), ptr(enc.p("fc_mu.weight")),
              ptr(enc.p("fc_logvar_hidden.weight")), ptr(enc.p("fc_logvar.weight")), ptr(ws.comb), ptr(ws.lh),
              ptr(ws.dmu_raw), ptr(ws.dlv_raw), ptr(ws.dlh), ptr(ws.dcomb), ptr(enc.g("condition_fc.weight")),
@@ -500,6 +531,14 @@
             return
         if self.persistent:
             halves = _lib.load().arcvae_enc_lstm_bwd_rs_halves(ws.B, ws.T, d.H, d.L) == 1
+            if self._seam_rider and chunk_index == 0:
+                self._seam_rider = False
+                call("arcvae_enc_lstm_backward_persistent_rs_seam", self._wx[0], self._wh[0], ptr(ws.cseq), ptr(ws.gseq),
+                     ptr(ws.dcomb), 2 * d.H, ptr(ws.dG), ptr(ws.dcs), ptr(ws.dxs), ptr(ws.ppart), C.c_long(ws.ppart.numel()), ptr(ws.psync),
+                     sig, ws.B, ws.T, d.H, d.L, s0, s1, chunk_index, (_lib.PERSIST_BF16 if ws.bf16_parts & 1 else 0) | rearmed,
+                     ptr(ws.trace_bwd), ptr(ws.dlh), 2 * d.H, ptr(self.enc.p("fc_logvar_hidden.weight")), 2 * d.H, 2 * d.H,
+                     stream_ptr())
+                return
             for hf in ((_lib.RS_HALF, _lib.RS_HALF | _lib.RS_HALF1) if halves else (0,)):
                 call("arcvae_enc_lstm_backward_persistent_rs", self._wx[0], self._wh[0], ptr(ws.cseq), ptr(ws.gseq),
                      ptr(ws.dcomb), 2 * d.H, ptr(ws.dG), ptr(ws.dcs), ptr(ws.dxs), ptr(ws.ppart), C.c_long(ws.ppart.numel()), ptr(ws.psync),
diff --git a/mlx-vae_amd/csrc/latent.hip b/mlx-vae_amd/csrc/latent.hip
--- a/mlx-vae_amd/csrc/latent.hip
+++ b/mlx-vae_amd/csrc/latent.hip
@@ -419,10 +419,16 @@
     if (!cond || !Wmu || !Wlh || !Wlv || !comb || !lh || !dmu_raw || !dlv_raw || !dlh || !dcomb || !dWc || !dbc ||
         !dWmu || !dbmu || !dWlh || !dblh || !dWlv || !dblv)
         return ARCVAE_ERR_ARG;
-    if (phase < 0 || phase > 2) return ARCVAE_ERR_ARG;
+    if (phase < 0 || phase > 4) return ARCVAE_ERR_ARG;
     const int H2 = 2 * H;
     const int ACC = ARCVAE_GEMM_ACCUMULATE;
     int rc;
+    const bool chain_only = phase == 3;
+    if (phase == 4) {
+        if ((rc = arcvae_gemm_f32(0, 0, B, H, H2, dlh, H2, Wlh + H, H2, dcomb + H, H2, nullptr, ACC, stream))) return rc;
+        phase = 2;
+    }
+    if (phase == 3) phase = 1;
     if (phase == 0 || phase == 1) {
         const bool pair = B <= 256 && (Z % 64) == 0 && (reinterpret_cast<uintptr_t>(dmu_raw) & 15) == 0 &&
                           (reinterpret_cast<uintptr_t>(dlv_raw) & 15) == 0;
@@ -439,7 +445,9 @@
         if ((rc = arcvae_gemm_f32(0, 0, B, H2, Z, dlv_raw, Z, Wlv, H2, dlh, H2, lh, ARCVAE_GEMM_DTANH, stream)))
             return rc;
         }
-        if ((rc = arcvae_gemm_f32(0, 0, B, H2, H2, dlh, H2, Wlh, H2, dcomb, H2, nullptr, ACC, stream))) return rc;
+        if (!chain_only) {
+            if ((rc = arcvae_gemm_f32(0, 0, B, H2, H2, dlh, H2, Wlh, H2, dcomb, H2, nullptr, ACC, stream))) return rc;
+        }
     }
     if ((phase == 0 || phase == 2) && arcvae_env_int("ARCVAE_HEADS_WGRAD_FUSED", 1) != 0) {
         HeadsWg g;
diff --git a/mlx-vae_amd/csrc/lstm.hip b/mlx-vae_amd/csrc/lstm.hip
--- a/mlx-vae_amd/csrc/lstm.hip
+++ b/mlx-vae_amd/csrc/lstm.hip
@@ -2200,10 +2200,17 @@
     int fw_dbg;
     int parmask;
     unsigned* done;
+    const float* add_A;
+    const float* add_W;
+    float* dh_top_w;
+    int add_lda, add_ldw;
 };
-
-template <int LL, bool WR, int MF, bool FW = false, int RG = 1, int NG = 1, bool SB = false>
+constexpr int RS_SEAM_K = 512;
+constexpr int RS_SEAM_FLOATS = 8 * RS_SEAM_K + 4 * 64;
+
+template <int LL, bool WR, int MF, bool FW = false, int RG = 1, int NG = 1, bool SB = false, bool SM = false>
 __global__ __launch_bounds__(256, NG) void lstm_bwd_persist_rs_kernel(PersistRsArgs ar) {
+    static_assert(!SM || (RG == 1 && NG == 1 && !FW), "the seam rider: one-row-group forms, weight gradients by GEMM");
     static_assert(MF == 0 || WR, "the 4x4x1 form keeps its weights in registers");
     static_assert(!FW || MF == 1, "fused weight gradients: 4x4x1 form only");
     static_assert(RG == 1 || (MF != 0 && !FW) || (MF == 0 && (RG == 2 || RG == 4) && WR && !FW), "row groups: 4x4 forms or 16-row tiles; weight gradients by GEMM");
@@ -2240,6 +2247,24 @@
     }
     const int RX = NG == 1 ? a.RX : max(0, min(16, a.RX - 16 * (int)grp));
     const bool tr = a.trace && xcc == 0 && role == 0 && grp == 0 && tid == 0;
+    float* sma = dxl + RG * 128;
+    float* smr = sma + 8 * RS_SEAM_K;
+    const int srow0 = a.row_base + (int)xcc * a.row_xs;
+    f32x4 sa[SM ? 4 : 1];
+    float sw[SM ? 16 : 1], sold = 0.f;
+    if constexpr (SM) {
+        const int rw = tid >> 5;
+        const bool rok = rw < RX && srow0 + rw < B;
+        const float* ap = ar.add_A + (long)min(srow0 + rw, B - 1) * ar.add_lda + 4 * (tid & 31);
+#pragma unroll
+        for (int i = 0; i < 4; ++i)
+            sa[i] = rok ? *reinterpret_cast<const f32x4*>(ap + 128 * i) : f32x4{0.f, 0.f, 0.f, 0.f};
+        const float* wp = ar.add_W + (long)(16 * (tid >> 3)) * ar.add_ldw + role * 8 + (tid & 7);
+#pragma unroll
+        for (int i = 0; i < 16; ++i) sw[i] = wp[(long)i * ar.add_ldw];
+        if (tid < 64 && (tid >> 3) < RX && srow0 + (tid >> 3) < B)
+            sold = ar.dh_top_w[(long)(srow0 + (tid >> 3)) * a.ld_dh_top + role * 8 + (tid & 7)];
+    }
     const int r = lane & 15, q4 = (lane >> 4) * 4;
     f32x4 wr[(WR && !MF) ? S : 1][(WR && !MF) ? 4 : 1][(WR && !MF) ? 2 : 1];
     float wq[MF == 1 ? S : 1][MF == 1 ? 2 : 1][MF == 1 ? 32 : 1];
@@ -2294,7 +2319,40 @@
     for (int i = tid; i < RG * DGL; i += 256) dgl[i] = 0.f;
     if constexpr (FW)
         for (int i = tid; i < ar.V * 33; i += 256) dtl[i] = 0.f;
+    if constexpr (SM) {
+#pragma unroll
+        for (int i = 0; i < 4; ++i) *reinterpret_cast<f32x4*>(sma + (tid >> 5) * RS_SEAM_K + 4 * (tid & 31) + 128 * i) = sa[i];
+    }
     __syncthreads();
+    if constexpr (SM) {
+        float sacc[8];
+#pragma unroll
+        for (int rw = 0; rw < 8; ++rw) {
+            sacc[rw] = 0.f;
+#pragma unroll
+            for (int j = 0; j < 4; ++j) {
+                const f32x4 av = *reinterpret_cast<const f32x4*>(sma + rw * RS_SEAM_K + 16 * (tid >> 3) + 4 * j);
+                sacc[rw] = fmaf(av.x, sw[4 * j], sacc[rw]);
+                sacc[rw] = fmaf(av.y, sw[4 * j + 1], sacc[rw]);
+                sacc[rw] = fmaf(av.z, sw[4 * j + 2], sacc[rw]);
+                sacc[rw] = fmaf(av.w, sw[4 * j + 3], sacc[rw]);
+            }
+        }
+#pragma unroll
+        for (int rw = 0; rw < 8; ++rw) {
+            sacc[rw] += __shfl_xor(sacc[rw], 8);
+            sacc[rw] += __shfl_xor(sacc[rw], 16);
+            sacc[rw] += __shfl_xor(sacc[rw], 32);
+        }
+        if (lane < 8) {
+#pragma unroll
+            for (int rw = 0; rw < 8; ++rw) smr[wave * 64 + rw * 8 + lane] = sacc[rw];
+        }
+        __syncthreads();
+        if (tid < 64 && (tid >> 3) < RX && srow0 + (tid >> 3) < B)
+            ar.dh_top_w[(long)(srow0 + (tid >> 3)) * a.ld_dh_top + role * 8 + (tid & 7)] =
+                sold + ((smr[tid] + smr[64 + tid]) + (smr[128 + tid] + smr[192 + tid]));
+    }
     const int row0 = a.row_base + (int)xcc * a.row_xs + 16 * (int)grp;
     const long sH = (long)B * H, sG = (long)B * G, lH = (long)T * sH, lG = (long)T * sG;
     auto dgl_row = [&](int g, int l, int rw) -> float* {
@@ -2999,10 +3057,14 @@
 struct FusedWgrad {
     const float* hseq; const int32_t* x_tb; float* const* dWx; float* const* dWh; float* const* dbias; float* dtable; int V;
 };
+struct SeamAdd {
+    const float* A; int lda; const float* W; int ldw; int K;
+};
 int launch_bwd_rs(const float* const* Wx, const float* const* Wh, const float* cseq, const float* gseq,
                   const float* dh_top, int ld_dh_top, float* dG, float* dcs, float* dxs, float* part_ws, long part_ws_floats,
                   unsigned* sync_ws, unsigned* start_signal, int B, int T, int H, int L, int s_begin, int s_end,
-                  int chunk_index, unsigned long long* trace, const FusedWgrad* fused, int flags, hipStream_t stream) {
+                  int chunk_index, unsigned long long* trace, const FusedWgrad* fused, int flags, hipStream_t stream,
+                  const SeamAdd* seam = nullptr) {
     if (!Wx || !Wh || !cseq || !gseq || !dh_top || !dG || !dcs || !dxs || !part_ws || !sync_ws) return ARCVAE_ERR_ARG;
     if (H != 256 || L < 1 || L > 2 || B < 1 || B > 256 || T < 1 || ld_dh_top < H) return ARCVAE_ERR_ARG;
     if (arcvae_env_int("ARCVAE_PERSIST", 1) == 0) return ARCVAE_ERR_ARG;
@@ -3017,6 +3079,10 @@
     const int S = T + 2 * (L - 1);
     if (s_begin < 0 || s_end > S || s_begin >= s_end) return ARCVAE_ERR_ARG;
     if (chunk_index < 0 || chunk_index >= 8 || (chunk_index == 0) != (s_begin == 0)) return ARCVAE_ERR_ARG;
+    if (seam && (chunk_index != 0 || halves || two || rgn != 1 || fused || (flags & ARCVAE_PERSIST_BF16) || !seam->A || !seam->W || seam->K != RS_SEAM_K ||
+                 seam->lda < seam->K || (seam->lda % 4) != 0 || (reinterpret_cast<uintptr_t>(seam->A) & 15) != 0 || seam->ldw < H))
+        return ARCVAE_ERR_ARG;
+    if (seam && (arcvae_env_int("ARCVAE_RS_WREG", 1) == 0 || arcvae_env_int("ARCVAE_RS_MFMA", 1) == 0)) return ARCVAE_ERR_ARG;
     const int bwd_base = (halves && half) ? PS2_BWD_FLAGS : PS_BWD;
     if (chunk_index == 0 && !(flags & 1)) {
         int rc = two ? arcvae_zero(reinterpret_cast<float*>(sync_ws + PS2_BWD_FLAGS), 1, PS2_CU - PS2_BWD_FLAGS, PS2_CU - PS2_BWD_FLAGS, stream)
@@ -3048,6 +3114,8 @@
     ar.parmask = single ? 0 : 1;
     ar.done = sync_ws + PS3_DONE;
     ar.hseq = nullptr; ar.x_tb = nullptr; ar.dW[0] = ar.dW[1] = ar.dW[2] = nullptr; ar.dbias1 = nullptr; ar.dtable = nullptr; ar.V = 0;
+    ar.add_A = seam ? seam->A : nullptr; ar.add_W = seam ? seam->W : nullptr; ar.dh_top_w = seam ? const_cast<float*>(dh_top) : nullptr;
+    ar.add_lda = seam ? seam->lda : 0; ar.add_ldw = seam ? seam->ldw : 0;
     if (fused) {
         if (!fused->hseq || !fused->x_tb || !fused->dWx || !fused->dWh || !fused->dbias || !fused->dtable || fused->V < 1 ||
             fused->V > 128)
@@ -3064,7 +3132,8 @@
         }
     }
     const bool wreg = arcvae_env_int("ARCVAE_RS_WREG", 1) != 0 || fused || rgn > 1;
-    size_t lds = sizeof(float) * ((wreg ? 0 : (size_t)(2 * L - 1) * 256 * 36) + (size_t)rgn * (L * 16 * 32 + 128) + (fused ? 128 * 33 : 0));
+    size_t lds = sizeof(float) * ((wreg ? 0 : (size_t)(2 * L - 1) * 256 * 36) + (size_t)rgn * (L * 16 * 32 + 128) + (fused ? 128 * 33 : 0) +
+                                  (seam ? RS_SEAM_FLOATS : 0));
     if (lds < persist_lds_floor()) lds = persist_lds_floor();
     if (two) lds = persist2_lds_bytes();
     auto launch = [&](auto kern) {
@@ -3097,6 +3166,9 @@
         if (L == 1) launch(lstm_bwd_persist_rs_kernel<1, true, 1, false, 2>); else launch(lstm_bwd_persist_rs_kernel<2, true, 1, false, 2>);
     } else if (rgn == 4) {
         if (L == 1) launch(lstm_bwd_persist_rs_kernel<1, true, 1, false, 4>); else launch(lstm_bwd_persist_rs_kernel<2, true, 1, false, 4>);
+    } else if (seam) {
+        if (L == 1) launch(lstm_bwd_persist_rs_kernel<1, true, 1, false, 1, 1, false, true>);
+        else launch(lstm_bwd_persist_rs_kernel<2, true, 1, false, 1, 1, false, true>);
     } else if (L == 1) {
         if (fused) launch(lstm_bwd_persist_rs_kernel<1, true, 1, true>);
         else if (mf) launch(lstm_bwd_persist_rs_kernel<1, true, 1>);
@@ -3120,6 +3192,18 @@
                                                       unsigned long long* trace, hipStream_t stream) {
     return launch_bwd_rs(Wx, Wh, cseq, gseq, dh_top, ld_dh_top, dG, dcs, dxs, part_ws, part_ws_floats, sync_ws, start_signal, B, T, H, L,
                          s_begin, s_end, chunk_index, trace, nullptr, flags, stream);
+}
+
+extern "C" int arcvae_enc_lstm_backward_persistent_rs_seam(const float* const* Wx, const float* const* Wh, const float* cseq,
+                                                           const float* gseq, float* dh_top, int ld_dh_top, float* dG,
+                                                           float* dcs, float* dxs, float* part_ws, long part_ws_floats,
+                                                           unsigned* sync_ws, unsigned* start_signal, int B, int T, int H, int L,
+                                                           int s_begin, int s_end, int chunk_index, int flags,
+                                                           unsigned long long* trace, const float* add_A, int lda,
+                                                           const float* add_W, int ldw, int add_K, hipStream_t stream) {
+    const SeamAdd seam{add_A, lda, add_W, ldw, add_K};
+    return launch_bwd_rs(Wx, Wh, cseq, gseq, dh_top, ld_dh_top, dG, dcs, dxs, part_ws, part_ws_floats, sync_ws, start_signal, B, T, H, L,
+                         s_begin, s_end, chunk_index, trace, nullptr, flags, stream, &seam);
 }
 
 extern "C" int arcvae_enc_lstm_backward_fused(const float* const* Wx, const float* const* Wh, const float* cseq,
diff --git a/mlx-vae_amd/csrc/misc.hip b/mlx-vae_amd/csrc/misc.hip
--- a/mlx-vae_amd/csrc/misc.hip
+++ b/mlx-vae_amd/csrc/misc.hip
@@ -1,4 +1,5 @@
 #include "ops.h"
+#include "skinny.h"
 #include <algorithm>
 
 namespace {
@@ -566,11 +567,38 @@
 }
 
 namespace {
+struct Table0 {
+    const float* emb; const float* Wx0; const float* bias0; float* table0;
+    int V, E, G;
+};
+template <bool TABLE>
 __global__ __launch_bounds__(256) void enc_prologue_kernel(const int32_t* __restrict__ x_bt, int32_t* x_tb, int B, int T,
                                                            float4* zero, long nz4, float4* zero2, long nz4b, unsigned* sync, int nsync, int keep,
                                                            const float* __restrict__ cond, const float* __restrict__ Wc,
                                                            const float* __restrict__ bc, float* comb, float* stats,
-                                                           int nstats, int H, int C, float* onehot, int V, int Vp) {
+                                                           int nstats, int H, int C, float* onehot, int V, int Vp, Table0 tb) {
+    if constexpr (TABLE) {
+        __shared__ float red[4 * 256];
+        const int tid = threadIdx.x, lane = tid & 63, wave = tid >> 6;
+        const int nx = tb.G >> 4, ntiles = nx * ((tb.V + 15) >> 4);
+        for (int tile = blockIdx.x; tile < ntiles; tile += gridDim.x) {
+            const int m0 = (tile / nx) * 16, n0 = (tile % nx) * 16;
+            const int arow = min(m0 + (lane & 15), tb.V - 1);
+            const int bcol = min(n0 + (lane & 15), tb.G - 1);
+            f32x4 acc0 = {0.f, 0.f, 0.f, 0.f}, acc1 = {0.f, 0.f, 0.f, 0.f};
+            skinny_accum_kk(acc0, acc1, tb.emb, (long)arow * tb.E, tb.Wx0, (long)bcol * tb.E, tb.E, wave, lane);
+            skinny_store_partial(red, acc0, acc1, wave, lane);
+            __syncthreads();
+            const int row = tid >> 4, col = tid & 15;
+            const int gr = m0 + row, gc = n0 + col;
+            if (gr < tb.V && gc < tb.G) {
+                float v = skinny_reduced(red, row, col);
+                v += tb.bias0[gc];
+                tb.table0[(long)gr * tb.G + gc] = v;
+            }
+            __syncthreads();
+        }
+    }
     const long gt = (long)blockIdx.x * 256 + threadIdx.x, gs = (long)gridDim.x * 256;
     if (onehot) {
         const long n = (long)B * T * Vp;
@@ -602,21 +630,53 @@
 }
 }
 
-extern "C" int arcvae_enc_prologue(const int32_t* x_bt, int32_t* x_tb, float* zero_f32, long n_zero, float* zero2_f32,
-                                   long n_zero2, unsigned* sync_ws, int n_sync, int sync_keep, const float* cond, const float* Wc, const float* bc, float* comb,
-                                   float* stats, int n_stats, float* onehot_ws, int V, int B, int T, int H, int C,
-                                   hipStream_t stream) {
+namespace {
+int launch_enc_prologue(const int32_t* x_bt, int32_t* x_tb, float* zero_f32, long n_zero, float* zero2_f32,
+                        long n_zero2, unsigned* sync_ws, int n_sync, int sync_keep, const float* cond, const float* Wc, const float* bc, float* comb,
+                        float* stats, int n_stats, float* onehot_ws, int V, int B, int T, int H, int C, const Table0* tb,
+                        hipStream_t stream) {
     if (!x_bt || !x_tb || B <= 0 || T <= 0) return ARCVAE_ERR_ARG;
     if (onehot_ws && V <= 0) return ARCVAE_ERR_ARG;
     if (comb && (!cond || !Wc || !bc || !stats || n_stats <= 0 || H <= 0 || C < 0)) return ARCVAE_ERR_ARG;
     if (zero_f32 && ((n_zero % 4) != 0 || (reinterpret_cast<uintptr_t>(zero_f32) & 15) != 0)) return ARCVAE_ERR_ARG;
     if (zero2_f32 && ((n_zero2 % 4) != 0 || (reinterpret_cast<uintptr_t>(zero2_f32) & 15) != 0)) return ARCVAE_ERR_ARG;
     if (n_sync < 0 || (n_sync > 0 && !sync_ws)) return ARCVAE_ERR_ARG;
-    hipLaunchKernelGGL(enc_prologue_kernel, dim3(256), dim3(256), 0, stream, x_bt, x_tb, B, T,
+    if (tb) {
+        if (!tb->emb || !tb->Wx0 || !tb->bias0 || !tb->table0 || tb->V <= 0 || tb->V > 256 || tb->E <= 0 || (tb->E % 64) != 0 ||
+            tb->G <= 0 || (tb->G % 16) != 0 || (reinterpret_cast<uintptr_t>(tb->emb) & 15) != 0 ||
+            (reinterpret_cast<uintptr_t>(tb->Wx0) & 15) != 0)
+            return ARCVAE_ERR_ARG;
+        const int ntiles = (tb->G / 16) * ceil_div(tb->V, 16);
+        hipLaunchKernelGGL(enc_prologue_kernel<true>, dim3(std::max(256, std::min(ntiles, 2048))), dim3(256), 0, stream, x_bt, x_tb, B, T,
+                           reinterpret_cast<float4*>(zero_f32), zero_f32 ? n_zero / 4 : 0L, reinterpret_cast<float4*>(zero2_f32),
+                           zero2_f32 ? n_zero2 / 4 : 0L, sync_ws, n_sync, sync_keep, cond, Wc, bc, comb,
+                           stats, n_stats, H, C, onehot_ws, V, (V + 3) & ~3, *tb);
+        return arcvae_launch_status();
+    }
+    hipLaunchKernelGGL(enc_prologue_kernel<false>, dim3(256), dim3(256), 0, stream, x_bt, x_tb, B, T,
                        reinterpret_cast<float4*>(zero_f32), zero_f32 ? n_zero / 4 : 0L, reinterpret_cast<float4*>(zero2_f32),
                        zero2_f32 ? n_zero2 / 4 : 0L, sync_ws, n_sync, sync_keep, cond, Wc, bc, comb,
-                       stats, n_stats, H, C, onehot_ws, V, (V + 3) & ~3);
-    return arcvae_launch_status();
+                       stats, n_stats, H, C, onehot_ws, V, (V + 3) & ~3, Table0{});
+    return arcvae_launch_status();
+}
+}
+
+extern "C" int arcvae_enc_prologue(const int32_t* x_bt, int32_t* x_tb, float* zero_f32, long n_zero, float* zero2_f32,
+                                   long n_zero2, unsigned* sync_ws, int n_sync, int sync_keep, const float* cond, const float* Wc, const float* bc, float* comb,
+                                   float* stats, int n_stats, float* onehot_ws, int V, int B, int T, int H, int C,
+                                   hipStream_t stream) {
+    return launch_enc_prologue(x_bt, x_tb, zero_f32, n_zero, zero2_f32, n_zero2, sync_ws, n_sync, sync_keep, cond, Wc, bc, comb, stats,
+                               n_stats, onehot_ws, V, B, T, H, C, nullptr, stream);
+}
+
+extern "C" int arcvae_enc_prologue_table0(const int32_t* x_bt, int32_t* x_tb, float* zero_f32, long n_zero, float* zero2_f32,
+                                          long n_zero2, unsigned* sync_ws, int n_sync, int sync_keep, const float* cond, const float* Wc,
+                                          const float* bc, float* comb, float* stats, int n_stats, float* onehot_ws, int V, int B,
+                                          int T, int H, int C, const float* emb, const float* Wx0, const float* bias0,
+                                          float* table0, int E, int G, hipStream_t stream) {
+    const Table0 tb{emb, Wx0, bias0, table0, V, E, G};
+    return launch_enc_prologue(x_bt, x_tb, zero_f32, n_zero, zero2_f32, n_zero2, sync_ws, n_sync, sync_keep, cond, Wc, bc, comb, stats,
+                               n_stats, onehot_ws, V, B, T, H, C, &tb, stream);
 }
 
 extern "C" int arcvae_transpose_tokens(const int32_t* src, int32_t* dst, int B, int T, hipStream_t stream) {
```

Result: no change. 73130 (median of 6 runs) (+0.9%).
